# Fan-Luo/Legal-RAG

Hardware: AMD Instinct MI355X
Metric: queries/sec + Recall@10 (hybrid top-10) on UCC-en (higher is better)
Workload: dtype f32 dense (long batches: fp16 first pass, candidates re-scored in f32) / f64 bm25+fusion; 1 GPU; UCC-en 591 chunks, dense(768-d FlatIP)+BM25 hybrid fusion top-10 (BASELINE configs[1]); unique_queries=1168, top_k=10, fusion=rrf_norm_blend w=0.6/0.4 alpha=0.5 rrf_k=60 min_final=0.2

## Files before the change

### include/amdretrieval.h

```cpp
#ifndef AMDRETRIEVAL_H
#define AMDRETRIEVAL_H

#include <stdint.h>

#ifdef __cplusplus
extern "C" {
#endif

#define AMDR_OK 0
#define AMDR_EINVAL (-1)
#define AMDR_EHIP (-2)
#define AMDR_ENOMEM (-3)
#define AMDR_ENODEV (-4)

#define AMDR_MAX_K 256
#define AMDR_MAX_DIM 1024
#define AMDR_MAXSIM_DIM 128
#define AMDR_MAXSIM_QLEN 32

typedef struct amdr_dense amdr_dense_t;
typedef struct amdr_dense_small amdr_dense_small_t;
typedef struct amdr_bm25 amdr_bm25_t;
typedef struct amdr_maxsim amdr_maxsim_t;
typedef struct amdr_tokenizer amdr_tokenizer_t;
typedef struct amdr_tokenizer_device amdr_tokenizer_device_t;
typedef struct amdr_graph amdr_graph_t;

const char* amdr_last_error(void);
int amdr_version(void);
int amdr_device_count(int32_t* count);
int amdr_device_name(int32_t device, char* buf, int32_t buf_len);
int amdr_workspace_growths(int64_t* out);

int amdr_dense_create(const float* X_host, int64_t n, int32_t d, int32_t device, amdr_dense_t** out);
int amdr_dense_create_from_device(const float* X_dev, int64_t n, int32_t d, int32_t device, amdr_dense_t** out);
int amdr_dense_add(amdr_dense_t* h, const float* X_host, int64_t n_add);
int amdr_dense_ntotal(const amdr_dense_t* h, int64_t* n);
int amdr_dense_dim(const amdr_dense_t* h, int32_t* d);
int amdr_dense_reserve(amdr_dense_t* h, int32_t nq_max, int32_t k_max);
int amdr_dense_search(amdr_dense_t* h, const float* Q_host, int32_t nq, int32_t k,
                      float* scores_host, int64_t* ids_host);
int amdr_dense_search_device(amdr_dense_t* h, const float* Q_dev, int32_t nq, int32_t k,
                             float* scores_dev, int64_t* ids_dev, void* stream);
int amdr_dense_score_rows(amdr_dense_t* h, const float* Q_host, int32_t nq, const int64_t* rows_host, int32_t m,
                          float* scores_host);
int amdr_dense_read_rows(const amdr_dense_t* h, int64_t row0, int64_t nrows, float* out_host);
int amdr_dense_plan_info(const amdr_dense_t* h, int32_t nq, int32_t k, char* buf, int32_t buf_len);
int amdr_dense_workspace_plan(int64_t n, int32_t d, int32_t nq_max, int32_t k_max, int32_t nq, int32_t k, int64_t* out6);
int amdr_dense_hi_counters(amdr_dense_t* h, int64_t* out6);
int amdr_dense_profile_begin(amdr_dense_t* h, int32_t max_launches);
int amdr_dense_profile_end(amdr_dense_t* h, double* total_ms, int32_t* launches);
int amdr_dense_destroy(amdr_dense_t* h);

int amdr_bm25_create(const int64_t* term_ptr, const int32_t* post_doc, const int32_t* post_tf,
                     const double* idf, const int32_t* doc_len, int64_t n_terms, int64_t n_docs,
                     double avgdl, double k1, double b, int32_t device, amdr_bm25_t** out);
int amdr_bm25_ndocs(const amdr_bm25_t* h, int64_t* n);
int amdr_bm25_reserve(amdr_bm25_t* h, int32_t nq_max, int32_t k_max, int64_t total_terms_max);
int amdr_bm25_workspace_plan(int64_t n_docs, int32_t nq_max, int32_t k_max, int32_t nq, int32_t k, int64_t* out2);
int amdr_bm25_plan_info(const amdr_bm25_t* h, int32_t nq, int32_t k, char* buf, int32_t buf_len);
int amdr_bm25_search(amdr_bm25_t* h, const int32_t* q_terms, const int64_t* q_ptr, int32_t nq, int32_t k,
                     double* scores_host, int64_t* ids_host);
int amdr_bm25_search_device(amdr_bm25_t* h, const int32_t* q_terms_dev, const int64_t* q_ptr_dev,
                            int32_t nq, int32_t k, double* scores_dev, int64_t* ids_dev, void* stream);
int amdr_bm25_scores(amdr_bm25_t* h, const int32_t* q_terms, const int64_t* q_ptr, int32_t nq,
                     double* scores_host);
int amdr_bm25_destroy(amdr_bm25_t* h);

int amdr_tokenizer_create(const char* vocab_blob, const int64_t* vocab_offsets, int64_t n_terms, amdr_tokenizer_t** out);
int amdr_tokenizer_encode(const amdr_tokenizer_t* t, const char* text_blob, const int64_t* text_offsets, int32_t nq,
                          int32_t* term_ids, int64_t capacity, int64_t* q_ptr, int32_t* needs_segmenter);
int amdr_tokenizer_encode_joined(const amdr_tokenizer_t* t, const char* text_blob, int64_t n_bytes, int32_t nq,
                                 int32_t* term_ids, int64_t capacity, int64_t* q_ptr, int32_t* needs_segmenter);
int amdr_tokenizer_encode_ptrs(const amdr_tokenizer_t* t, const char* const* texts, const int64_t* n_bytes, int32_t nq,
                               int32_t* term_ids, int64_t capacity, int64_t* q_ptr, int32_t* needs_segmenter);
int amdr_tokenizer_spans(const char* text, int64_t n_bytes, int32_t* starts, int32_t* ends, int32_t capacity,
                         int32_t* n_tokens);
int amdr_tokenizer_destroy(amdr_tokenizer_t* t);
int amdr_tokenizer_pack(const char* const* texts, const int64_t* n_bytes, int32_t nq, char* blob, int64_t capacity,
                        int64_t* offsets);

int amdr_tokenizer_device_create(const amdr_tokenizer_t* host, int32_t device, amdr_tokenizer_device_t** out);
int amdr_tokenizer_device_reserve(amdr_tokenizer_device_t* h, int32_t nq_max, int64_t bytes_max);
int amdr_tokenizer_encode_device(amdr_tokenizer_device_t* h, const char* text_dev, const int64_t* offs_dev, int32_t nq,
                                 int64_t n_bytes, int32_t* term_ids_dev, int64_t capacity, int64_t* q_ptr_dev,
                                 int32_t* needs_segmenter_dev, void* stream);
int amdr_tokenizer_device_destroy(amdr_tokenizer_device_t* h);

int amdr_maxsim_create(const float* D_host, const int64_t* doc_ptr, int64_t n_docs, int32_t dim,
                       int32_t device, amdr_maxsim_t** out);
int amdr_maxsim_ndocs(const amdr_maxsim_t* h, int64_t* n);
int amdr_maxsim_plan_info(const amdr_maxsim_t* h, int32_t nq, char* buf, int32_t buf_len);
int amdr_maxsim_reserve(amdr_maxsim_t* h, int32_t nq_max, int32_t k_max);
int amdr_maxsim_workspace_plan(int64_t n_docs, int32_t split_image, int32_t nq_max, int32_t k_max, int32_t nq, int32_t k,
                               int64_t* out2);
int amdr_maxsim_search(amdr_maxsim_t* h, const float* Q_host, int32_t nq, int32_t q_len, int32_t k,
                       float* scores_host, int64_t* ids_host);
int amdr_maxsim_search_device(amdr_maxsim_t* h, const float* Q_dev, int32_t nq, int32_t q_len, int32_t k,
                              float* scores_dev, int64_t* ids_dev, void* stream);
int amdr_maxsim_scores(amdr_maxsim_t* h, const float* Q_host, int32_t nq, int32_t q_len, float* scores_host);
int amdr_maxsim_destroy(amdr_maxsim_t* h);

#define AMDR_FUSE_RRF_NORM_BLEND 0
#define AMDR_FUSE_RRF 1
#define AMDR_FUSE_WRRF 2
#define AMDR_FUSE_WEIGHTED_SUM 3

typedef struct amdr_fuse_params {
  int32_t method;
  int32_t rrf_k;
  double alpha;
  double w_dense, w_bm25, w_colbert;
  double min_final_score;
} amdr_fuse_params_t;

#define AMDR_FUSE_NVALS 9
#define AMDR_FV_SCORE 0
#define AMDR_FV_RRF_NORM 1
#define AMDR_FV_WSUM 2
#define AMDR_FV_NORM_DENSE 3
#define AMDR_FV_NORM_BM25 4
#define AMDR_FV_NORM_COLBERT 5
#define AMDR_FV_CONTRIB_DENSE 6
#define AMDR_FV_CONTRIB_BM25 7
#define AMDR_FV_CONTRIB_COLBERT 8

int amdr_fuse(const amdr_fuse_params_t* p, int32_t nq,
              const int64_t* dense_ids, const double* dense_scores, int32_t kd,
              const int64_t* bm25_ids, const double* bm25_scores, int32_t kb,
              const int64_t* colbert_ids, const double* colbert_scores, int32_t kc,
              int64_t* out_ids, double* out_vals, int32_t* out_mask, int32_t* out_count);
int amdr_fuse_device(const amdr_fuse_params_t* p, int32_t nq,
                     const int64_t* dense_ids, const float* dense_scores, int32_t kd, const int64_t* dense_row2uid,
                     const int64_t* bm25_ids, const double* bm25_scores, int32_t kb, const int64_t* bm25_row2uid,
                     const int64_t* colbert_ids, const float* colbert_scores, int32_t kc, const int64_t* colbert_row2uid,
                     int64_t* out_ids, double* out_vals, int32_t* out_mask, int32_t* out_count,
                     int32_t device, void* stream);

int amdr_dense_search_fuse_device(amdr_dense_t* h, const float* Q_dev, int32_t nq, int32_t k,
                                  const amdr_fuse_params_t* p, const int64_t* dense_row2uid,
                                  const int64_t* bm25_ids, const double* bm25_scores, int32_t kb,
                                  const int64_t* bm25_row2uid, float* dense_scores_dev, int64_t* dense_ids_dev,
                                  int64_t* out_ids, double* out_vals, int32_t* out_mask, int32_t* out_count,
                                  void* stream);

int amdr_hybrid_small_device(amdr_dense_t* dense, amdr_bm25_t* bm25, const float* Q_dev, const int32_t* q_terms_dev,
                             const int64_t* q_ptr_dev, int32_t nq, int32_t kd, int32_t kb, const amdr_fuse_params_t* p,
                             const int64_t* dense_row2uid, const int64_t* bm25_row2uid, float* dense_scores_dev,
                             int64_t* dense_ids_dev, double* bm25_scores_dev, int64_t* bm25_ids_dev, int64_t* out_ids,
                             double* out_vals, int32_t* out_mask, int32_t* out_count, void* stream);

int amdr_dense_two_pass_fallbacks(amdr_dense_t* h, int64_t* out);
int amdr_dense_small_create(amdr_dense_t* dense, amdr_dense_small_t** out);
int amdr_dense_small_approx_device(amdr_dense_small_t* h, const float* Q_dev, int32_t nq, float* S_dev, int64_t ldS,
                                   float* eps_dev , void* stream);
int amdr_dense_small_destroy(amdr_dense_small_t* h);

int amdr_rerank_blend(int32_t nq, int32_t max_out, const int32_t* count, int64_t* ids, double* vals,
                      int32_t* mask, const double* ce_raw, int32_t top_n, double beta, double* out_rerank);
int amdr_rerank_blend_device(int32_t nq, int32_t max_out, const int32_t* count, int64_t* ids, double* vals,
                             int32_t* mask, const double* ce_raw, int32_t top_n, double beta,
                             double* out_rerank, int32_t device, void* stream);

int amdr_fuse_compact_device(int32_t nq, int32_t max_out, int32_t w, const int64_t* ids, const double* vals,
                             const int32_t* mask, const int32_t* count, int64_t* out_rows, double* out_scores,
                             int32_t* out_mask, int32_t* out_count, int32_t device, void* stream);

typedef struct amdr_graph_params {
  int32_t limit;
  int32_t default_depth;
  int32_t lang;
  int32_t pad0;
  double min_conf;
  const int32_t* rel_max_depth;
  const int32_t* rel_allowed;
  const double* rel_weight;
  const double* decay;
} amdr_graph_params_t;
int amdr_graph_create(const int64_t* node_ptr, const int32_t* edge_dst, const int32_t* edge_rel,
                      const double* edge_conf_raw, const double* edge_conf_eff, const int32_t* edge_has_evidence,
                      const int32_t* node_present, const int64_t* node_row, const int32_t* row_node,
                      const float* row_norm, const int32_t* row_lang, int32_t n_nodes, int64_t n_edges,
                      int64_t n_rows, int32_t n_rel, int32_t device, amdr_graph_t** out);
int amdr_graph_reserve(amdr_graph_t* h, int32_t nq_max, int32_t k_max, int32_t limit_max);
int amdr_graph_walk(amdr_graph_t* h, const int64_t* seeds_host, const int32_t* seed_count_host, int32_t ld,
                    int32_t seed_n, int32_t nq, const amdr_graph_params_t* params, int32_t* out_count,
                    int32_t* out_node, int32_t* out_depth, int32_t* out_parent, int32_t* out_rel, int32_t* out_evidence,
                    double* out_conf);
int amdr_graph_search(amdr_graph_t* h, amdr_dense_t* dense, const float* Q_host, const int64_t* seeds_host,
                      const int32_t* seed_count_host, int32_t ld, int32_t seed_n, int32_t nq, int32_t k,
                      const amdr_graph_params_t* params, int32_t* out_count, int64_t* out_rows, double* out_final,
                      float* out_semantic, int32_t* out_depth, int32_t* out_rel, double* out_conf);
int amdr_graph_search_device(amdr_graph_t* h, amdr_dense_t* dense, const float* Q_dev, const int32_t* qsel_dev,
                             const int64_t* seeds_dev, const int32_t* seed_count_dev, int32_t ld, int32_t seed_n,
                             int32_t ng, int32_t k, const amdr_graph_params_t* params, int32_t* out_count,
                             int64_t* out_rows, double* out_final, float* out_semantic, int32_t* out_depth,
                             int32_t* out_rel, double* out_conf, void* stream);
int amdr_graph_destroy(amdr_graph_t* h);

int amdr_merge_topk_f32_device(const float* scores, const int64_t* ids, int32_t n_parts, int32_t nq, int32_t k_in,
                               int32_t k_out, float* out_scores, int64_t* out_ids, int32_t device, void* stream);
int amdr_merge_topk_f64_device(const double* scores, const int64_t* ids, int32_t n_parts, int32_t nq, int32_t k_in,
                               int32_t k_out, double* out_scores, int64_t* out_ids, int32_t device, void* stream);

typedef struct amdr_shard_chan {
  void* scores;
  int64_t* ids;
  int32_t k;
  int32_t f64;
} amdr_shard_chan_t;
int amdr_shard_row_words(const amdr_shard_chan_t* chans, int32_t n_chan, int64_t* words);
int amdr_shard_pack_device(const amdr_shard_chan_t* chans, int32_t n_chan, int32_t nq, int64_t id_offset, int64_t* send,
                           int32_t device, void* stream);
int amdr_shard_merge_device(const int64_t* gathered, int32_t world, int32_t nq, const amdr_shard_chan_t* out_chans,
                            int32_t n_chan, int32_t device, void* stream);

#ifdef __cplusplus
}
#endif
#endif
```

### legal-rag_amd/_native.py

```python
from __future__ import annotations

import ctypes as C
import math
import os
from pathlib import Path
from typing import Optional, Sequence, Tuple

import numpy as np

LIB_NAME = "libamdretrieval.so"
MAX_K = 256
MAX_DIM = 1024
MAXSIM_DIM = 128
MAXSIM_QLEN = 32
FUSE_NVALS = 9
FUSE_METHODS = {"rrf_norm_blend": 0, "rrf": 1, "wrrf": 2, "weighted_sum": 3}
FV = dict(score=0, rrf_norm=1, weighted_sum=2, dense_norm=3, bm25_norm=4, colbert_norm=5,
          contrib_dense=6, contrib_bm25=7, contrib_colbert=8)

EXPORTS = (
    "amdr_last_error", "amdr_version", "amdr_device_count", "amdr_device_name", "amdr_workspace_growths",
    "amdr_dense_create", "amdr_dense_create_from_device", "amdr_dense_add", "amdr_dense_ntotal", "amdr_dense_dim",
    "amdr_dense_reserve", "amdr_dense_search", "amdr_dense_search_device", "amdr_dense_search_fuse_device", "amdr_hybrid_small_device", "amdr_dense_small_create", "amdr_dense_small_approx_device", "amdr_dense_small_destroy", "amdr_dense_two_pass_fallbacks", "amdr_dense_read_rows", "amdr_dense_score_rows",
    "amdr_dense_plan_info", "amdr_dense_workspace_plan", "amdr_dense_hi_counters", "amdr_dense_profile_begin", "amdr_dense_profile_end", "amdr_dense_destroy",
    "amdr_bm25_create", "amdr_bm25_ndocs", "amdr_bm25_reserve", "amdr_bm25_workspace_plan", "amdr_bm25_plan_info", "amdr_bm25_search", "amdr_bm25_search_device",
    "amdr_bm25_scores", "amdr_bm25_destroy",
    "amdr_tokenizer_create", "amdr_tokenizer_encode", "amdr_tokenizer_encode_joined", "amdr_tokenizer_encode_ptrs", "amdr_tokenizer_spans", "amdr_tokenizer_destroy",
    "amdr_tokenizer_pack", "amdr_tokenizer_device_create", "amdr_tokenizer_device_reserve", "amdr_tokenizer_encode_device",
    "amdr_tokenizer_device_destroy",
    "amdr_maxsim_create", "amdr_maxsim_ndocs", "amdr_maxsim_plan_info", "amdr_maxsim_reserve", "amdr_maxsim_workspace_plan", "amdr_maxsim_search",
    "amdr_maxsim_search_device", "amdr_maxsim_scores", "amdr_maxsim_destroy",
    "amdr_fuse", "amdr_fuse_device", "amdr_rerank_blend", "amdr_rerank_blend_device", "amdr_fuse_compact_device",
    "amdr_merge_topk_f32_device", "amdr_merge_topk_f64_device",
    "amdr_shard_row_words", "amdr_shard_pack_device", "amdr_shard_merge_device",
    "amdr_graph_create", "amdr_graph_reserve", "amdr_graph_walk", "amdr_graph_search", "amdr_graph_search_device",
    "amdr_graph_destroy",
)


SIGNATURES = {
    "amdr_last_error": "", "amdr_version": "", "amdr_device_count": "P", "amdr_device_name": "iPi", "amdr_workspace_growths": "P",
    "amdr_dense_create": "PliiP", "amdr_dense_create_from_device": "PliiP", "amdr_dense_add": "PPl",
    "amdr_dense_ntotal": "PP", "amdr_dense_dim": "PP", "amdr_dense_reserve": "Pii", "amdr_dense_search": "PPiiPP",
    "amdr_dense_search_device": "PPiiPPP", "amdr_dense_search_fuse_device": "PPiiPPPPiPPPPPPPP", "amdr_hybrid_small_device": "PPPPPiiiPPPPPPPPPPPP", "amdr_dense_small_create": "PP", "amdr_dense_small_approx_device": "PPiPlPP", "amdr_dense_small_destroy": "P", "amdr_dense_two_pass_fallbacks": "PP", "amdr_dense_read_rows": "PllP", "amdr_dense_score_rows": "PPiPiP",
    "amdr_dense_plan_info": "PiiPi", "amdr_dense_workspace_plan": "liiiiiP", "amdr_dense_hi_counters": "PP", "amdr_dense_profile_begin": "Pi", "amdr_dense_profile_end": "PPP", "amdr_dense_destroy": "P",
    "amdr_bm25_create": "PPPPPlldddiP", "amdr_bm25_ndocs": "PP", "amdr_bm25_reserve": "Piil", "amdr_bm25_workspace_plan": "liiiiP", "amdr_bm25_plan_info": "PiiPi",
    "amdr_bm25_search": "PPPiiPP", "amdr_bm25_search_device": "PPPiiPPP", "amdr_bm25_scores": "PPPiP",
    "amdr_bm25_destroy": "P",
    "amdr_tokenizer_create": "PPlP", "amdr_tokenizer_encode": "PPPiPlPP", "amdr_tokenizer_encode_joined": "PPliPlPP", "amdr_tokenizer_encode_ptrs": "PPPiPlPP", "amdr_tokenizer_spans": "PlPPiP",
    "amdr_tokenizer_destroy": "P",
    "amdr_tokenizer_pack": "PPiPlP", "amdr_tokenizer_device_create": "PiP", "amdr_tokenizer_device_reserve": "Pil",
    "amdr_tokenizer_encode_device": "PPPilPlPPP", "amdr_tokenizer_device_destroy": "P",
    "amdr_maxsim_create": "PPliiP", "amdr_maxsim_ndocs": "PP", "amdr_maxsim_plan_info": "PiPi", "amdr_maxsim_reserve": "Pii", "amdr_maxsim_workspace_plan": "liiiiiP",
    "amdr_maxsim_search": "PPiiiPP", "amdr_maxsim_search_device": "PPiiiPPP", "amdr_maxsim_scores": "PPiiP",
    "amdr_maxsim_destroy": "P",
    "amdr_fuse": "Pi" + "PPi" * 3 + "PPPP", "amdr_fuse_device": "Pi" + "PPiP" * 3 + "PPPP" + "iP",
    "amdr_rerank_blend": "iiPPPPPidP", "amdr_rerank_blend_device": "iiPPPPPidPiP",
    "amdr_fuse_compact_device": "iiiPPPPPPPPiP",
    "amdr_merge_topk_f32_device": "PPiiiiPPiP", "amdr_merge_topk_f64_device": "PPiiiiPPiP",
    "amdr_shard_row_words": "PiP", "amdr_shard_pack_device": "PiilPiP", "amdr_shard_merge_device": "PiiPiiP",
    "amdr_graph_create": "P" * 11 + "illiiP", "amdr_graph_reserve": "Piii", "amdr_graph_walk": "PPPiiiP" + "P" * 7,
    "amdr_graph_search": "PPPPPiiiiP" + "P" * 7, "amdr_graph_search_device": "PPPPPPiiiiP" + "P" * 8,
    "amdr_graph_destroy": "P",
}
_KIND = {"P": C.c_void_p, "i": C.c_int32, "l": C.c_int64, "d": C.c_double}


class NativeError(RuntimeError):
    """A libamdretrieval call returned a non-zero status."""


class FuseParams(C.Structure):
    _fields_ = [("method", C.c_int32), ("rrf_k", C.c_int32), ("alpha", C.c_double), ("w_dense", C.c_double),
                ("w_bm25", C.c_double), ("w_colbert", C.c_double), ("min_final_score", C.c_double)]


class ShardChan(C.Structure):
    _fields_ = [("scores", C.c_void_p), ("ids", C.c_void_p), ("k", C.c_int32), ("f64", C.c_int32)]


class GraphParams(C.Structure):
    _fields_ = [("limit", C.c_int32), ("default_depth", C.c_int32), ("lang", C.c_int32), ("pad0", C.c_int32),
                ("min_conf", C.c_double), ("rel_max_depth", C.c_void_p), ("rel_allowed", C.c_void_p),
                ("rel_weight", C.c_void_p), ("decay", C.c_void_p)]


GRAPH_MAX_LIMIT = 4096
GRAPH_MAX_SEEDS = 1024


_lib: Optional[C.CDLL] = None


_pystr = False


def _pystrings():
    global _pystr
    if _pystr is False:
        _pystr = None
        p = lib_path().parent / "_amdr_pystrings.so"
        if p.exists() and os.environ.get("AMDR_NO_PYSTRINGS") != "1":
            try:
                import importlib.machinery
                import importlib.util
                loader = importlib.machinery.ExtensionFileLoader("_amdr_pystrings", str(p))
                spec = importlib.util.spec_from_loader("_amdr_pystrings", loader)
                mod = importlib.util.module_from_spec(spec)
                loader.exec_module(mod)
                _pystr = mod
            except Exception:
                _pystr = None
    return _pystr


def lib_path() -> Path:
    env = os.environ.get("AMDR_LIB")
    if env:
        return Path(env)
    return Path(__file__).resolve().parent / "lib" / LIB_NAME


def load() -> C.CDLL:
    global _lib
    if _lib is not None:
        return _lib
    if os.environ.get("AMDR_NO_TORCH_PRELOAD") != "1":
        try:
            import torch
        except Exception:
            pass
    p = lib_path()
    if not p.exists():
        raise NativeError(
            f"{p} not found: the HIP extension is not built. Run `python -c 'import __graft_entry__ as g; g.build()'` "
            f"(or `make -C legal-rag_amd/csrc`). There is no CPU fallback.")
    lib = C.CDLL(str(p))
    lib.amdr_last_error.restype = C.c_char_p
    for name in EXPORTS:
        fn = getattr(lib, name)
        if name != "amdr_last_error":
            fn.restype = C.c_int
        fn.argtypes = [_KIND[k] for k in SIGNATURES[name]]
    _lib = lib
    return lib


def _check(rc: int, what: str) -> None:
    if rc != 0:
        msg = load().amdr_last_error()
        raise NativeError(f"{what} failed (status {rc}): {msg.decode('utf-8', 'replace') if msg else ''}")


def device_count() -> int:
    n = C.c_int32(0)
    rc = load().amdr_device_count(C.byref(n))
    return int(n.value) if rc == 0 else 0


def device_name(device: int = 0) -> str:
    buf = C.create_string_buffer(256)
    _check(load().amdr_device_name(C.c_int32(device), buf, C.c_int32(256)), "amdr_device_name")
    return buf.value.decode()


def dense_workspace_plan(n: int, d: int, nq_max: int, k_max: int, nq: int,
                         k: int) -> Tuple[Tuple[int, int, int], Tuple[int, int, int]]:
    out = (C.c_int64 * 6)()
    _check(load().amdr_dense_workspace_plan(C.c_int64(n), C.c_int32(d), C.c_int32(nq_max), C.c_int32(k_max), C.c_int32(nq),
                                            C.c_int32(k), out), "amdr_dense_workspace_plan")
    v = [int(x) for x in out]
    return tuple(v[:3]), tuple(v[3:])


def bm25_workspace_plan(n_docs: int, nq_max: int, k_max: int, nq: int, k: int) -> Tuple[int, int]:
    out = (C.c_int64 * 2)()
    _check(load().amdr_bm25_workspace_plan(C.c_int64(n_docs), C.c_int32(nq_max), C.c_int32(k_max), C.c_int32(nq),
                                           C.c_int32(k), out), "amdr_bm25_workspace_plan")
    return int(out[0]), int(out[1])


def maxsim_workspace_plan(n_docs: int, split_image: bool, nq_max: int, k_max: int, nq: int, k: int) -> Tuple[int, int]:
    out = (C.c_int64 * 2)()
    _check(load().amdr_maxsim_workspace_plan(C.c_int64(n_docs), C.c_int32(1 if split_image else 0), C.c_int32(nq_max),
                                             C.c_int32(k_max), C.c_int32(nq), C.c_int32(k), out),
           "amdr_maxsim_workspace_plan")
    return int(out[0]), int(out[1])


def workspace_growths() -> int:
    n = C.c_int64(0)
    _check(load().amdr_workspace_growths(C.byref(n)), "amdr_workspace_growths")
    return int(n.value)


def _p(a: Optional[np.ndarray], ctype):
    if a is None:
        return None
    return a.ctypes.data_as(C.POINTER(ctype))


def _vp(ptr: int):
    return C.c_void_p(int(ptr) if ptr else 0)


def _c(a, dtype) -> np.ndarray:
    return np.ascontiguousarray(a, dtype=dtype)


class DenseIndex:

    def __init__(self, X: Optional[np.ndarray] = None, *, device: int = 0, dim: Optional[int] = None,
                 device_ptr: Optional[int] = None, n: Optional[int] = None, keepalive=None):
        lib = load()
        self._h = C.c_void_p()
        self.device = int(device)
        self._keepalive = keepalive
        if device_ptr is not None:
            assert n is not None and dim is not None
            _check(lib.amdr_dense_create_from_device(_vp(device_ptr), C.c_int64(n), C.c_int32(dim),
                                                     C.c_int32(device), C.byref(self._h)),
                   "amdr_dense_create_from_device")
            self.d = int(dim)
        else:
            if X is None:
                X = np.zeros((0, int(dim)), dtype=np.float32)
            X = _c(X, np.float32)
# ... 414 lines not shown
        if keep[3].shape[0] < int(limit) + 1:
            raise ValueError("decay needs limit + 1 entries")
        p = GraphParams(int(limit), int(default_depth), int(lang), 0, float(min_conf), *(x.ctypes.data or None for x in keep))
        return p, keep

    def walk(self, seeds: Sequence[Sequence[int]], params: GraphParams):
        nq = len(seeds)
        ld = max([len(s) for s in seeds] + [1])
        S = np.full((max(nq, 1), ld), -1, dtype=np.int64)
        for i, s in enumerate(seeds):
            S[i, :len(s)] = s
        cnt = np.array([len(s) for s in seeds] + [0] * (nq == 0), dtype=np.int32)
        L = int(params.limit)
        outs = [np.empty((max(nq, 1), L), dtype=t) for t in (np.int32,) * 5 + (np.float64,)]
        oc = np.zeros(max(nq, 1), dtype=np.int32)
        _check(load().amdr_graph_walk(self._h, S.ctypes.data, cnt.ctypes.data, ld, ld, nq, C.byref(params), oc.ctypes.data,
                                      *(o.ctypes.data for o in outs)), "amdr_graph_walk")
        node, depth, parent, rel, evid, conf = outs
        return [[(int(node[q, i]), int(depth[q, i]), int(parent[q, i]), int(rel[q, i]), bool(evid[q, i]),
                  float(conf[q, i])) for i in range(int(oc[q]))] for q in range(nq)]

    def search(self, dense: "DenseIndex", Q: np.ndarray, seeds: np.ndarray, seed_count: np.ndarray, seed_n: int, k: int,
               params: GraphParams):
        Q = _c(Q, np.float32).reshape(-1, dense.d)
        nq = Q.shape[0]
        seeds = _c(seeds, np.int64).reshape(nq, -1)
        seed_count = _c(seed_count, np.int32).reshape(nq)
        out = self._outputs(nq, k)
        _check(load().amdr_graph_search(self._h, dense._h, Q.ctypes.data, seeds.ctypes.data, seed_count.ctypes.data,
                                        seeds.shape[1], int(seed_n), nq, int(k), C.byref(params),
                                        *(out[n].ctypes.data for n in self.OUTS)), "amdr_graph_search")
        return out

    OUTS = ("count", "rows", "final", "semantic", "depth", "relation", "edge_conf")
    _OUT_T = (np.int32, np.int64, np.float64, np.float32, np.int32, np.int32, np.float64)

    @classmethod
    def _outputs(cls, nq: int, k: int):
        return {n: np.empty((nq,) if n == "count" else (nq, k), dtype=t) for n, t in zip(cls.OUTS, cls._OUT_T)}

    def search_device(self, dense: "DenseIndex", q_ptr: int, qsel_ptr: int, seeds_ptr: int, seed_count_ptr: int, ld: int,
                      seed_n: int, ng: int, k: int, params: GraphParams, outs: Sequence[int], stream: int = 0) -> None:
        _check(load().amdr_graph_search_device(self._h, dense._h, _vp(q_ptr), _vp(qsel_ptr), _vp(seeds_ptr),
                                               _vp(seed_count_ptr), int(ld), int(seed_n), int(ng), int(k),
                                               C.byref(params), *(_vp(o) for o in outs), _vp(stream)),
               "amdr_graph_search_device")

    def close(self) -> None:
        if getattr(self, "_h", None) and self._h.value:
            load().amdr_graph_destroy(self._h)
            self._h = C.c_void_p()

    def __del__(self):
        try:
            self.close()
        except Exception:
            pass


def make_fuse_params(*, method: str = "rrf_norm_blend", rrf_k: int = 60, alpha: float = 0.5, w_dense: float = 0.6,
                     w_bm25: float = 0.4, w_colbert: float = 0.35, min_final_score: float = -math.inf) -> FuseParams:
    m = FUSE_METHODS.get(str(method).lower(), 0)
    return FuseParams(m, int(rrf_k), float(alpha), float(w_dense), float(w_bm25), float(w_colbert),
                      float(min_final_score))


def _chan(ids, scores, sdtype, nq):
    if ids is None or scores is None:
        return None, None, 0
    ids = _c(ids, np.int64).reshape(nq, -1)
    scores = _c(scores, sdtype).reshape(nq, -1)
    assert ids.shape == scores.shape
    if ids.shape[1] == 0:
        return None, None, 0
    return ids, scores, int(ids.shape[1])


def fuse(params: FuseParams, nq: int, dense=None, bm25=None, colbert=None):
    di, ds, kd = _chan(*(dense or (None, None)), np.float64, nq)
    bi, bs, kb = _chan(*(bm25 or (None, None)), np.float64, nq)
    ci, cs, kc = _chan(*(colbert or (None, None)), np.float64, nq)
    mo = kd + kb + kc
    out_ids = np.full((nq, max(mo, 1)), -1, dtype=np.int64)
    out_vals = np.zeros((nq, max(mo, 1), FUSE_NVALS), dtype=np.float64)
    out_mask = np.zeros((nq, max(mo, 1)), dtype=np.int32)
    out_count = np.zeros((nq,), dtype=np.int32)
    if mo == 0 or nq == 0:
        return out_ids[:, :0], out_vals[:, :0], out_mask[:, :0], out_count
    _check(load().amdr_fuse(C.byref(params), C.c_int32(nq), _p(di, C.c_int64), _p(ds, C.c_double), C.c_int32(kd),
                            _p(bi, C.c_int64), _p(bs, C.c_double), C.c_int32(kb), _p(ci, C.c_int64),
                            _p(cs, C.c_double), C.c_int32(kc), _p(out_ids, C.c_int64), _p(out_vals, C.c_double),
                            _p(out_mask, C.c_int32), _p(out_count, C.c_int32)), "amdr_fuse")
    return out_ids, out_vals, out_mask, out_count


def fuse_device(params: FuseParams, nq: int, dense, bm25, colbert, out_ids: int, out_vals: int, out_mask: int,
                out_count: int, *, device: int = 0, stream: int = 0) -> None:
    def un(c):
        return c if c is not None else (0, 0, 0, 0)
    d, b, c = un(dense), un(bm25), un(colbert)
    _check(load().amdr_fuse_device(C.byref(params), C.c_int32(nq),
                                   _vp(d[0]), _vp(d[1]), C.c_int32(d[2]), _vp(d[3]),
                                   _vp(b[0]), _vp(b[1]), C.c_int32(b[2]), _vp(b[3]),
                                   _vp(c[0]), _vp(c[1]), C.c_int32(c[2]), _vp(c[3]),
                                   _vp(out_ids), _vp(out_vals), _vp(out_mask), _vp(out_count),
                                   C.c_int32(device), _vp(stream)), "amdr_fuse_device")


def rerank_blend(count: np.ndarray, ids: np.ndarray, vals: np.ndarray, mask: np.ndarray, ce_raw: np.ndarray,
                 beta: float):
    nq, max_out = ids.shape
    ce_raw = _c(ce_raw, np.float64).reshape(nq, -1)
    top_n = int(ce_raw.shape[1])
    out = np.full((nq, max_out, 2), np.nan, dtype=np.float64)
    assert ids.flags.c_contiguous and vals.flags.c_contiguous and mask.flags.c_contiguous
    count = _c(count, np.int32)
    _check(load().amdr_rerank_blend(C.c_int32(nq), C.c_int32(max_out), _p(count, C.c_int32), _p(ids, C.c_int64),
                                    _p(vals, C.c_double), _p(mask, C.c_int32), _p(ce_raw, C.c_double),
                                    C.c_int32(top_n), C.c_double(beta), _p(out, C.c_double)), "amdr_rerank_blend")
    return out


def rerank_blend_device(nq: int, max_out: int, count: int, ids: int, vals: int, mask: int, ce_raw: int, top_n: int,
                        beta: float, out_rerank: int, *, device: int = 0, stream: int = 0) -> None:
    _check(load().amdr_rerank_blend_device(C.c_int32(nq), C.c_int32(max_out), _vp(count), _vp(ids), _vp(vals),
                                           _vp(mask), _vp(ce_raw), C.c_int32(top_n), C.c_double(beta),
                                           _vp(out_rerank), C.c_int32(device), _vp(stream)),
           "amdr_rerank_blend_device")


class DenseSmallApprox:

    def __init__(self, dense: "DenseIndex"):
        self._h = C.c_void_p()
        self._dense = dense
        _check(load().amdr_dense_small_create(dense._h, C.byref(self._h)), "amdr_dense_small_create")

    def approx_device(self, q_ptr: int, nq: int, s_ptr: int, ld: int, eps_ptr: int = 0, stream: int = 0) -> None:
        _check(load().amdr_dense_small_approx_device(self._h, _vp(q_ptr), C.c_int32(nq), _vp(s_ptr), C.c_int64(ld), _vp(eps_ptr),
                                                     _vp(stream)), "amdr_dense_small_approx_device")

    def close(self) -> None:
        if self._h:
            load().amdr_dense_small_destroy(self._h)
            self._h = C.c_void_p()

    def __del__(self):
        try:
            self.close()
        except Exception:
            pass


def hybrid_small_plan(dense: "DenseIndex", bm25: "BM25Index", nq: int, kd: int, kb: int, dense_row2uid: int,
                      bm25_row2uid: int, dense_scores: int, dense_ids: int, bm25_scores: int, bm25_ids: int, out_ids: int,
                      out_vals: int, out_mask: int, out_count: int):
    return (load().amdr_hybrid_small_device, dense._h, bm25._h, C.c_int32(nq), C.c_int32(kd), C.c_int32(kb),
            _vp(dense_row2uid), _vp(bm25_row2uid), _vp(dense_scores), _vp(dense_ids), _vp(bm25_scores), _vp(bm25_ids),
            _vp(out_ids), _vp(out_vals), _vp(out_mask), _vp(out_count))


def hybrid_small_device(plan, params: "FuseParams", q_emb: int, q_terms: int, q_ptr: int, stream: int = 0) -> None:
    fn, dh, bh, nq, kd, kb, m0, m1, ds, di, bs, bi, oi, ov, om, oc = plan
    rc = fn(dh, bh, q_emb, q_terms, q_ptr, nq, kd, kb, C.byref(params), m0, m1, ds, di, bs, bi, oi, ov, om, oc, stream)
    if rc:
        _check(rc, "amdr_hybrid_small_device")


def fuse_compact_device(nq: int, max_out: int, w: int, ids: int, vals: int, mask: int, count: int, out_rows: int,
                        out_scores: int, out_mask: int, out_count: int, *, device: int = 0, stream: int = 0) -> None:
    _check(load().amdr_fuse_compact_device(nq, max_out, w, ids, vals, mask, count, out_rows, out_scores, out_mask, out_count,
                                           device, stream), "amdr_fuse_compact_device")


def merge_topk_device(scores: int, ids: int, n_parts: int, nq: int, k_in: int, k_out: int, out_scores: int,
                      out_ids: int, *, f64: bool, device: int = 0, stream: int = 0) -> None:
    fn = load().amdr_merge_topk_f64_device if f64 else load().amdr_merge_topk_f32_device
    _check(fn(_vp(scores), _vp(ids), C.c_int32(n_parts), C.c_int32(nq), C.c_int32(k_in), C.c_int32(k_out),
              _vp(out_scores), _vp(out_ids), C.c_int32(device), _vp(stream)), "amdr_merge_topk_device")


def shard_chans(chans):
    arr = (ShardChan * len(chans))()
    for c, (sp, ip, k, f64) in zip(arr, chans):
        c.scores, c.ids, c.k, c.f64 = int(sp) if sp else None, int(ip) if ip else None, int(k), 1 if f64 else 0
    return arr, len(chans)


def shard_row_words(ks: Sequence[int]) -> int:
    arr, n = shard_chans([(0, 0, k, False) for k in ks])
    w = C.c_int64(0)
    _check(load().amdr_shard_row_words(arr, C.c_int32(n), C.byref(w)), "amdr_shard_row_words")
    return int(w.value)


def shard_pack_args(args, nq: int, id_offset: int, send_ptr: int, *, device: int = 0, stream: int = 0) -> None:
    _check(load().amdr_shard_pack_device(args[0], args[1], nq, id_offset, send_ptr, device, stream),
           "amdr_shard_pack_device")


def shard_merge_args(gathered_ptr: int, world: int, nq: int, args, *, device: int = 0, stream: int = 0) -> None:
    _check(load().amdr_shard_merge_device(gathered_ptr, world, nq, args[0], args[1], device, stream),
           "amdr_shard_merge_device")


def shard_pack_device(chans, nq: int, id_offset: int, send_ptr: int, *, device: int = 0, stream: int = 0) -> None:
    shard_pack_args(shard_chans(chans), nq, id_offset, send_ptr, device=device, stream=stream)


def shard_merge_device(gathered_ptr: int, world: int, nq: int, out_chans, *, device: int = 0, stream: int = 0) -> None:
    shard_merge_args(gathered_ptr, world, nq, shard_chans(out_chans), device=device, stream=stream)
```

### legal-rag_amd/csrc/bm25.hip

```cpp
#include "common.hpp"
#include "topk.hpp"

#include <cfloat>
#include <cmath>
#include <cstdlib>
#include <mutex>
#include <new>
#include <vector>


#include "bm25_core.hpp"

using namespace amdr;

struct amdr_bm25 {
  int device = 0;
  int64_t n_terms = 0, n_docs = 0, nnz = 0;
  double avgdl = 0, k1 = 1.5, b = 0.75;
  long long* term_ptr = nullptr;
  int* post_doc = nullptr;
  double* post_w = nullptr;
  double* idf = nullptr;
  hipStream_t stream = nullptr;
  std::mutex mu;
  DevBuf part[2], qterms, qptr, sbuf, ibuf, full;
  DevBuf ticket;
};

namespace {

constexpr int kSlabMax = 4096;

struct BmPlan {
  int slab, nslabs, cap, cap_merge, waves;
  size_t lds, part_bytes;
};

void bm_plan(int64_t n_docs, int nq, int k, BmPlan* p) {
  const int64_t n = n_docs > 0 ? n_docs : 1;
  auto balanced = [&](int slab_max) {
    p->nslabs = (int)((n + slab_max - 1) / slab_max);
    p->slab = (int)(((n + p->nslabs - 1) / p->nslabs + 15) / 16 * 16);
    if (p->slab > slab_max) p->slab = slab_max;
    p->nslabs = (int)((n + p->slab - 1) / p->slab);
  };
  balanced(kBmOneWaveDocs);
  const bool argmax = bm_use_argmax(k, p->slab);
  if (!argmax) balanced(kSlabMax);
  p->waves = 1;
  p->cap_merge = topk_cap(k);
  p->cap = argmax ? (k <= 16 ? 16 : kBmArgmaxK) : p->cap_merge;
  p->lds = (size_t)p->slab * sizeof(double) + (size_t)p->waves * p->cap * sizeof(C64) + 4 * sizeof(int) +
           128 * sizeof(long) + 8;
  p->part_bytes = (size_t)p->nslabs * nq * k * sizeof(C64);
}

size_t bm_part_bytes(int64_t n_docs, int nq, int k) {
  BmPlan p;
  bm_plan(n_docs, nq, k, &p);
  return p.part_bytes;
}
size_t bm_reserve_bytes(int64_t n_docs, int nq_max, int k_max) {
  size_t need = 0;
  for (int k = 1; k <= k_max; ++k) {
    const size_t b = bm_part_bytes(n_docs, nq_max, k);
    need = b > need ? b : need;
  }
  return need;
}

static bool bm_select_enabled() {
  const char* e = getenv("AMDR_BM25_SELECT");
  return !(e && e[0] == '0');
}

int bm_run(amdr_bm25* h, int ws, const int* q_terms_dev, const long long* q_ptr_dev, int nq, int k, double* scores_dev,
           int64_t* ids_dev, double* full_dev, hipStream_t st) {
  BmPlan p;
  bm_plan(h->n_docs, nq, k, &p);
  C64* part = nullptr;
  if (scores_dev) {
    int rc = h->part[ws].ensure(bm_part_bytes(h->n_docs, nq, k));
    if (rc) return rc;
    part = h->part[ws].as<C64>();
  }
  const bool direct = scores_dev && p.nslabs == 1;
  double* fs = direct ? scores_dev : nullptr;
  long long* fi = direct ? (long long*)ids_dev : nullptr;
  if (direct) part = nullptr;
  if (p.lds > 48 * 1024) {
    return fail(AMDR_EINVAL, "bm25: slab needs %zu B of LDS", p.lds);
  }
#define AMDR_BM_LAUNCH(NVT)                                                                                          \
  hipLaunchKernelGGL((bm25_score_topk_kernel<1, NVT>), dim3(p.nslabs, nq), dim3(64), p.lds, st, h->term_ptr,         \
                     h->post_doc, h->post_w, h->idf, (long)h->n_terms, (long)h->n_docs, q_terms_dev, q_ptr_dev, nq, k, \
                     p.cap, p.slab, bm_select_enabled() ? 1 : 0, full_dev, part, fs, fi)
  const int nv = bm_use_argmax(k, p.slab) ? (p.slab + 63) / 64 : 1;
  if (nv <= 4) AMDR_BM_LAUNCH(4);
  else if (nv <= 8) AMDR_BM_LAUNCH(8);
  else if (nv <= 10) AMDR_BM_LAUNCH(10);
  else if (nv <= 16) AMDR_BM_LAUNCH(16);
  else if (nv <= 20) AMDR_BM_LAUNCH(20);
  else AMDR_BM_LAUNCH(32);
#undef AMDR_BM_LAUNCH
  AMDR_HIP(hipGetLastError());
  if (scores_dev && !direct) {
    size_t lds = (size_t)kBmWaves * p.cap_merge * sizeof(C64) + kBmWaves * sizeof(int);
    hipLaunchKernelGGL(bm25_merge_kernel, dim3(nq), dim3(256), lds, st, part, p.nslabs, nq, k, p.cap_merge, scores_dev,
                       (long long*)ids_dev);
    AMDR_HIP(hipGetLastError());
  }
  return AMDR_OK;
}

}
namespace amdr {
int bm25_small_raw(amdr_bm25_t* h, int nq, int k, Bm25Raw* out) {
  if (!h->ticket.p) return fail(AMDR_EINVAL, "bm25: handle without arrival counters");
  BmPlan p;
  bm_plan(h->n_docs, nq, k, &p);
  out->term_ptr = h->term_ptr;
  out->post_doc = h->post_doc;
  out->post_w = h->post_w;
  out->idf = h->idf;
  out->n_terms = (long)h->n_terms;
  out->n_docs = (long)h->n_docs;
  out->ticket = h->ticket.as<int>();
  out->slab = p.slab;
  out->nslabs = p.nslabs;
  out->cap = p.cap;
  out->lds = p.lds;
  out->argmax = bm_use_argmax(k, p.slab);
  out->nvt = out->argmax ? (p.slab + 63) / 64 : 1;
  out->select_on = bm_select_enabled();
  return AMDR_OK;
}
std::mutex& bm25_mutex(amdr_bm25_t* h) { return h->mu; }
}
namespace {

template <class T>
int upload(T** dst, const T* src, size_t count) {
  *dst = nullptr;
  size_t bytes = (count + 1) * sizeof(T);
  AMDR_HIP(hipMalloc((void**)dst, bytes));
  if (count) AMDR_HIP(hipMemcpy(*dst, src, count * sizeof(T), hipMemcpyHostToDevice));
  return AMDR_OK;
}

}

extern "C" {

int amdr_bm25_create(const int64_t* term_ptr, const int32_t* post_doc, const int32_t* post_tf, const double* idf,
                     const int32_t* doc_len, int64_t n_terms, int64_t n_docs, double avgdl, double k1, double b,
                     int32_t device, amdr_bm25_t** out) {
  AMDR_REQUIRE(out != nullptr, "bm25_create: out is null");
  *out = nullptr;
  AMDR_REQUIRE(term_ptr && idf && doc_len, "bm25_create: null array");
  AMDR_REQUIRE(n_terms >= 0 && n_docs >= 1 && n_docs < (1ll << 31), "bm25_create: bad sizes");
  AMDR_REQUIRE(n_terms < (1ll << 31), "bm25_create: too many terms");
  AMDR_REQUIRE(term_ptr[0] == 0, "bm25_create: term_ptr[0] != 0");
  for (int64_t t = 0; t < n_terms; ++t)
    AMDR_REQUIRE(term_ptr[t + 1] >= term_ptr[t], "bm25_create: term_ptr not monotone at %lld", (long long)t);
  const int64_t nnz = term_ptr[n_terms];
  AMDR_REQUIRE(nnz == 0 || (post_doc && post_tf), "bm25_create: null postings");
  for (int64_t t = 0; t < n_terms; ++t)
    for (int64_t p = term_ptr[t]; p < term_ptr[t + 1]; ++p) {
      AMDR_REQUIRE(post_doc[p] >= 0 && post_doc[p] < n_docs, "bm25_create: posting %lld doc out of range", (long long)p);
      AMDR_REQUIRE(p == term_ptr[t] || post_doc[p] > post_doc[p - 1],
                   "bm25_create: postings of term %lld not strictly ascending", (long long)t);
    }
  int rc = check_device(device);
  if (rc) return rc;
  amdr_bm25* h = new (std::nothrow) amdr_bm25();
  if (!h) return fail(AMDR_ENOMEM, "bm25_create: host alloc");
  h->device = device;
  h->n_terms = n_terms;
  h->n_docs = n_docs;
  h->nnz = nnz;
  h->avgdl = avgdl;
  h->k1 = k1;
  h->b = b;
  std::vector<double> pw((size_t)nnz);
  {
    const double k1p1 = k1 + 1, one_minus_b = 1 - b;
    for (int64_t p = 0; p < nnz; ++p) {
      const double qf = (double)post_tf[p];
      const double dl = (double)doc_len[post_doc[p]];
      const double denom = qf + k1 * (one_minus_b + b * dl / avgdl);
      pw[(size_t)p] = qf * k1p1 / denom;
    }
  }
  rc = upload(&h->term_ptr, (const long long*)term_ptr, (size_t)n_terms + 1);
  if (!rc) rc = upload(&h->post_doc, post_doc, (size_t)nnz);
  if (!rc) rc = upload(&h->post_w, pw.data(), (size_t)nnz);
  if (!rc) rc = upload(&h->idf, idf, (size_t)n_terms);
  if (!rc && hipStreamCreateWithFlags(&h->stream, hipStreamNonBlocking) != hipSuccess)
    rc = fail(AMDR_EHIP, "bm25_create: stream");
  if (!rc) rc = h->ticket.ensure(64 * sizeof(int));
  if (!rc && hipMemset(h->ticket.p, 0, 64 * sizeof(int)) != hipSuccess) rc = fail(AMDR_EHIP, "bm25_create: memset");
  if (rc) {
    amdr_bm25_destroy(h);
    return rc;
  }
  *out = h;
  return AMDR_OK;
}

int amdr_bm25_ndocs(const amdr_bm25_t* h, int64_t* n) {
  AMDR_REQUIRE(h && n, "bm25_ndocs: null");
  *n = h->n_docs;
  return AMDR_OK;
}

int amdr_bm25_reserve(amdr_bm25_t* h, int32_t nq_max, int32_t k_max, int64_t total_terms_max) {
  AMDR_REQUIRE(h != nullptr, "bm25_reserve: null handle");
  AMDR_REQUIRE(nq_max >= 1 && k_max >= 1 && k_max <= AMDR_MAX_K && total_terms_max >= 0, "bm25_reserve: bad sizes");
  std::lock_guard<std::mutex> g(h->mu);
  AMDR_HIP(hipSetDevice(h->device));
  int rc = h->part[0].ensure(bm_reserve_bytes(h->n_docs, nq_max, k_max));
  if (!rc) rc = h->qterms.ensure((size_t)(total_terms_max + 1) * sizeof(int));
  if (!rc) rc = h->qptr.ensure((size_t)(nq_max + 1) * sizeof(long long));
  if (!rc) rc = h->sbuf.ensure((size_t)nq_max * k_max * sizeof(double));
  if (!rc) rc = h->ibuf.ensure((size_t)nq_max * k_max * sizeof(int64_t));
  return rc;
}

int amdr_bm25_workspace_plan(int64_t n_docs, int32_t nq_max, int32_t k_max, int32_t nq, int32_t k, int64_t* out2) {
  AMDR_REQUIRE(out2 != nullptr, "bm25_workspace_plan: null");
  AMDR_REQUIRE(n_docs >= 1 && n_docs < (1ll << 31), "bm25_workspace_plan: bad n_docs");
  AMDR_REQUIRE(nq_max >= 1 && k_max >= 1 && k_max <= AMDR_MAX_K && nq >= 1 && k >= 1 && k <= AMDR_MAX_K,
               "bm25_workspace_plan: bad sizes");
  out2[0] = (int64_t)bm_reserve_bytes(n_docs, nq_max, k_max);
  out2[1] = (int64_t)bm_part_bytes(n_docs, nq, k);
  return AMDR_OK;
}

int amdr_bm25_plan_info(const amdr_bm25_t* h, int32_t nq, int32_t k, char* buf, int32_t buf_len) {
  AMDR_REQUIRE(h && buf && buf_len > 0, "bm25_plan_info: null");
  AMDR_REQUIRE(nq >= 1 && k >= 1 && k <= AMDR_MAX_K, "bm25_plan_info: bad sizes");
  BmPlan p;
  bm_plan(h->n_docs, nq, k, &p);
  snprintf(buf, buf_len, "bm25_score_topk_kernel slabs=%d of <= %d documents, ranked by %s%s", p.nslabs, p.slab,
           bm_use_argmax(k, p.slab) ? "the register arg-max rounds" : "the staged selector",
           p.nslabs == 1 ? " (one slab: direct)" : " + bm25_merge_kernel");
  return AMDR_OK;
}

static int bm_check(const amdr_bm25* h, const void* qt, const void* qp, int nq, int k) {
  AMDR_REQUIRE(h != nullptr, "bm25: null handle");
  AMDR_REQUIRE(nq >= 0, "bm25: nq=%d", nq);
  AMDR_REQUIRE(k >= 1 && k <= AMDR_MAX_K, "bm25: k=%d outside [1,%d]", k, AMDR_MAX_K);
  AMDR_REQUIRE(nq == 0 || qp, "bm25: null q_ptr");
  (void)qt;
  return AMDR_OK;
}

int amdr_bm25_search_device(amdr_bm25_t* h, const int32_t* q_terms_dev, const int64_t* q_ptr_dev, int32_t nq,
                            int32_t k, double* scores_dev, int64_t* ids_dev, void* stream) {
  int rc = bm_check(h, q_terms_dev, q_ptr_dev, nq, k);
  if (rc) return rc;
  AMDR_REQUIRE(nq == 0 || (scores_dev && ids_dev), "bm25: null output");
  if (nq == 0) return AMDR_OK;
  std::lock_guard<std::mutex> g(h->mu);
  AMDR_HIP(hipSetDevice(h->device));
  return bm_run(h, 0, q_terms_dev, (const long long*)q_ptr_dev, nq, k, scores_dev, ids_dev, nullptr, (hipStream_t)stream);
}

static int bm_stage_queries(amdr_bm25* h, const int32_t* q_terms, const int64_t* q_ptr, int nq) {
  AMDR_REQUIRE(q_ptr[0] == 0, "bm25: q_ptr[0] != 0");
  for (int i = 0; i < nq; ++i) AMDR_REQUIRE(q_ptr[i + 1] >= q_ptr[i], "bm25: q_ptr not monotone");
  const int64_t tot = q_ptr[nq];
  AMDR_REQUIRE(tot == 0 || q_terms, "bm25: null q_terms");
  int rc = h->qterms.ensure((size_t)(tot + 1) * sizeof(int));
  if (!rc) rc = h->qptr.ensure((size_t)(nq + 1) * sizeof(long long));
  if (rc) return rc;
  if (tot) AMDR_HIP(hipMemcpyAsync(h->qterms.p, q_terms, (size_t)tot * sizeof(int), hipMemcpyHostToDevice, h->stream));
  AMDR_HIP(hipMemcpyAsync(h->qptr.p, q_ptr, (size_t)(nq + 1) * sizeof(long long), hipMemcpyHostToDevice, h->stream));
  return AMDR_OK;
}

int amdr_bm25_search(amdr_bm25_t* h, const int32_t* q_terms, const int64_t* q_ptr, int32_t nq, int32_t k,
                     double* scores_host, int64_t* ids_host) {
  int rc = bm_check(h, q_terms, q_ptr, nq, k);
  if (rc) return rc;
  AMDR_REQUIRE(nq == 0 || (scores_host && ids_host), "bm25: null output");
  if (nq == 0) return AMDR_OK;
  std::lock_guard<std::mutex> g(h->mu);
  AMDR_HIP(hipSetDevice(h->device));
// ... 55 lines not shown
```

### legal-rag_amd/csrc/bm25_core.hpp

```cpp
#pragma once
#include "common.hpp"
#include "topk.hpp"

#include <cfloat>
#include <cmath>

namespace amdr {

constexpr int kBmWaves = 4;
constexpr int kBmArgmaxK = 96;
__host__ __device__ inline bool bm_use_argmax(int k, int slab) {
  return slab <= 2048 && (k <= 16 || (k <= kBmArgmaxK && k * ((slab + 63) >> 6) <= 480));
}
constexpr int kBmTok = 32;
constexpr int kBmOneWaveDocs = 2048;

__device__ __forceinline__ long uniform_i64(long v) {
  const unsigned lo = (unsigned)__builtin_amdgcn_readfirstlane((int)(unsigned)((unsigned long)v & 0xffffffffu));
  const unsigned hi = (unsigned)__builtin_amdgcn_readfirstlane((int)(unsigned)((unsigned long)v >> 32));
  return (long)(((unsigned long)hi << 32) | lo);
}

__device__ __forceinline__ long lower_bound_i32(const int* __restrict__ a, long lo, long hi, int key) {
  while (lo < hi) {
// ... 6 lines not shown
  return lo;
}

__device__ __forceinline__ double bm25_ranked(double raw) {
  const double x = raw + 0.0;
  return (x != x) ? -DBL_MAX : x;
}

template <int NV>
__device__ __forceinline__ int bm25_argmax_rounds(const double* sc, int m, int k, long lo, int lane, C64* out) {
  const double ninf = -INFINITY;
  double sv[NV];
#pragma unroll
  for (int v = 0; v < NV; ++v) sv[v] = (lane + 64 * v < m) ? bm25_ranked(sc[lane + 64 * v]) : ninf;
  int got = 0;
#if defined(AMDR_BM_ABL) && AMDR_BM_ABL == 1
  for (int it = 0; it < 1; ++it) {
#else
  for (int it = 0; it < k; ++it) {
#endif
    double lm = sv[0];
#pragma unroll
    for (int v = 1; v < NV; ++v) lm = max_f64_raw(lm, sv[v]);
    const double wm = wave_allmax_f64(lm);
    if (wm == ninf) break;
    unsigned long long fm = 0ull;
    int fv = 0;
#pragma unroll
    for (int v = NV - 1; v >= 0; --v) {
      const unsigned long long hit = __ballot(sv[v] == wm);
      fm = hit ? hit : fm;
      fv = hit ? v : fv;
    }
    const int wl = (int)__builtin_ctzll(fm);
    const bool mine = (lane == wl);
#pragma unroll
    for (int v = 0; v < NV; ++v) sv[v] = (mine && v == fv) ? ninf : sv[v];
    if (lane == 0) out[it] = C64::make(wm, lo + wl + 64 * fv);
    got = it + 1;
  }
  return got;
}

template <int NV>
__device__ __forceinline__ int bm25_select_f32(const double* sc, int m, int k, long lo, int lane, C32* scratch,
                                               double* xs , C64* out) {
  u32 img[NV];
  u32 lb = 0u;
#pragma unroll
  for (int v = 0; v < NV; ++v) {
    const int i = lane + 64 * v;
    img[v] = (i < m) ? ord32((float)sc[lane + 64 * v]) : 0u;
    lb = img[v] > lb ? img[v] : lb;
  }
  u32 T = 0u;
#pragma unroll
  for (int bit = 31; bit >= 0; --bit) {
    const u32 cand = T | (1u << bit);
    T = (__popcll(__ballot(lb >= cand)) >= k) ? cand : T;
  }
  const u32 Te = T > 1u ? T : 1u;
  int mine = 0;
#pragma unroll
  for (int v = 0; v < NV; ++v) mine += (img[v] >= Te) ? 1 : 0;
  int incl = mine;
#pragma unroll
  for (int s = 1; s < 64; s <<= 1) {
    const int o = __shfl_up(incl, s);
    incl += (lane >= s) ? o : 0;
  }
  int cnt = __builtin_amdgcn_readlane(incl, 63);
  const bool overflow = cnt > 64;
  if (!overflow) {
    int at = incl - mine;
#pragma unroll
    for (int v = 0; v < NV; ++v) {
      if (img[v] >= Te) {
        C32 c;
        c.c = ((u64)img[v] << 32) | (u64)(((0xffffu - (u32)(lane + 64 * v)) << 8) | (u32)at);
        scratch[at] = c;
        xs[at] = bm25_ranked(sc[lane + 64 * v]);
        ++at;
      }
    }
  }
  if (overflow) {
    int above = 0;
#pragma unroll
    for (int v = 0; v < NV; ++v) above += __popcll(__ballot(img[v] > T));
    if (T == 0u || above > 64) return -1;
    int need = k - above;
    need = need < 0 ? 0 : need;
    if (need > 0) {
      double x0 = 0.0;
      bool have = false;
#pragma unroll
      for (int v = 0; v < NV; ++v) {
        const u64 mk = __ballot(img[v] == T);
        if (!have && mk) {
          x0 = __shfl(bm25_ranked(sc[lane + 64 * v]), (int)__builtin_ctzll(mk));
          have = true;
        }
      }
      u64 differ = 0ull;
#pragma unroll
      for (int v = 0; v < NV; ++v) differ |= __ballot(img[v] == T && bm25_ranked(sc[lane + 64 * v]) != x0);
      if (differ) return -1;
    }
    cnt = 0;
#pragma unroll
    for (int v = 0; v < NV; ++v) {
      const bool hi = img[v] > T;
      const bool eq = img[v] == T;
      const u64 mh = __ballot(hi), me = __ballot(eq);
      const int before_h = (int)__builtin_amdgcn_mbcnt_hi((u32)(mh >> 32), __builtin_amdgcn_mbcnt_lo((u32)mh, 0u));
      const int before_e = (int)__builtin_amdgcn_mbcnt_hi((u32)(me >> 32), __builtin_amdgcn_mbcnt_lo((u32)me, 0u));
      const int nh = __popcll(mh);
      int ne = __popcll(me);
      ne = ne < need ? ne : need;
      const bool take = hi || (eq && before_e < ne);
      if (take) {
        const int at = cnt + (hi ? before_h : nh + before_e);
        C32 c;
        c.c = ((u64)img[v] << 32) | (u64)(((0xffffu - (u32)(lane + 64 * v)) << 8) | (u32)at);
        scratch[at] = c;
        xs[at] = bm25_ranked(sc[lane + 64 * v]);
      }
      cnt += nh + ne;
      need -= ne;
    }
  }
  wave_lds_fence();
  C32 c = (lane < cnt) ? scratch[lane] : C32::pad();
  if (cnt <= 16)
    c = wave_sortN_desc<C32, 16>(c, lane);
  else if (cnt <= 32)
    c = wave_sortN_desc<C32, 32>(c, lane);
  else
    c = wave_sortN_desc<C32, 64>(c, lane);
  const u32 low = (u32)c.c;
  const int doc = (lane < cnt) ? (int)(0xffffu - (low >> 8)) : 0;
  const double x = xs[(lane < cnt) ? (int)(low & 63u) : 0];
  const u32 im = (u32)(c.c >> 32);
  const u32 im_n = (u32)__shfl_down((int)im, 1);
  const double x_n = __shfl_down(x, 1);
  const bool undecided = lane < k && lane + 1 < cnt && im == im_n && x != x_n;
  if (__ballot(undecided)) return -1;
  const int got = cnt < k ? cnt : k;
  if (lane < got) out[lane] = C64::make(x, lo + doc);
  return got;
}

__device__ __forceinline__ void bm25_all_zero_result(int m, int k, long lo, int lane, size_t row, double* fin_scores,
                                                     long long* fin_ids, C64* part_row) {
  for (int j = lane; j < k; j += 64) {
    const bool v = j < m;
    if (fin_ids) {
      fin_scores[row * k + j] = v ? 0.0 : -DBL_MAX;
      fin_ids[row * k + j] = v ? lo + j : -1ll;
    } else {
      part_row[j] = v ? C64::make(0.0, lo + j) : C64::pad();
    }
  }
}

template <int NV>
__device__ __forceinline__ int bm25_rank_slab(const double* sc, int m, int k, long lo, int lane, bool use_select,
                                              C32* scratch, double* xs, C64* out) {
  int got = -1;
  if (k <= 64 && use_select) {
    got = bm25_select_f32<NV>(sc, m, k, lo, lane, scratch, xs, out);
    wave_lds_fence();
  }
  if (got < 0) {
    got = bm25_argmax_rounds<NV>(sc, m, k, lo, lane, out);
    wave_lds_fence();
  }
  return got;
}

template <int WAVES, int NVT>
__device__ __forceinline__ void bm25_block_query(
    const long long* __restrict__ term_ptr, const int* __restrict__ post_doc, const double* __restrict__ post_w,
    const double* __restrict__ idf, long n_terms, long n_docs, const int* __restrict__ q_terms,
    const long long* __restrict__ q_ptr, int nq, int k, int cap, int slab, int use_select,
    double* __restrict__ scores_out , C64* __restrict__ part ,
    double* __restrict__ fin_scores , long long* __restrict__ fin_ids,
    int qi_arg, int slab_ix, unsigned char* smem) {
  double* sc = reinterpret_cast<double*>(smem);
  C64* lists = reinterpret_cast<C64*>(sc + slab);
  int* cnts = reinterpret_cast<int*>(lists + (size_t)WAVES * cap);
  long* tk_ps = reinterpret_cast<long*>(cnts + 4);
  long* tk_pe = tk_ps + kBmTok;
  double* tk_w = reinterpret_cast<double*>(tk_pe + kBmTok);
  int* tk_n = reinterpret_cast<int*>(tk_ps + 128);
  constexpr int NT = WAVES * 64;

  const int tid = threadIdx.x, lane = tid & 63, wave = tid >> 6;
  const int qi = qi_arg;
  const long lo = (long)slab_ix * slab;
  long hi = lo + slab;
  if (hi > n_docs) hi = n_docs;
  const int m = (int)(hi - lo);

  for (int i = tid; i < m; i += NT) sc[i] = 0.0;
  block_sync<WAVES>();

  int nt_total = 0;
  const long t0 = q_ptr[qi], t1 = q_ptr[qi + 1];
  for (long tb = t0; tb < t1; tb += kBmTok) {
    const int nt_all = (int)((t1 - tb) < kBmTok ? (t1 - tb) : kBmTok);
    if (tid < 64) {
      long ps = 0, pe = 0;
      double w = 0.0;
      if (tid < nt_all) {
        const int term = q_terms[tb + tid];
        if (term >= 0 && term < n_terms) {
          const long p0 = term_ptr[term], p1 = term_ptr[term + 1];
          ps = (lo == 0) ? p0 : lower_bound_i32(post_doc, p0, p1, (int)lo);
          pe = (hi >= n_docs) ? p1 : lower_bound_i32(post_doc, ps, p1, (int)hi);
          w = idf[term];
        }
      }
      const bool keep = pe > ps;
      const unsigned long long km = __ballot(keep);
      const unsigned long long below = (tid == 0) ? 0ull : (km & (~0ull >> (64 - tid)));
      if (keep) {
        const int at = __popcll(below);
        tk_ps[at] = ps;
        tk_pe[at] = pe;
        tk_w[at] = w;
      }
      if (tid == 0) *tk_n = __popcll(km);
    }
    block_sync<WAVES>();
    const int nt = __builtin_amdgcn_readfirstlane(*tk_n);
    nt_total += nt;
    if (nt == 0) {
      block_sync<WAVES>();
      continue;
    }
    constexpr int kAhead = 8;
    int t = 0, base = 0;
    long ps = uniform_i64(tk_ps[0]);
    int len = __builtin_amdgcn_readfirstlane((int)(tk_pe[0] - tk_ps[0]));
    double w = tk_w[0];
#if defined(AMDR_BM_ABL) && AMDR_BM_ABL == 2
    t = nt;
#endif
    while (t < nt) {
      int dd[kAhead];
      double ww[kAhead], wv[kAhead];
      bool ok[kAhead];
#pragma unroll
      for (int u = 0; u < kAhead; ++u) {
        const bool have = t < nt;
        const int j = base + tid;
        ok[u] = have && j < len;
        int jj = ok[u] ? j : len - 1;
        jj = jj < 0 ? 0 : jj;
        dd[u] = post_doc[ps + jj];
        ww[u] = post_w[ps + jj];
        wv[u] = w;
        if (have) {
          base += NT;
          if (base >= len) {
            ++t;
            base = 0;
            if (t < nt) {
              ps = uniform_i64(tk_ps[t]);
              len = __builtin_amdgcn_readfirstlane((int)(tk_pe[t] - tk_ps[t]));
              w = tk_w[t];
            }
          }
        }
      }
#pragma unroll
      for (int u = 0; u < kAhead; ++u) {
        if (WAVES == 1) {
          if (ok[u])
            __hip_atomic_fetch_add(&sc[dd[u] - lo], wv[u] * ww[u], __ATOMIC_RELAXED, __HIP_MEMORY_SCOPE_WAVEFRONT);
        } else {
          if (ok[u]) sc[dd[u] - lo] += wv[u] * ww[u];
          block_sync<WAVES>();
        }
      }
      if (WAVES == 1) wave_lds_fence();
    }
  }

  if (scores_out) {
    for (int i = tid; i < m; i += NT) scores_out[(size_t)qi * n_docs + lo + i] = sc[i];
  }
  if (!part && !fin_ids) return;
  if (nt_total == 0) {
    if (wave == 0)
      bm25_all_zero_result(m, k, lo, lane, (size_t)qi, fin_scores, fin_ids,
                           part ? part + ((size_t)slab_ix * nq + qi) * k : nullptr);
    return;
  }
#if defined(AMDR_BM_ABL) && AMDR_BM_ABL == 3
  if (fin_ids && tid < k) {
    fin_ids[(size_t)qi * k + tid] = tid;
    fin_scores[(size_t)qi * k + tid] = sc[tid];
  }
  return;
#endif

  WaveTopK<C64> tk;
  tk.init(lists + (size_t)wave * cap, cap, k);
  bool done = false;
  if (WAVES == 1 && bm_use_argmax(k, slab)) {
    C32* scratch = reinterpret_cast<C32*>(tk_ps);
    double* xs = reinterpret_cast<double*>(tk_ps + 64);
    const int got = bm25_rank_slab<NVT>(sc, m, k, lo, lane, use_select != 0, scratch, xs, tk.buf);
    tk.cnt = got;
    done = true;
  }
  if (!done) {
    for (int base = wave * 64; base < m; base += WAVES * 64) {
      int i = base + lane;
      bool v = i < m;
      C64 c = v ? C64::make(sc[i], lo + i) : C64::pad();
      tk.push_lanes(c, v, lane);
    }
    tk.finalize(lane);
  }
  if (WAVES > 1) block_combine_topk(tk, lists, cap, WAVES, wave, lane, cnts);
  if (wave == 0) {
    if (fin_ids) {
      for (int j = lane; j < k; j += 64) {
        bool v = j < tk.cnt;
        fin_scores[(size_t)qi * k + j] = v ? unord64(tk.buf[j].key) : -DBL_MAX;
        fin_ids[(size_t)qi * k + j] = v ? tk.buf[j].idv : -1ll;
      }
    } else {
      C64* dst = part + ((size_t)slab_ix * nq + qi) * k;
      for (int j = lane; j < k; j += 64) dst[j] = (j < tk.cnt) ? tk.buf[j] : C64::pad();
    }
  }
}

template <int WAVES, int NVT>
__global__ __launch_bounds__(WAVES * 64) void bm25_score_topk_kernel(
    const long long* __restrict__ term_ptr, const int* __restrict__ post_doc, const double* __restrict__ post_w,
    const double* __restrict__ idf, long n_terms, long n_docs, const int* __restrict__ q_terms,
    const long long* __restrict__ q_ptr, int nq, int k, int cap, int slab, int use_select,
    double* __restrict__ scores_out , C64* __restrict__ part ,
    double* __restrict__ fin_scores , long long* __restrict__ fin_ids) {
  extern __shared__ __attribute__((aligned(16))) unsigned char smem[];
  bm25_block_query<WAVES, NVT>(term_ptr, post_doc, post_w, idf, n_terms, n_docs, q_terms, q_ptr, nq, k, cap, slab, use_select, scores_out, part, fin_scores, fin_ids,
                               (int)blockIdx.y, (int)blockIdx.x, smem);
}

static __global__ __launch_bounds__(256) void bm25_merge_kernel(const C64* __restrict__ part, int nparts, int nq, int k,
                                                          int cap, double* __restrict__ out_scores,
                                                          long long* __restrict__ out_ids) {
  extern __shared__ __attribute__((aligned(16))) unsigned char smem[];
  C64* lists = reinterpret_cast<C64*>(smem);
  int* cnts = reinterpret_cast<int*>(lists + (size_t)kBmWaves * cap);
  const int lane = threadIdx.x & 63, wave = threadIdx.x >> 6;
  const int qi = blockIdx.x;
  WaveTopK<C64> tk;
  tk.init(lists + (size_t)wave * cap, cap, k);
  const long total = (long)nparts * k;
  for (long base = (long)wave * 64; base < total; base += (long)kBmWaves * 64) {
    long i = base + lane;
    bool v = i < total;
    C64 c = C64::pad();
    if (v) {
      long p = i / k, j = i - p * k;
      c = part[((size_t)p * nq + qi) * k + j];
      v = !c.is_pad();
    }
    tk.push_lanes(c, v, lane);
  }
  tk.finalize(lane);
  block_combine_topk(tk, lists, cap, kBmWaves, wave, lane, cnts);
  if (wave == 0) {
    for (int j = lane; j < k; j += 64) {
      bool v = j < tk.cnt;
      C64 c = v ? tk.buf[j] : C64::pad();
      out_scores[(size_t)qi * k + j] = v ? unord64(c.key) : -DBL_MAX;
      out_ids[(size_t)qi * k + j] = v ? c.idv : -1ll;
    }
  }
}

}
```

### legal-rag_amd/csrc/dense.hip

```cpp
#include "common.hpp"
#include "dense_dot.hpp"
#include "topk.hpp"

#include <algorithm>
#include <cfloat>
#include <mutex>
#include <new>
#include <vector>

namespace amdr {

constexpr int kWaves = 4;

template <int NQ, int CH, int U, bool NT>
__global__ __launch_bounds__(256) void dense_scan_topk_kernel(const float* __restrict__ X, long n, int d,
                                                               const float* __restrict__ Q, int nq_total, int k,
                                                               int cap, long rows_per_block,
                                                               C32* __restrict__ part ,
                                                               float* __restrict__ fin_scores ,
                                                               long long* __restrict__ fin_ids) {
  extern __shared__ __attribute__((aligned(16))) unsigned char smem[];
  C32* lists = reinterpret_cast<C32*>(smem);
  int* cnts = reinterpret_cast<int*>(lists + (size_t)kWaves * NQ * cap);

  const int lane = threadIdx.x & 63;
  const int wave = threadIdx.x >> 6;
  const int qbase = blockIdx.y * NQ;

  float4 q[NQ][CH];
#pragma unroll
  for (int b = 0; b < NQ; ++b) {
#pragma unroll
    for (int c = 0; c < CH; ++c) {
      int col = c * 256 + lane * 4;
      bool ok = (qbase + b < nq_total) && (col < d);
      q[b][c] = ok ? *reinterpret_cast<const float4*>(Q + (size_t)(qbase + b) * d + col) : make_float4(0, 0, 0, 0);
    }
  }

  WaveTopK<C32> tk[NQ];
#pragma unroll
  for (int b = 0; b < NQ; ++b) tk[b].init(lists + ((size_t)b * kWaves + wave) * cap, cap, k);

  const long row_lo = (long)blockIdx.x * rows_per_block;
  long row_hi = row_lo + rows_per_block;
  if (row_hi > n) row_hi = n;

  for (long r0 = row_lo + (long)wave * U; r0 < row_hi; r0 += (long)kWaves * U) {
    float4 x[U][CH];
#pragma unroll
    for (int u = 0; u < U; ++u) {
      long r = r0 + u;
      if (r >= row_hi) r = row_hi - 1;
      const float* xr = X + (size_t)r * d;
#pragma unroll
      for (int c = 0; c < CH; ++c) {
        int col = c * 256 + lane * 4;
        if (NT) {
          typedef float nt4 __attribute__((ext_vector_type(4)));
          const nt4 t_ = (col < d) ? __builtin_nontemporal_load(reinterpret_cast<const nt4*>(xr + col)) : nt4{0, 0, 0, 0};
          x[u][c] = make_float4(t_.x, t_.y, t_.z, t_.w);
        } else {
          x[u][c] = (col < d) ? *reinterpret_cast<const float4*>(xr + col) : make_float4(0, 0, 0, 0);
        }
      }
    }
#pragma unroll
    for (int u = 0; u < U; ++u) {
      const long r = r0 + u;
      const bool rv = r < row_hi;
#pragma unroll
      for (int b = 0; b < NQ; ++b) {
        float acc = 0.f;
#pragma unroll
        for (int c = 0; c < CH; ++c) acc = dot4(x[u][c], q[b][c], acc);
        acc = wave_sum_to_lane63(acc);
        float s = __int_as_float(__builtin_amdgcn_readlane(__float_as_int(acc), 63));
        if (rv) tk[b].push_uniform(C32::make(s, (u32)r), lane);
      }
    }
  }

#pragma unroll
  for (int b = 0; b < NQ; ++b) tk[b].finalize(lane);
#pragma unroll
  for (int b = 0; b < NQ; ++b) {
    block_combine_topk(tk[b], lists + (size_t)b * kWaves * cap, cap, kWaves, wave, lane, cnts);
    if (wave == 0 && qbase + b < nq_total) {
      if (fin_ids) {
        for (int j = lane; j < k; j += 64) {
          const bool v = j < tk[b].cnt;
          const C32 c = v ? tk[b].buf[j] : C32::pad();
          fin_scores[(size_t)(qbase + b) * k + j] = v ? c.score() : -FLT_MAX;
          fin_ids[(size_t)(qbase + b) * k + j] = v ? c.id() : -1ll;
        }
      } else {
        C32* dst = part + ((size_t)blockIdx.x * nq_total + (qbase + b)) * k;
        for (int j = lane; j < k; j += 64) dst[j] = (j < tk[b].cnt) ? tk[b].buf[j] : C32::pad();
      }
    }
    __syncthreads();
  }
}

__global__ __launch_bounds__(256) void dense_score_rows_kernel(const float* __restrict__ X, long n, int d,
                                                                const float* __restrict__ Q, int nq,
                                                                const long long* __restrict__ rows, int m,
                                                                float* __restrict__ out) {
  const int lane = threadIdx.x & 63, wave = threadIdx.x >> 6;
  const long idx = (long)blockIdx.x * kWaves + wave;
  if (idx >= (long)nq * m) return;
  const int qi = (int)(idx / m);
  const long long r = rows[idx];
  if (r < 0 || r >= n) {
    if (lane == 0) out[idx] = -FLT_MAX;
    return;
  }
  const float acc = dense_row_dot(X + (size_t)r * d, Q + (size_t)qi * d, d, lane);
  if (lane == 63) out[idx] = acc;
}

__global__ __launch_bounds__(256) void dense_all_scores_kernel(const float* __restrict__ X, long n, int d,
                                                                const float* __restrict__ Q, int nq, long ldS,
                                                                float* __restrict__ S) {
  const int lane = threadIdx.x & 63, wave = threadIdx.x >> 6;
  const long idx = (long)blockIdx.x * kWaves + wave;
  if (idx >= (long)nq * n) return;
  const int qi = (int)(idx / n);
  const long r = idx - (long)qi * n;
  const float acc = dense_row_dot(X + (size_t)r * d, Q + (size_t)qi * d, d, lane);
  if (lane == 63) S[(size_t)qi * ldS + r] = acc;
}

__global__ __launch_bounds__(256) void dense_merge_kernel(const C32* __restrict__ part, int nparts, int nq, int k,
                                                           int cap, float* __restrict__ out_scores,
                                                           long long* __restrict__ out_ids) {
  extern __shared__ __attribute__((aligned(16))) unsigned char smem[];
  C32* lists = reinterpret_cast<C32*>(smem);
  int* cnts = reinterpret_cast<int*>(lists + (size_t)kWaves * cap);
  const int lane = threadIdx.x & 63, wave = threadIdx.x >> 6;
  const int qi = blockIdx.x;
  WaveTopK<C32> tk;
  tk.init(lists + (size_t)wave * cap, cap, k);
  const long total = (long)nparts * k;
  for (long base = (long)wave * 64; base < total; base += (long)kWaves * 64) {
    long i = base + lane;
    bool v = i < total;
    C32 c = C32::pad();
    if (v) {
      long p = i / k, j = i - p * k;
      c = part[((size_t)p * nq + qi) * k + j];
      v = !c.is_pad();
    }
// ... 324 lines not shown
  p->kc = kc;
  p->tiles = ((long)h->n + 31) / 32;
  dense_mfma_plan((long)h->n, h->d, m, k, &p->scan, grids);
  p->ldM = (p->tiles + 31) / 32 * 32;
  p->scan.ld = p->ldM;
  p->ldS2 = (long)kc * 32;
  p->qcap = dense_hi2_qcap((long)h->n, p->qtiles, kc);
  p->off_S2 = up((size_t)m * p->ldM * sizeof(float));
  p->off_MT = p->off_S2 + up((size_t)m * p->ldS2 * sizeof(float));
  p->off_qlist = p->off_MT + up((size_t)(2048 + 64 * kHi2Tiles) * 64 * sizeof(float));
  p->smat_bytes = p->off_qlist + up((size_t)m * p->qcap * sizeof(C32));
  p->off_count = up((size_t)m * kc * sizeof(int));
  p->off_unres = p->off_count + up((size_t)m * sizeof(int));
  p->off_tau = p->off_unres + up((size_t)m * sizeof(int));
  p->off_qcount = p->off_tau + up((size_t)m * sizeof(float));
  p->off_flag = p->off_qcount + up((size_t)m * sizeof(unsigned int));
  p->aux_bytes = p->off_flag + 256;
}

struct TwoLevelPlan {
  DenseMfmaPlan scan, tk1, pass2;
  long tiles, cand_rows;
  size_t m_bytes, s2_bytes, aux_bytes, part_bytes;
};
void two_level_plan(const amdr_dense* h, int m, int k, TwoLevelPlan* t, bool grids = true) {
  t->tiles = ((long)h->n + 31) / 32;
  dense_mfma_plan((long)h->n, h->d, m, k, &t->scan, grids);
  dense_mfma_plan(t->tiles, h->d, m, k, &t->tk1, false);
  t->scan.ld = t->tk1.ld;
  t->cand_rows = (long)m * k * 32;
  dense_mfma_plan(t->cand_rows, h->d, m, k, &t->pass2, grids);
  t->m_bytes = ((size_t)m * t->tk1.ld * sizeof(float) + 255) / 256 * 256;
  t->s2_bytes = ((size_t)m * t->pass2.ld * sizeof(float) + 255) / 256 * 256;
  t->aux_bytes = (size_t)m * k * (sizeof(int64_t) + sizeof(float)) + (size_t)(m * k + 64) * sizeof(int) + 256 + 256;
  t->part_bytes = t->tk1.part_bytes > t->pass2.part_bytes ? t->tk1.part_bytes : t->pass2.part_bytes;
}

struct Need {
  size_t smat, part, aux;
  void add(const Need& o) { smat = std::max(smat, o.smat), part = std::max(part, o.part), aux = std::max(aux, o.aux); }
};
size_t score_rows_bytes(const amdr_dense* h, int nq) { return (size_t)nq * (size_t)(((long)h->n + 31) / 32 * 32) * sizeof(float); }

Need pass_need(const amdr_dense* h, Form form, int m, int k) {
  if (form == Form::Scan) {
    ScanPlan p;
    make_plan(h->n, h->d, m, k, &p);
    return {0, p.part_bytes, 0};
  }
  if (form == Form::TwoLevel) {
    TwoLevelPlan t;
    two_level_plan(h, m, k, &t, false);
    return {t.m_bytes + t.s2_bytes, t.part_bytes, t.aux_bytes};
  }
  if (form == Form::Hi) {
    Hi2Plan p;
    hi2_plan(h, m, k, hi_kc_max(k), &p, false);
    return {p.smat_bytes, 0, p.aux_bytes};
  }
  DenseMfmaPlan p;
  dense_mfma_plan((long)h->n, h->d, m, k, &p, false);
  return {p.s_bytes, p.part_bytes, 0};
}
Need call_need(const amdr_dense* h, const Route& r, int nq, int k) {
  const Form form = r.hi ? Form::TwoLevel : r.form;
  const int chunk = r.hi ? two_level_chunk(nq, k) : r.chunk;
  Need need = pass_need(h, form, chunk, k);
  if (nq % chunk) need.add(pass_need(h, form, nq % chunk, k));
  if (r.hi) need.add(pass_need(h, Form::Hi, hi2_chunk(h, nq), k));
  return need;
}
Need reserve_need(const amdr_dense* h, const DensePins& pins, int nq_max, int k_max) {
  Need need{0, 0, 0};
  int ks[8], nk = 0;
  for (int k = 1; k < k_max; ++k)
    if (topk_cap(k + 1) != topk_cap(k)) ks[nk++] = k;
  ks[nk++] = k_max;
  int nq = 1;
  for (; nq <= nq_max; ++nq) {
    const Route r = dense_route(h, pins, nq, k_max);
    if (r.form != Form::Scan && r.form != Form::RowWaves) break;
    for (int i = 0; i < nk; ++i) need.add(pass_need(h, r.form, r.chunk, ks[i]));
    if (r.form == Form::RowWaves) need.add({score_rows_bytes(h, r.chunk), 0, 0});
  }
  if (nq > nq_max) return need;
  int k_batched = 0;
  for (int k = 1; k <= k_max; ++k) {
    const Route lo = dense_route(h, pins, nq, k), hi = dense_route(h, pins, nq_max, k);
    if (lo.form == Form::Batched || hi.form == Form::Batched) k_batched = k;
    if (hi.hi) need.add(pass_need(h, Form::Hi, hi2_chunk(h, nq_max), k));
    if (hi.hi || lo.form == Form::TwoLevel || hi.form == Form::TwoLevel)
      for (int m = two_level_chunk(nq_max, k); m >= 1; --m) need.add(pass_need(h, Form::TwoLevel, m, k));
  }
  if (k_batched)
    for (int m = batched_chunk(h, nq_max); m >= 1; --m) need.add(pass_need(h, Form::Batched, m, k_batched));
  return need;
}
int ensure_need(amdr_dense* h, int ws, const Need& need) {
  int rc = h->smat[ws].ensure(need.smat);
  if (!rc) rc = h->part[ws].ensure(need.part);
  if (!rc) rc = h->aux[ws].ensure(need.aux);
  return rc;
}

template <class F>
int profiled(amdr_dense* h, hipStream_t st, F&& launch) {
  const bool on = h->prof_on && (size_t)(h->prof_used + 2) <= h->prof_ev.size();
  if (on) AMDR_HIP(hipEventRecord(h->prof_ev[h->prof_used], st));
  const int rc = launch();
  if (rc) return rc;
  if (on) {
    AMDR_HIP(hipEventRecord(h->prof_ev[h->prof_used + 1], st));
    h->prof_used += 2;
  }
  return AMDR_OK;
}

int launch_merge(const C32* part, int nparts, int nq, int k, int cap, float* out_scores, int64_t* out_ids, hipStream_t st) {
  const size_t lds = (size_t)kWaves * cap * sizeof(C32) + kWaves * sizeof(int);
  hipLaunchKernelGGL(dense_merge_kernel, dim3(nq), dim3(256), lds, st, part, nparts, nq, k, cap, out_scores, (long long*)out_ids);
  AMDR_HIP(hipGetLastError());
  return AMDR_OK;
}
int topk_pass(const DenseMfmaPlan& p, const float* S, long cols, int m, int k, DevBuf& partb, float* out_scores,
              int64_t* out_ids, hipStream_t st) {
  const bool direct = p.slabs == 1;
  int rc = dense_mfma_launch_topk(p, S, cols, m, k, partb.p, direct ? out_scores : nullptr, direct ? out_ids : nullptr, st);
  if (rc || direct) return rc;
  return launch_merge(partb.as<C32>(), p.slabs, m, k, p.cap, out_scores, out_ids, st);
}

bool small_hi_ready(amdr_dense* h, int m, hipStream_t st) {
  if (h->small_failed) return false;
  hipStreamCaptureStatus cs = hipStreamCaptureStatusNone;
  const bool capturing = st && hipStreamIsCapturing(st, &cs) == hipSuccess && cs != hipStreamCaptureStatusNone;
  if (!h->small) {
    if (capturing) return false;
    if (dense_small_create_from(h->device, h->X, h->n, h->d, &h->small) != AMDR_OK || !dense_small_usable(h->small)) {
      h->small_failed = true;
      return false;
    }
  }
  const size_t need = (size_t)m * sizeof(float);
  if (capturing && (h->small_eps.cap < need || !h->small_fb.p)) return false;
  if (h->small_eps.ensure(need) != AMDR_OK) return false;
  if (!h->small_fb.p) {
    if (h->small_fb.ensure(sizeof(unsigned int)) != AMDR_OK) return false;
    (void)hipMemset(h->small_fb.p, 0, sizeof(unsigned int));
  }
  return capturing ? true : dense_small_reserve(h->small, m) == AMDR_OK;
}

int run_search_batched(amdr_dense* h, int ws, const DensePins& pins, const Route& r, const float* Q_dev, int nq, int k,
                       float* scores_dev, int64_t* ids_dev, hipStream_t st, const FuseTail* tail) {
  float* S = h->smat[ws].as<float>();
  const long n = (long)h->n;
  DenseMfmaPlan p;
  int rc;
  for (int q0 = 0; q0 < nq; q0 += r.chunk) {
    const int m = nq - q0 < r.chunk ? nq - q0 : r.chunk;
    if (q0 == 0 || m != r.chunk) dense_mfma_plan(n, h->d, m, k, &p);
    const PassForm f = batched_pass_form(h, pins, r, p, m, k, tail);
    const float* Qc = Q_dev + (size_t)q0 * h->d;
    float* os = scores_dev + (size_t)q0 * k;
    int64_t* oi = ids_dev + (size_t)q0 * k;
    if (f.small_hi && small_hi_ready(h, m, st)) {
      rc = profiled(h, st, [&] { return amdr_dense_small_approx_device(h->small, Qc, m, S, p.ld, h->small_eps.as<float>(), st); });
      if (rc) return rc;
      if ((rc = dense_hi_select_launch(tail, q0, S, p.ld, n, m, k, h->X, Qc, h->d, h->small_eps.as<float>(), os, oi,
                                       h->small_fb.as<unsigned int>(), st)))
        return rc;
      continue;
    }
    rc = profiled(h, st, [&]() -> int {
      if (f.scores == PassForm::RowWaves) {
        hipLaunchKernelGGL(dense_all_scores_kernel, dim3(ceil_div((long)m * n, kWaves)), dim3(256), 0, st, h->X, n, h->d, Qc,
                           m, p.ld, S);
        AMDR_HIP(hipGetLastError());
        return AMDR_OK;
      }
      if (f.scores == PassForm::Panel) {
        DensePanelPlan pp;
        dense_panel_plan(n, h->d, m, &pp);
        return dense_panel_launch_scores(pp, h->X, n, h->d, Qc, m, p.ld, S, st);
      }
      return dense_mfma_launch_scores(p, h->X, n, h->d, Qc, m, S, st);
    });
    if (rc) return rc;
    if (f.select_fuse) {
      if ((rc = dense_select_fuse_launch(*tail, q0, S, p.ld, n, m, k, p.cap, os, oi, st))) return rc;
      continue;
    }
    if ((rc = topk_pass(p, S, n, m, k, h->part[ws], os, oi, st))) return rc;
    if (tail && (rc = dense_fuse_plain_launch(*tail, q0, m, k, os, oi, st))) return rc;
  }
  return AMDR_OK;
}

int two_level_pass(amdr_dense* h, int ws, const float* Qc, int m, int k, float* out_scores, int64_t* out_ids,
                   hipStream_t st) {
  TwoLevelPlan t;
  two_level_plan(h, m, k, &t);
  float* M = h->smat[ws].as<float>();
  float* S2 = reinterpret_cast<float*>(reinterpret_cast<unsigned char*>(h->smat[ws].p) + t.m_bytes);
  unsigned char* aux = reinterpret_cast<unsigned char*>(h->aux[ws].p);
  int64_t* tile_ids = reinterpret_cast<int64_t*>(aux);
  float* tile_max = reinterpret_cast<float*>(aux + (size_t)m * k * sizeof(int64_t));
  int* list = reinterpret_cast<int*>(aux + (size_t)m * k * (sizeof(int64_t) + sizeof(float)));
  int* count = list + (size_t)m * k;
  int rc;
  if ((rc = profiled(h, st, [&] { return dense_mfma_launch_scores(t.scan, h->X, (long)h->n, h->d, Qc, m, M, st, 1); }))) return rc;
  if ((rc = topk_pass(t.tk1, M, t.tiles, m, k, h->part[ws], tile_max, tile_ids, st))) return rc;
  if ((rc = dense_tiles_unique_launch(tile_ids, m * k, t.tiles, list, count, st))) return rc;
  if ((rc = dense_mfma_launch_scores(t.pass2, h->X, t.cand_rows, h->d, Qc, m, S2, st, 2, list, count, (long)h->n))) return rc;
  if ((rc = topk_pass(t.pass2, S2, t.cand_rows, m, k, h->part[ws], out_scores, out_ids, st))) return rc;
  return dense_tiles_remap_launch(out_ids, m * k, list, count, (long)h->n, st);
}

int hi2_pass(amdr_dense* h, int ws, const float* Qc, int m, int k, int kc, float* out_scores, int64_t* out_ids, hipStream_t st) {
  Hi2Plan p;
  hi2_plan(h, m, k, kc, &p);
  unsigned char* sm = reinterpret_cast<unsigned char*>(h->smat[ws].p);
  unsigned char* ax = reinterpret_cast<unsigned char*>(h->aux[ws].p);
  float* M = reinterpret_cast<float*>(sm);
  float* S2 = reinterpret_cast<float*>(sm + p.off_S2);
  float* MT = reinterpret_cast<float*>(sm + p.off_MT);
  C32* qlist = reinterpret_cast<C32*>(sm + p.off_qlist);
  int* list = reinterpret_cast<int*>(ax);
  int* count = reinterpret_cast<int*>(ax + p.off_count);
  int* unres = reinterpret_cast<int*>(ax + p.off_unres);
  float* tau = reinterpret_cast<float*>(ax + p.off_tau);
  unsigned int* qcount = reinterpret_cast<unsigned int*>(ax + p.off_qcount);
  int* flag = reinterpret_cast<int*>(ax + p.off_flag);
  unsigned int* stats = h->stats.as<unsigned int>();
  int rc;
  if ((rc = dense_hi2_launch_sample(h->X, (long)h->n, h->d, Qc, m, p.qtiles, MT, st, h->x_scale))) return rc;
  if ((rc = dense_hi2_launch_tau(MT, (long)h->n, h->d, m, p.qtiles, kc, tau, qcount, flag, stats, st))) return rc;
  {
    const char* sp = getenv("AMDR_DENSE_HI_SCANS");
    const bool split = sp && sp[0] == 's';
    const int qt = dense_hi_max_queries(h->d);
    for (int y = 0; y < (split ? p.qtiles : 1); ++y) {
      const int q0 = y * qt, mq = split ? (m - q0 < qt ? m - q0 : qt) : m;
      rc = profiled(h, st, [&] {
        return dense_hi2_launch_emit(h->X, (long)h->n, h->d, Qc + (size_t)q0 * h->d, mq, tau + q0, qlist + (size_t)q0 * p.qcap,
                                     qcount + q0, p.qcap, st, h->x_scale, split ? 1 : p.qtiles);
      });
      if (rc) return rc;
    }
  }
  h->hi_queries += m;
  h->hi_passes += p.qtiles;
  if ((rc = dense_hi2_launch_select(qlist, qcount, p.qcap, m, kc, k, Qc, h->d, h->row_norm_max, h->x_scale, p.tiles, list,
                                    count, unres, flag, stats + 2, st)))
    return rc;
  if ((rc = dense_mfma_launch_scores(p.scan, h->X, (long)h->n, h->d, Qc, m, M, st, 1, nullptr, nullptr, 0, flag))) return rc;
  if ((rc = dense_hi2_launch_exact_select(M, p.ldM, p.tiles, m, k, kc, list, count, unres, flag, st))) return rc;
  if ((rc = dense_rescore_tiles_launch(h->X, (long)h->n, h->d, Qc, m, list, count, kc, kc, p.ldS2, S2, st))) return rc;
  return dense_final_topk_launch(S2, p.ldS2, list, count, kc, kc, (long)h->n, m, k, out_scores, out_ids, st);
}

int run_search_two_level(amdr_dense* h, int ws, const DensePins& pins, Route r, const float* Q_dev, int nq, int k,
                         float* scores_dev, int64_t* ids_dev, hipStream_t st) {
  hipStreamCaptureStatus cap_st = hipStreamCaptureStatusNone;
  (void)hipStreamIsCapturing(st, &cap_st);
  const bool capturing = cap_st != hipStreamCaptureStatusNone;
  if (r.hi && !capturing && hi_adapt(h, pins)) r = dense_route(h, pins, nq, k);
  const bool hi = r.form == Form::Hi;
  int rc;
  for (int q0 = 0; q0 < nq; q0 += r.chunk) {
    const int m = nq - q0 < r.chunk ? nq - q0 : r.chunk;
    const float* Qc = Q_dev + (size_t)q0 * h->d;
    float* os = scores_dev + (size_t)q0 * k;
    int64_t* oi = ids_dev + (size_t)q0 * k;
    rc = hi ? hi2_pass(h, ws, Qc, m, k, r.kc, os, oi, st) : two_level_pass(h, ws, Qc, m, k, os, oi, st);
    if (rc) return rc;
  }
  if (hi && h->hi_host && !capturing && !h->hi_copy_pending) {
    AMDR_HIP(hipMemcpyAsync(h->hi_host, h->stats.as<unsigned int>() + 2, 3 * sizeof(unsigned int), hipMemcpyDeviceToHost, st));
    AMDR_HIP(hipEventRecord(h->hi_ev, st));
    h->hi_copy_pending = true;
  }
  return AMDR_OK;
}

int run_search_scan(amdr_dense* h, int ws, const float* Q_dev, int nq, int k, float* scores_dev, int64_t* ids_dev,
                    hipStream_t st) {
  ScanPlan p;
  make_plan(h->n, h->d, nq, k, &p);
  C32* part = h->part[ws].as<C32>();
  const bool direct = h->n > 0 && p.grid_x == 1;
  float* fs = direct ? scores_dev : nullptr;
  int64_t* fi = direct ? ids_dev : nullptr;
  if (h->n > 0) {
    const int rc = profiled(h, st, [&] {
      switch (p.nq_per_block) {
        case 1: return launch_scan_ch<1>(p, h, Q_dev, nq, k, part, fs, fi, st);
        case 2: return launch_scan_ch<2>(p, h, Q_dev, nq, k, part, fs, fi, st);
        case 4: return launch_scan_ch<4>(p, h, Q_dev, nq, k, part, fs, fi, st);
        default: return launch_scan_ch<8>(p, h, Q_dev, nq, k, part, fs, fi, st);
      }
    });
    if (rc) return rc;
  }
  if (direct) return AMDR_OK;
  return launch_merge(part, h->n > 0 ? p.grid_x : 0, nq, k, p.cap, scores_dev, ids_dev, st);
}

int run_search(amdr_dense* h, int ws, const float* Q_dev, int nq, int k, float* scores_dev, int64_t* ids_dev,
               hipStream_t st, const FuseTail* tail = nullptr) {
  const DensePins pins = read_pins();
  const Route r = dense_route(h, pins, nq, k);
  int rc = ensure_need(h, ws, call_need(h, r, nq, k));
  if (rc) return rc;
  switch (r.form) {
    case Form::Batched: return run_search_batched(h, ws, pins, r, Q_dev, nq, k, scores_dev, ids_dev, st, tail);
    case Form::RowWaves: rc = run_search_batched(h, ws, pins, r, Q_dev, nq, k, scores_dev, ids_dev, st, nullptr); break;
    case Form::TwoLevel:
    case Form::Hi: rc = run_search_two_level(h, ws, pins, r, Q_dev, nq, k, scores_dev, ids_dev, st); break;
    case Form::Scan: rc = run_search_scan(h, ws, Q_dev, nq, k, scores_dev, ids_dev, st); break;
  }
  if (rc || !tail) return rc;
  return dense_fuse_plain_launch(*tail, 0, nq, k, scores_dev, ids_dev, st);
}

int check_search_args(const amdr_dense* h, const void* Q, int nq, int k, const void* s, const void* i) {
// ... 52 lines not shown

extern "C" {

int amdr_dense_create(const float* X_host, int64_t n, int32_t d, int32_t device, amdr_dense_t** out) {
  AMDR_REQUIRE(out != nullptr, "dense_create: out is null");
  *out = nullptr;
  AMDR_REQUIRE(n >= 0 && n < (1ll << 32), "dense_create: n=%lld outside [0, 2^32)", (long long)n);
  AMDR_REQUIRE(d >= 4 && d <= AMDR_MAX_DIM && d % 4 == 0, "dense_create: d=%d must be a multiple of 4 in [4,%d]", d,
               AMDR_MAX_DIM);
  AMDR_REQUIRE(n == 0 || X_host != nullptr, "dense_create: X is null");
  int rc = check_device(device);
  if (rc) return rc;
  amdr_dense* h = new (std::nothrow) amdr_dense();
  if (!h) return fail(AMDR_ENOMEM, "dense_create: host alloc");
  h->device = device;
  h->n = n;
  h->d = d;
  h->cap_rows = n;
  hipError_t e = hipStreamCreateWithFlags(&h->stream, hipStreamNonBlocking);
  if (e == hipSuccess && n > 0) e = hipMalloc((void**)&h->X, (size_t)n * d * sizeof(float));
  if (e == hipSuccess && n > 0) e = hipMemcpy(h->X, X_host, (size_t)n * d * sizeof(float), hipMemcpyHostToDevice);
  if (e != hipSuccess) {
    amdr_dense_destroy(h);
    return fail(e == hipErrorOutOfMemory ? AMDR_ENOMEM : AMDR_EHIP, "dense_create: %s", hipGetErrorString(e));
  }
  if ((rc = update_stats(h, 0, n))) {
    amdr_dense_destroy(h);
    return rc;
  }
  *out = h;
  return AMDR_OK;
}

int amdr_dense_create_from_device(const float* X_dev, int64_t n, int32_t d, int32_t device, amdr_dense_t** out) {
  AMDR_REQUIRE(out != nullptr, "dense_create_from_device: out is null");
  *out = nullptr;
  AMDR_REQUIRE(n >= 0 && n < (1ll << 32), "dense_create_from_device: n=%lld outside [0, 2^32)", (long long)n);
  AMDR_REQUIRE(d >= 4 && d <= AMDR_MAX_DIM && d % 4 == 0, "dense_create_from_device: bad d=%d", d);
  AMDR_REQUIRE(n == 0 || X_dev != nullptr, "dense_create_from_device: X is null");
  AMDR_REQUIRE(((uintptr_t)X_dev & 15) == 0, "dense_create_from_device: X must be 16-byte aligned");
  int rc = check_device(device);
  if (rc) return rc;
  amdr_dense* h = new (std::nothrow) amdr_dense();
  if (!h) return fail(AMDR_ENOMEM, "dense_create_from_device: host alloc");
  h->device = device;
  h->n = n;
  h->d = d;
  h->cap_rows = n;
  h->X = const_cast<float*>(X_dev);
  h->owns = false;
  hipError_t e = hipStreamCreateWithFlags(&h->stream, hipStreamNonBlocking);
  if (e != hipSuccess) {
    amdr_dense_destroy(h);
    return fail(AMDR_EHIP, "dense_create_from_device: %s", hipGetErrorString(e));
  }
  AMDR_HIP(hipDeviceSynchronize());
  if ((rc = update_stats(h, 0, n))) {
    amdr_dense_destroy(h);
    return rc;
  }
  *out = h;
  return AMDR_OK;
}

int amdr_dense_add(amdr_dense_t* h, const float* X_host, int64_t n_add) {
  AMDR_REQUIRE(h != nullptr, "dense_add: null handle");
  AMDR_REQUIRE(h->owns, "dense_add: handle wraps caller-owned memory");
  AMDR_REQUIRE(n_add >= 0 && (n_add == 0 || X_host), "dense_add: bad arguments");
  AMDR_REQUIRE(h->n + n_add < (1ll << 32), "dense_add: too many rows");
  std::lock_guard<std::mutex> g(h->mu);
  AMDR_HIP(hipSetDevice(h->device));
  if (n_add == 0) return AMDR_OK;
  if (h->n + n_add > h->cap_rows) {
    int64_t ncap = h->cap_rows * 2 > h->n + n_add ? h->cap_rows * 2 : h->n + n_add;
    float* nx = nullptr;
    AMDR_HIP(hipMalloc((void**)&nx, (size_t)ncap * h->d * sizeof(float)));
    if (h->n > 0) AMDR_HIP(hipMemcpy(nx, h->X, (size_t)h->n * h->d * sizeof(float), hipMemcpyDeviceToDevice));
    if (h->X) (void)hipFree(h->X);
    h->X = nx;
    h->cap_rows = ncap;
  }
  AMDR_HIP(hipMemcpy(h->X + (size_t)h->n * h->d, X_host, (size_t)n_add * h->d * sizeof(float), hipMemcpyHostToDevice));
  const int64_t row0 = h->n;
  h->n += n_add;
  if (h->small) {
    (void)hipDeviceSynchronize();
    (void)amdr_dense_small_destroy(h->small);
    h->small = nullptr;
  }
  h->small_failed = false;
  h->hi_level = 0;
  h->hi_off = false;
  if (h->hi_copy_pending && hipEventSynchronize(h->hi_ev) == hipSuccess) {
    h->hi_copy_pending = false;
    for (int i = 0; i < 3; ++i) h->hi_seen[i] = h->hi_host[i];
  }
  h->lvl_f0 = h->hi_seen[1];
  h->lvl_p0 = (int64_t)h->hi_seen[2];
  return update_stats(h, row0, n_add);
}

int amdr_dense_ntotal(const amdr_dense_t* h, int64_t* n) {
  AMDR_REQUIRE(h && n, "dense_ntotal: null");
  *n = h->n;
  return AMDR_OK;
}
int amdr_dense_dim(const amdr_dense_t* h, int32_t* d) {
  AMDR_REQUIRE(h && d, "dense_dim: null");
  *d = h->d;
  return AMDR_OK;
}

int amdr_dense_reserve(amdr_dense_t* h, int32_t nq_max, int32_t k_max) {
  AMDR_REQUIRE(h != nullptr, "dense_reserve: null handle");
  AMDR_REQUIRE(nq_max >= 1 && k_max >= 1 && k_max <= AMDR_MAX_K, "dense_reserve: bad sizes");
  std::lock_guard<std::mutex> g(h->mu);
  AMDR_HIP(hipSetDevice(h->device));
  const DensePins pins = read_pins();
  int rc = ensure_need(h, 0, reserve_need(h, pins, nq_max, k_max));
  if (rc) return rc;
  if ((rc = h->qbuf.ensure((size_t)nq_max * h->d * sizeof(float)))) return rc;
  if ((rc = h->sbuf.ensure((size_t)nq_max * k_max * sizeof(float)))) return rc;
  if (small_hi_shape(h, pins, nq_max, k_max < 12 ? k_max : 12, 0))
    (void)small_hi_ready(h, batched_chunk(h, nq_max), nullptr);
  return h->ibuf.ensure((size_t)nq_max * k_max * sizeof(int64_t));
}

int amdr_dense_search_device(amdr_dense_t* h, const float* Q_dev, int32_t nq, int32_t k, float* scores_dev,
                             int64_t* ids_dev, void* stream) {
  int rc = check_search_args(h, Q_dev, nq, k, scores_dev, ids_dev);
  if (rc) return rc;
  if (nq == 0) return AMDR_OK;
  std::lock_guard<std::mutex> g(h->mu);
  AMDR_HIP(hipSetDevice(h->device));
  return run_search(h, 0, Q_dev, nq, k, scores_dev, ids_dev, (hipStream_t)stream);
}

int amdr_dense_search_fuse_device(amdr_dense_t* h, const float* Q_dev, int32_t nq, int32_t k,
                                  const amdr_fuse_params_t* p, const int64_t* dense_row2uid, const int64_t* bm25_ids,
                                  const double* bm25_scores, int32_t kb, const int64_t* bm25_row2uid,
                                  float* dense_scores_dev, int64_t* dense_ids_dev, int64_t* out_ids, double* out_vals,
                                  int32_t* out_mask, int32_t* out_count, void* stream) {
  int rc = check_search_args(h, Q_dev, nq, k, dense_scores_dev, dense_ids_dev);
  if (rc) return rc;
  AMDR_REQUIRE(p != nullptr, "dense_search_fuse: null params");
  AMDR_REQUIRE(p->method >= 0 && p->method <= AMDR_FUSE_WEIGHTED_SUM, "dense_search_fuse: method=%d", p->method);
  AMDR_REQUIRE(kb >= 0 && kb <= AMDR_MAX_K && (kb == 0 || (bm25_ids && bm25_scores)), "dense_search_fuse: bad BM25 lists");
  AMDR_REQUIRE(nq == 0 || (out_ids && out_vals && out_mask && out_count), "dense_search_fuse: null output");
  if (nq == 0) return AMDR_OK;
  std::lock_guard<std::mutex> g(h->mu);
  AMDR_HIP(hipSetDevice(h->device));
  FuseTail tail{p, dense_row2uid, bm25_ids, bm25_scores, kb, bm25_row2uid, out_ids, out_vals, out_mask, out_count};
  return run_search(h, 0, Q_dev, nq, k, dense_scores_dev, dense_ids_dev, (hipStream_t)stream, &tail);
}

int amdr_dense_search(amdr_dense_t* h, const float* Q_host, int32_t nq, int32_t k, float* scores_host,
                      int64_t* ids_host) {
  int rc = check_search_args(h, Q_host, nq, k, scores_host, ids_host);
  if (rc) return rc;
  if (nq == 0) return AMDR_OK;
  std::lock_guard<std::mutex> g(h->mu);
  AMDR_HIP(hipSetDevice(h->device));
  if ((rc = h->qbuf.ensure((size_t)nq * h->d * sizeof(float)))) return rc;
  if ((rc = h->sbuf.ensure((size_t)nq * k * sizeof(float)))) return rc;
  if ((rc = h->ibuf.ensure((size_t)nq * k * sizeof(int64_t)))) return rc;
  AMDR_HIP(hipMemcpyAsync(h->qbuf.p, Q_host, (size_t)nq * h->d * sizeof(float), hipMemcpyHostToDevice, h->stream));
  rc = run_search(h, 1, h->qbuf.as<float>(), nq, k, h->sbuf.as<float>(), h->ibuf.as<int64_t>(), h->stream);
  if (rc) return rc;
  AMDR_HIP(hipMemcpyAsync(scores_host, h->sbuf.p, (size_t)nq * k * sizeof(float), hipMemcpyDeviceToHost, h->stream));
  AMDR_HIP(hipMemcpyAsync(ids_host, h->ibuf.p, (size_t)nq * k * sizeof(int64_t), hipMemcpyDeviceToHost, h->stream));
  AMDR_HIP(hipStreamSynchronize(h->stream));
  return AMDR_OK;
}

int amdr_dense_score_rows(amdr_dense_t* h, const float* Q_host, int32_t nq, const int64_t* rows_host, int32_t m,
                          float* scores_host) {
  AMDR_REQUIRE(h != nullptr, "dense_score_rows: null handle");
  AMDR_REQUIRE(nq >= 0 && m >= 0, "dense_score_rows: bad sizes");
  if (nq == 0 || m == 0) return AMDR_OK;
  AMDR_REQUIRE(Q_host && rows_host && scores_host, "dense_score_rows: null buffer");
  std::lock_guard<std::mutex> g(h->mu);
  AMDR_HIP(hipSetDevice(h->device));
  int rc;
  const size_t cnt = (size_t)nq * m;
  if ((rc = h->qbuf.ensure((size_t)nq * h->d * sizeof(float)))) return rc;
  if ((rc = h->sbuf.ensure(cnt * sizeof(float)))) return rc;
  if ((rc = h->ibuf.ensure(cnt * sizeof(int64_t)))) return rc;
  AMDR_HIP(hipMemcpyAsync(h->qbuf.p, Q_host, (size_t)nq * h->d * sizeof(float), hipMemcpyHostToDevice, h->stream));
  AMDR_HIP(hipMemcpyAsync(h->ibuf.p, rows_host, cnt * sizeof(int64_t), hipMemcpyHostToDevice, h->stream));
  hipLaunchKernelGGL(dense_score_rows_kernel, dim3(ceil_div((long)cnt, kWaves)), dim3(256), 0, h->stream, h->X,
                     (long)h->n, h->d, h->qbuf.as<float>(), nq, h->ibuf.as<long long>(), m, h->sbuf.as<float>());
  AMDR_HIP(hipGetLastError());
  AMDR_HIP(hipMemcpyAsync(scores_host, h->sbuf.p, cnt * sizeof(float), hipMemcpyDeviceToHost, h->stream));
  AMDR_HIP(hipStreamSynchronize(h->stream));
  return AMDR_OK;
}

int amdr_dense_read_rows(const amdr_dense_t* h, int64_t row0, int64_t nrows, float* out_host) {
  AMDR_REQUIRE(h && out_host, "dense_read_rows: null");
  AMDR_REQUIRE(row0 >= 0 && nrows >= 0 && row0 + nrows <= h->n, "dense_read_rows: range outside [0,%lld)",
               (long long)h->n);
  AMDR_HIP(hipSetDevice(h->device));
  if (nrows)
    AMDR_HIP(hipMemcpy(out_host, h->X + (size_t)row0 * h->d, (size_t)nrows * h->d * sizeof(float),
                       hipMemcpyDeviceToHost));
  return AMDR_OK;
}

int amdr_dense_workspace_plan(int64_t n, int32_t d, int32_t nq_max, int32_t k_max, int32_t nq, int32_t k, int64_t* out6) {
  AMDR_REQUIRE(out6 != nullptr, "dense_workspace_plan: null");
  AMDR_REQUIRE(n >= 1 && n < (1ll << 32) && d >= 4 && d <= AMDR_MAX_DIM && d % 4 == 0, "dense_workspace_plan: bad shape");
  AMDR_REQUIRE(nq_max >= 1 && k_max >= 1 && k_max <= AMDR_MAX_K && nq >= 1 && k >= 1 && k <= AMDR_MAX_K,
               "dense_workspace_plan: bad sizes");
  amdr_dense h;
  h.n = n;
  h.d = d;
  h.hi_ok = dense_hi_supported(d);
  const DensePins pins = read_pins();
  const Need res = reserve_need(&h, pins, nq_max, k_max), used = call_need(&h, dense_route(&h, pins, nq, k), nq, k);
  out6[0] = (int64_t)res.smat, out6[1] = (int64_t)res.part, out6[2] = (int64_t)res.aux;
  out6[3] = (int64_t)used.smat, out6[4] = (int64_t)used.part, out6[5] = (int64_t)used.aux;
  return AMDR_OK;
}

int amdr_dense_plan_info(const amdr_dense_t* h, int32_t nq, int32_t k, char* buf, int32_t buf_len) {
  AMDR_REQUIRE(h && buf && buf_len > 0, "dense_plan_info: null");
  AMDR_REQUIRE(nq >= 1 && k >= 1 && k <= AMDR_MAX_K, "dense_plan_info: bad sizes");
  const DensePins pins = read_pins();
  const Route r = dense_route(h, pins, nq, k);
  const int m = r.chunk;
  if (h->n <= 0) {
    snprintf(buf, buf_len, "empty index");
  } else if (r.form == Form::Hi) {
    Hi2Plan p;
    hi2_plan(h, m, k, r.kc, &p);
    snprintf(buf, buf_len,
             "dense_hi_tilemax_kernel fp16 first pass queries_per_launch=%d scans_per_launch=%d (%d per scan, one tail): per-query lists of the "
             "approximate tile maxima above a sampled threshold (every %ld-th tile, width level %d) -> top-%d + rounding-bound "
             "check + exact re-scoring of each query's tiles at or above its cut (<= %d each) + top-k: 4 launches behind the "
             "scan(s), the exact first pass behind a device flag in 2",
             m, p.qtiles, m < dense_hi_max_queries(h->d) ? m : dense_hi_max_queries(h->d),
             dense_hi2_sample_stride((long)h->n, p.qtiles), r.hi_level, r.kc, r.kc);
  } else if (r.form == Form::TwoLevel) {
    TwoLevelPlan t;
    two_level_plan(h, m, k, &t);
    snprintf(buf, buf_len,
             "dense_mfma_scores_kernel tile-maxima grid=%dx%d queries_per_launch=%d two-level: top-%d of %ld tile maxima "
             "+ re-scoring of <= %d candidate tiles + top-k%s",
             t.scan.grid_x, t.scan.grid_y, m, k, t.tiles, m * k,
             r.hi ? " (fp16 first pass given up: too many unresolved queries)" : "");
  } else if (r.form != Form::Scan) {
    DenseMfmaPlan p;
    dense_mfma_plan((long)h->n, h->d, m, k, &p);
    const PassForm f = batched_pass_form(h, pins, r, p, m, k, nullptr);
    const char* tail = p.slabs == 1 ? "scores_slab_topk_kernel" : "scores_slab_topk_kernel + dense_merge_kernel";
    if (f.small_hi && !h->small_failed) {
      snprintf(buf, buf_len,
               "dsh_scores_kernel fp16 first pass queries_per_launch=%d (dsh_split_queries_kernel + v_mfma_f32_32x32x16_f16 on "
               "fp16 roundings of both operands, proven per-query bound) + dense_hi_select_fuse_kernel (rows inside 2 eps of the "
               "k-th best re-scored exactly, top-k, fusion); exact form: dense_panel_scores_kernel",
               m);
    } else if (f.scores == PassForm::RowWaves) {
      snprintf(buf, buf_len, "dense_all_scores_kernel (one wave per query x row) + %s", tail);
    } else if (f.scores == PassForm::Panel) {
      DensePanelPlan pp;
      dense_panel_plan((long)h->n, h->d, m, &pp);
      snprintf(buf, buf_len, "dense_panel_scores_kernel nb=%d parts=%d blocks=%d queries_per_launch=%d + %s", pp.nb,
               pp.parts, pp.m_tiles * pp.parts, m, tail);
    } else {
      snprintf(buf, buf_len, "dense_mfma_scores_kernel query-tiles-in-LDS grid=%dx%d queries_per_launch=%d + %s",
               p.grid_x, p.grid_y, m, tail);
    }
  } else {
    ScanPlan p;
    make_plan(h->n, h->d, nq, k, &p);
    snprintf(buf, buf_len, "dense_scan_topk_kernel<NQ=%d> grid=%dx%d%s", p.nq_per_block, p.grid_x, p.grid_y,
             p.grid_x == 1 ? "" : " + dense_merge_kernel");
  }
  return AMDR_OK;
}

int amdr_dense_hi_counters(amdr_dense_t* h, int64_t* out6) {
  AMDR_REQUIRE(h && out6, "dense_hi_counters: null");
  std::lock_guard<std::mutex> g(h->mu);
  AMDR_HIP(hipSetDevice(h->device));
  out6[0] = h->hi_queries;
  out6[1] = out6[5] = 0;
  if (h->stats.p) {
    unsigned int c[3] = {0, 0, 0};
    AMDR_HIP(hipDeviceSynchronize());
    AMDR_HIP(hipMemcpy(c, h->stats.as<unsigned int>() + 2, sizeof(c), hipMemcpyDeviceToHost));
    out6[1] = (int64_t)c[0];
    out6[5] = (int64_t)c[1];
  }
  const DensePins pins = read_pins();
  out6[2] = pins.hi_level >= 0 ? pins.hi_level : h->hi_level;
  out6[3] = h->hi_ok && !h->hi_off ? 1 : 0;
  out6[4] = h->hi_passes;
  return AMDR_OK;
}

int amdr_dense_profile_begin(amdr_dense_t* h, int32_t max_launches) {
  AMDR_REQUIRE(h != nullptr && max_launches >= 1 && max_launches <= (1 << 16), "dense_profile_begin: bad arguments");
  std::lock_guard<std::mutex> g(h->mu);
  AMDR_HIP(hipSetDevice(h->device));
  while (h->prof_ev.size() < (size_t)max_launches * 2) {
    hipEvent_t e;
    AMDR_HIP(hipEventCreate(&e));
    h->prof_ev.push_back(e);
  }
  h->prof_used = 0;
  h->prof_on = true;
  return AMDR_OK;
}

int amdr_dense_profile_end(amdr_dense_t* h, double* total_ms, int32_t* launches) {
  AMDR_REQUIRE(h && total_ms && launches, "dense_profile_end: null");
  std::lock_guard<std::mutex> g(h->mu);
  AMDR_HIP(hipSetDevice(h->device));
  h->prof_on = false;
  double tot = 0;
  for (int i = 0; i + 1 < h->prof_used; i += 2) {
    float ms = 0;
    AMDR_HIP(hipEventSynchronize(h->prof_ev[i + 1]));
    AMDR_HIP(hipEventElapsedTime(&ms, h->prof_ev[i], h->prof_ev[i + 1]));
    tot += ms;
  }
  *total_ms = tot;
  *launches = h->prof_used / 2;
  h->prof_used = 0;
  return AMDR_OK;
}

int amdr_dense_two_pass_fallbacks(amdr_dense_t* h, int64_t* out) {
  AMDR_REQUIRE(h && out, "dense_two_pass_fallbacks: null");
  *out = 0;
  std::lock_guard<std::mutex> g(h->mu);
  if (!h->small_fb.p) return AMDR_OK;
  AMDR_HIP(hipSetDevice(h->device));
  unsigned int v = 0;
  AMDR_HIP(hipMemcpy(&v, h->small_fb.p, sizeof(v), hipMemcpyDeviceToHost));
  *out = (int64_t)v;
  return AMDR_OK;
}

int amdr_dense_destroy(amdr_dense_t* h) {
  if (!h) return AMDR_OK;
  (void)hipSetDevice(h->device);
  for (hipEvent_t e : h->prof_ev) (void)hipEventDestroy(e);
  if (h->stream) {
    (void)hipStreamSynchronize(h->stream);
    (void)hipStreamDestroy(h->stream);
  }
  if (h->owns && h->X) (void)hipFree(h->X);
  for (int w = 0; w < 2; ++w) {
    h->part[w].release();
    h->smat[w].release();
    h->aux[w].release();
  }
  h->qbuf.release();
  h->sbuf.release();
  h->ibuf.release();
  h->stats.release();
  if (h->small) (void)amdr_dense_small_destroy(h->small);
  h->small_eps.release();
  h->small_fb.release();
  if (h->hi_host) (void)hipHostFree(h->hi_host);
  if (h->hi_ev) (void)hipEventDestroy(h->hi_ev);
  delete h;
  return AMDR_OK;
}

int amdr_merge_topk_f32_device(const float* scores, const int64_t* ids, int32_t n_parts, int32_t nq, int32_t k_in,
                               int32_t k_out, float* out_scores, int64_t* out_ids, int32_t device, void* stream) {
  AMDR_REQUIRE(scores && ids && out_scores && out_ids, "merge_topk: null buffer");
  AMDR_REQUIRE(n_parts >= 1 && nq >= 1 && k_in >= 1 && k_out >= 1 && k_out <= AMDR_MAX_K, "merge_topk: bad sizes");
  AMDR_HIP(hipSetDevice(device));
  return launch_merge_parts<float>(scores, ids, n_parts, nq, k_in, k_out, out_scores, out_ids, (hipStream_t)stream);
}
int amdr_merge_topk_f64_device(const double* scores, const int64_t* ids, int32_t n_parts, int32_t nq, int32_t k_in,
                               int32_t k_out, double* out_scores, int64_t* out_ids, int32_t device, void* stream) {
  AMDR_REQUIRE(scores && ids && out_scores && out_ids, "merge_topk: null buffer");
  AMDR_REQUIRE(n_parts >= 1 && nq >= 1 && k_in >= 1 && k_out >= 1 && k_out <= AMDR_MAX_K, "merge_topk: bad sizes");
  AMDR_HIP(hipSetDevice(device));
  return launch_merge_parts<double>(scores, ids, n_parts, nq, k_in, k_out, out_scores, out_ids, (hipStream_t)stream);
}

}
```

### legal-rag_amd/csrc/fuse.hip

```cpp
#include "bm25_core.hpp"
#include "common.hpp"
#include "dense_dot.hpp"
#include "topk.hpp"

#include <cfloat>
#include <cmath>
#include <cstdlib>
#include <cstring>
#include <vector>

namespace amdr {

constexpr int kFuseMax = 3 * AMDR_MAX_K;

__device__ __forceinline__ double wave_min(double v) { return wave_allmin_f64(v); }
__device__ __forceinline__ double wave_max(double v) { return wave_allmax_f64(v); }
__device__ __forceinline__ void lds_sync() {
  __builtin_amdgcn_fence(__ATOMIC_ACQ_REL, "wavefront");
  __builtin_amdgcn_wave_barrier();
}

struct ChanIn {
  const long long* ids;
  const void* scores;
  const long long* row2uid;
  int k;
  int is_f64;
};

__device__ __forceinline__ double chan_score(const ChanIn& c, int qi, int j) {
  size_t off = (size_t)qi * c.k + j;
  return c.is_f64 ? ((const double*)c.scores)[off] : (double)((const float*)c.scores)[off];
}
__device__ __forceinline__ long long chan_uid(const ChanIn& c, int qi, int j) {
  long long id = c.ids[(size_t)qi * c.k + j];
  if (id >= 0 && c.row2uid) id = c.row2uid[id];
  return id;
}

struct FuseCtx {
  double rmn, rmx;
  bool rdeg, wrrf;
  double w[3], lo[3], hi[3];
};
template <class ScoreAt>
__device__ __forceinline__ void fuse_eval(const amdr_fuse_params_t& P, const FuseCtx& X, double t, const int (&pos)[3],
                                          ScoreAt&& score_at, double (&val)[AMDR_FUSE_NVALS], int& mk) {
  const double rrf_norm = X.rdeg ? 0.0 : (t - X.rmn) / (X.rmx - X.rmn);
  double nrm[3], raw[3], wt[3];
  mk = 0;
#pragma unroll
  for (int c = 0; c < 3; ++c) {
    const int p = pos[c];
    nrm[c] = 0.0;
    raw[c] = 0.0;
    if (p >= 0) {
      mk |= (1 << c);
      const double s = score_at(c, p);
      nrm[c] = (X.hi[c] - X.lo[c] < 1e-12) ? 0.0 : (s - X.lo[c]) / (X.hi[c] - X.lo[c]);
      const double wc = X.wrrf ? X.w[c] : 1.0;
      raw[c] = wc * (1.0 / (double)(P.rrf_k + p + 1));
    }
    wt[c] = X.w[c] * nrm[c];
  }
  const double wsum = (wt[0] + wt[1]) + wt[2];
  double score, con[3] = {0.0, 0.0, 0.0};
  if (P.method == AMDR_FUSE_WEIGHTED_SUM) {
    score = wsum;
#pragma unroll
    for (int c = 0; c < 3; ++c) con[c] = wt[c];
  } else if (P.method == AMDR_FUSE_RRF || P.method == AMDR_FUSE_WRRF) {
    score = rrf_norm;
    const double mass = score;
    if (!(mass <= 0.0 || t <= 1e-18)) {
#pragma unroll
      for (int c = 0; c < 3; ++c)
        if (pos[c] >= 0) con[c] = mass * raw[c] / t;
    }
  } else {
    score = P.alpha * rrf_norm + (1.0 - P.alpha) * wsum;
#pragma unroll
    for (int c = 0; c < 3; ++c) con[c] = 0.0 + (1.0 - P.alpha) * wt[c];
    const double mass = P.alpha * rrf_norm;
    if (!(mass <= 0.0 || t <= 1e-18)) {
#pragma unroll
      for (int c = 0; c < 3; ++c)
        if (pos[c] >= 0) con[c] = con[c] + mass * raw[c] / t;
    }
  }
  val[AMDR_FV_SCORE] = score;
  val[AMDR_FV_RRF_NORM] = rrf_norm;
  val[AMDR_FV_WSUM] = wsum;
  val[AMDR_FV_NORM_DENSE] = nrm[0];
  val[AMDR_FV_NORM_BM25] = nrm[1];
  val[AMDR_FV_NORM_COLBERT] = nrm[2];
  val[AMDR_FV_CONTRIB_DENSE] = con[0];
  val[AMDR_FV_CONTRIB_BM25] = con[1];
  val[AMDR_FV_CONTRIB_COLBERT] = con[2];
}

__global__ __launch_bounds__(64) void fuse_kernel(amdr_fuse_params_t P, ChanIn c0, ChanIn c1, ChanIn c2, int max_out,
                                                  long long* __restrict__ out_ids, double* __restrict__ out_vals,
                                                  int* __restrict__ out_mask, int* __restrict__ out_count) {
  extern __shared__ __attribute__((aligned(16))) unsigned char fsm[];
  long long* uid = reinterpret_cast<long long*>(fsm);
  double* sc = reinterpret_cast<double*>(uid + max_out);
  double* tot = sc + max_out;
  int* pos0 = reinterpret_cast<int*>(tot + max_out);
  int* pos[3] = {pos0, pos0 + max_out, pos0 + 2 * max_out};
  const int lane = threadIdx.x;
  const int qi = blockIdx.x;
  const ChanIn ch[3] = {c0, c1, c2};
  const double w[3] = {P.w_dense, P.w_bm25, P.w_colbert};

  int n[3];
  double lo[3], hi[3];
#pragma unroll
  for (int c = 0; c < 3; ++c) {
    int cnt = 0;
    double mn = INFINITY, mx = -INFINITY;
    for (int j = lane; j < ch[c].k; j += 64) {
      if (ch[c].ids[(size_t)qi * ch[c].k + j] >= 0) {
        cnt++;
        double s = chan_score(ch[c], qi, j);
        mn = fmin(mn, s);
        mx = fmax(mx, s);
      }
    }
    n[c] = wave_allsum_i32(cnt);
    lo[c] = wave_min(mn);
    hi[c] = wave_max(mx);
  }

  int U = 0;
#pragma unroll
  for (int c = 0; c < 3; ++c) {
    const int U0 = U;
    for (int base = 0; base < n[c]; base += 64) {
      const int j = base + lane;
      const bool v = j < n[c];
      long long my = v ? chan_uid(ch[c], qi, j) : -1;
      int f = -1;
      if (v)
        for (int u = 0; u < U0; ++u)
          if (uid[u] == my) {
            f = u;
            break;
          }
      const bool isnew = v && f < 0;
      const unsigned long long m = __ballot(isnew);
      const unsigned long long lt = (lane == 0) ? 0ull : (m & (~0ull >> (64 - lane)));
      const int idx = isnew ? U + __popcll(lt) : f;
      if (isnew) {
        uid[idx] = my;
        pos[0][idx] = -1;
// ... 263 lines not shown
  kept = __popcll(__ballot(kept != 0) & seg_bits);
  if (live && sl == 0) out_count[qi] = kept;
}

template <int W>
__global__ __launch_bounds__(64) void fuse_packed_kernel(amdr_fuse_params_t P, ChanIn c0, ChanIn c1, ChanIn c2, int nq,
                                                         int max_out, long long* __restrict__ out_ids,
                                                         double* __restrict__ out_vals, int* __restrict__ out_mask,
                                                         int* __restrict__ out_count) {
  FusePre none;
  none.have[0] = none.have[1] = none.have[2] = false;
  fuse_packed_body<W, false>(P, c0, c1, c2, nq, max_out, out_ids, out_vals, out_mask, out_count, none, blockIdx.x * (64 / W));
}

__global__ __launch_bounds__(64) void dense_select_fuse_kernel(amdr_fuse_params_t P, const float* __restrict__ S,
                                                               long ldS, long n, int nq, int kd, int cap,
                                                               float* __restrict__ fin_scores,
                                                               long long* __restrict__ fin_ids, ChanIn c0, ChanIn c1,
                                                               int max_out, long long* __restrict__ out_ids,
                                                               double* __restrict__ out_vals, int* __restrict__ out_mask,
                                                               int* __restrict__ out_count) {
  extern __shared__ __attribute__((aligned(16))) unsigned char smem[];
  C32* buf = reinterpret_cast<C32*>(smem);
  const int lane = threadIdx.x, sl = lane & 31;
  const int q = 2 * blockIdx.x + (lane >> 5);
  const bool has_q = q < nq;
  FusePre pre;
  pre.have[0] = pre.have[1] = true;
  pre.have[2] = false;
  pre.id[1] = -1;
  pre.s[1] = 0.0;
  if (has_q && sl < c1.k) {
    pre.id[1] = c1.ids[(size_t)q * c1.k + sl];
    pre.s[1] = chan_score(c1, q, sl);
  }
  C32 out = C32::pad();
  int got = select_row_pair_any(S, ldS, n, q, has_q, kd, lane, buf, out);
  if (got < 0) {
    for (int hh = 0; hh < 2; ++hh) {
      const int qq = 2 * blockIdx.x + hh;
      if (qq >= nq) break;
      const float* row = S + (size_t)qq * ldS;
      WaveTopK<C32> tk;
      tk.init(buf, cap, kd);
      for (long base = 0; base < n; base += 64) {
        const long r = base + lane;
        const bool v = r < n;
        tk.push_lanes(v ? C32::make(row[r], (u32)r) : C32::pad(), v, lane);
      }
      tk.finalize(lane);
      if ((lane >> 5) == hh) {
        got = tk.cnt;
        out = sl < tk.cnt ? tk.buf[sl] : C32::pad();
      }
      wave_lds_fence();
    }
  }
  const bool v = sl < got;
  if (has_q && sl < kd) {
    fin_scores[(size_t)q * kd + sl] = v ? out.score() : -FLT_MAX;
    fin_ids[(size_t)q * kd + sl] = v ? out.id() : -1ll;
  }
  pre.id[0] = v ? out.id() : -1ll;
  pre.s[0] = v ? (double)out.score() : 0.0;
  ChanIn none;
  none.ids = nullptr;
  none.scores = nullptr;
  none.row2uid = nullptr;
  none.k = 0;
  none.is_f64 = 0;
  fuse_packed_body<32, true>(P, c0, c1, none, nq, max_out, out_ids, out_vals, out_mask, out_count, pre, blockIdx.x * 2);
}

template <int V>
__device__ __forceinline__ int select_row_pair_margin(const float* __restrict__ S, long ldS, long n, int q, bool has_q, int k,
                                                      float margin, int lane, C32* scratch, C32& out, int& need) {
  const float* row = S + (size_t)q * ldS;
  const int j = lane & 31;
  tk_v4f blk[V / 4];
#pragma unroll
  for (int u = 0; u < V / 4; ++u) {
    const long c0 = 128L * u + 4 * j;
    const tk_v4f z = {0.f, 0.f, 0.f, 0.f};
    blk[u] = (has_q && c0 < ldS) ? __builtin_nontemporal_load(reinterpret_cast<const tk_v4f*>(row + c0)) : z;
  }
  u32 sk[V];
#pragma unroll
  for (int u = 0; u < V / 4; ++u)
#pragma unroll
    for (int e = 0; e < 4; ++e) {
      const long r = 128L * u + 4 * j + e;
      sk[4 * u + e] = (has_q && r < n) ? ord32(blk[u][e]) : 0u;
    }
  K32 lb;
  lb.c = 0u;
#pragma unroll
  for (int v = 0; v < V; ++v) lb.c = sk[v] > lb.c ? sk[v] : lb.c;
  const K32 sorted_best = wave_sortN_desc<K32, 32>(lb, lane);
  const int kk = (k - 1 < 31 ? k - 1 : 31);
  auto half_lane = [&](int x, int pos) -> int {
    const int a = __builtin_amdgcn_readlane(x, pos), b = __builtin_amdgcn_readlane(x, 32 + pos);
    return (lane & 32) ? b : a;
  };
  const u32 T = (u32)half_lane((int)sorted_best.c, kk);
  auto gather = [&](u32 Te, C32& c) -> int {
    int mine = 0;
#pragma unroll
    for (int v = 0; v < V; ++v) mine += (sk[v] >= Te) ? 1 : 0;
    int incl = mine;
    incl += __builtin_amdgcn_update_dpp(0, incl, 0x111, 0xf, 0xf, false);
    incl += __builtin_amdgcn_update_dpp(0, incl, 0x112, 0xf, 0xf, false);
    incl += __builtin_amdgcn_update_dpp(0, incl, 0x114, 0xf, 0xf, false);
    incl += __builtin_amdgcn_update_dpp(0, incl, 0x118, 0xf, 0xf, false);
    incl += __builtin_amdgcn_update_dpp(0, incl, 0x142, 0xa, 0xf, false);
    const int cnt = half_lane(incl, 31);
    if (cnt > 32) return -1;
    int at = (lane & 32) + incl - mine;
#pragma unroll
    for (int v = 0; v < V; ++v) {
      if (sk[v] >= Te) {
        C32 e;
        e.c = ((u64)sk[v] << 32) | (u64)(0xffffffffu - (u32)(128 * (v >> 2) + 4 * j + (v & 3)));
        scratch[at++] = e;
      }
    }
    wave_lds_fence();
    c = (j < cnt) ? scratch[lane] : C32::pad();
    c = wave_sortN_desc<C32, 32>(c, lane);
    wave_lds_fence();
    return cnt;
  };
  const u32 Te1 = T > 1u ? T : 1u;
  C32 c;
  int cnt = gather(Te1, c);
  if (cnt < 0) return -1;
  u32 cut = 1u;
  if (cnt > kk) {
    const float tk_f = __int_as_float(half_lane(__float_as_int(c.score()), kk));
    cut = ord32(tk_f - margin);
    cut = cut > 1u ? cut : 1u;
  }
  if (cut < Te1) {
    cnt = gather(cut, c);
    if (cnt < 0) return -1;
    need = cnt;
  } else {
    const unsigned long long m = __ballot(j < cnt && (u32)(c.c >> 32) >= cut);
    need = __popcll((lane & 32) ? (m >> 32) : (m & 0xffffffffull));
  }
  out = c;
  return cnt;
}

template <bool FUSE, int D128>
__global__ __launch_bounds__(64) void dense_hi_select_fuse_kernel(amdr_fuse_params_t P, const float* __restrict__ S, long ldS, long n,
                                                                  int nq, int kd, const float* __restrict__ X,
                                                                  const float* __restrict__ Q, int d,
                                                                  const float* __restrict__ eps, float margin_scale,
                                                                  float* __restrict__ fin_scores, long long* __restrict__ fin_ids,
                                                                  ChanIn c0, ChanIn c1, int max_out,
                                                                  long long* __restrict__ out_ids, double* __restrict__ out_vals,
                                                                  int* __restrict__ out_mask, int* __restrict__ out_count,
                                                                  unsigned int* __restrict__ fallbacks) {
  extern __shared__ __attribute__((aligned(16))) unsigned char smem[];
  C32* buf = reinterpret_cast<C32*>(smem);
  const int lane = threadIdx.x, sl = lane & 31, half = lane >> 5;
  const int q = 2 * blockIdx.x + half;
  const bool has_q = q < nq;
  FusePre pre;
  pre.have[0] = pre.have[1] = true;
  pre.have[2] = false;
  pre.id[1] = -1;
  pre.s[1] = 0.0;
  if (FUSE && has_q && sl < c1.k) {
    pre.id[1] = c1.ids[(size_t)q * c1.k + sl];
    pre.s[1] = chan_score(c1, q, sl);
  }
  const float e_q = has_q ? eps[q] : 0.f;
  const float margin = 2.f * e_q * margin_scale;
  bool exact_all = has_q && !(margin == margin && margin <= FLT_MAX);
  tk_v4f qv[D128];
#pragma unroll
  for (int u = 0; u < D128; ++u) {
    const tk_v4f z = {0.f, 0.f, 0.f, 0.f};
    qv[u] = has_q ? __builtin_nontemporal_load(reinterpret_cast<const tk_v4f*>(Q + (size_t)q * d + 128 * u + 4 * sl)) : z;
  }
  auto half_sum = [&](float v) -> float {
    v = dpp_add<0x111, 0xf>(v);
    v = dpp_add<0x112, 0xf>(v);
    v = dpp_add<0x114, 0xf>(v);
    v = dpp_add<0x118, 0xf>(v);
    v = dpp_add<0x142, 0xa>(v);
    const float s0 = __int_as_float(__builtin_amdgcn_readlane(__float_as_int(v), 31));
    const float s1 = __int_as_float(__builtin_amdgcn_readlane(__float_as_int(v), 63));
    return half ? s1 : s0;
  };
  auto row_load = [&](long r, tk_v4f (&xv)[D128]) {
    const float* xr = X + (size_t)r * d + 4 * sl;
#pragma unroll
    for (int u = 0; u < D128; ++u) xv[u] = *reinterpret_cast<const tk_v4f*>(xr + 128 * u);
  };
  auto row_fma = [&](const tk_v4f (&xv)[D128]) -> float {
    float acc = 0.f;
#pragma unroll
    for (int u = 0; u < D128; ++u)
#pragma unroll
      for (int e = 0; e < 4; ++e) acc = fmaf(xv[u][e], qv[u][e], acc);
    return half_sum(acc);
  };
  auto row_dot = [&](long r) -> float {
    tk_v4f xv[D128];
    row_load(r, xv);
    return row_fma(xv);
  };
  C32 out = C32::pad();
  int need = 0, got = 0;
  {
    const float mg = (has_q && !exact_all) ? margin : 0.f;
    if (n <= 256)
      got = select_row_pair_margin<8>(S, ldS, n, q, has_q, kd, mg, lane, buf, out, need);
    else if (n <= 512)
      got = select_row_pair_margin<16>(S, ldS, n, q, has_q, kd, mg, lane, buf, out, need);
    else if (n <= 640)
      got = select_row_pair_margin<20>(S, ldS, n, q, has_q, kd, mg, lane, buf, out, need);
    else
      got = select_row_pair_margin<32>(S, ldS, n, q, has_q, kd, mg, lane, buf, out, need);
    exact_all = exact_all || (has_q && got < 0);
    if (exact_all) need = 0;
  }
  if (__any(exact_all)) {
    const unsigned long long fbm = __ballot(exact_all && sl == 0);
    if (lane == 0 && fallbacks) atomicAdd(fallbacks, (unsigned int)__popcll(fbm));
    const C32 keep = out;
    const int keep_need = need, keep_got = got;
    float* xs = const_cast<float*>(S);
    for (long r = 0; r < n; ++r) {
      const float v = row_dot(r);
      if (exact_all && sl == 0) xs[(size_t)q * ldS + r] = v;
    }
    __threadfence_block();
    C32 o2 = C32::pad();
    int g2 = select_row_pair_any(xs, ldS, n, q, has_q && exact_all, kd, lane, buf, o2);
    if (g2 < 0) {
      for (int hh = 0; hh < 2; ++hh) {
        const int qq = 2 * blockIdx.x + hh;
        const bool mine_h = __shfl((int)exact_all, 32 * hh) != 0;
        if (qq >= nq || !mine_h) continue;
        const float* row = xs + (size_t)qq * ldS;
        WaveTopK<C32> tk;
        tk.init(buf, 128, kd);
        for (long base = 0; base < n; base += 64) {
          const long r = base + lane;
          const bool v = r < n;
          tk.push_lanes(v ? C32::make(row[r], (u32)r) : C32::pad(), v, lane);
        }
        tk.finalize(lane);
        if (half == hh) {
          g2 = tk.cnt;
          o2 = sl < tk.cnt ? tk.buf[sl] : C32::pad();
        }
        wave_lds_fence();
      }
    }
    if (exact_all) {
      out = o2;
      got = g2 < kd ? g2 : kd;
      need = 0;
    } else {
      out = keep;
      got = keep_got;
      need = keep_need;
    }
  }
  const int steps = __builtin_amdgcn_readfirstlane(max(__shfl(need, 0), __shfl(need, 32)));
  float mine_exact = 0.f;
  const int my_id = (int)out.id();
  for (int c = 0; c < steps; c += 2) {
    const int c1 = c + 1 < 32 ? c + 1 : 31;
    const int ra0 = __builtin_amdgcn_readlane(my_id, c), ra1 = __builtin_amdgcn_readlane(my_id, 32 + c);
    const int rb0 = __builtin_amdgcn_readlane(my_id, c1), rb1 = __builtin_amdgcn_readlane(my_id, 32 + c1);
    const bool la = c < need, lb = c + 1 < need;
    tk_v4f xa[D128], xb[D128];
    row_load(la ? (long)(half ? ra1 : ra0) : 0, xa);
    row_load(lb ? (long)(half ? rb1 : rb0) : 0, xb);
    const float va = row_fma(xa), vb = row_fma(xb);
    if (la && sl == c) mine_exact = va;
    if (lb && sl == c + 1) mine_exact = vb;
  }
  if (need > 0) {
    C32 c = (sl < need) ? C32::make(mine_exact, (u32)out.id()) : C32::pad();
    c = wave_sortN_desc<C32, 32>(c, lane);
    out = c;
    got = need < kd ? need : kd;
  }
  const bool v = sl < got && sl < kd;
  if (has_q && sl < kd) {
    fin_scores[(size_t)q * kd + sl] = v ? out.score() : -FLT_MAX;
    fin_ids[(size_t)q * kd + sl] = v ? out.id() : -1ll;
  }
  if (FUSE) {
    pre.id[0] = v ? out.id() : -1ll;
    pre.s[0] = v ? (double)out.score() : 0.0;
    ChanIn none;
    none.ids = nullptr;
    none.scores = nullptr;
    none.row2uid = nullptr;
    none.k = 0;
    none.is_f64 = 0;
    fuse_packed_body<32, true>(P, c0, c1, none, nq, max_out, out_ids, out_vals, out_mask, out_count, pre, blockIdx.x * 2);
  }
}

struct SmallArgs {
  const long long* term_ptr;
  const int* post_doc;
  const double* post_w;
  const double* idf;
  long n_terms, n_docs;
  const int* q_terms;
  const long long* q_ptr;
  int kb, cap, slab, use_select;
  double* bm_scores;
  long long* bm_ids;
  const float* X;
  const float* Q;
  long n_rows;
  int d, rows_per_block, blocks_per_query;
  float* S;
  long ldS;
  int kd, cap_sel;
  float* d_scores;
  long long* d_ids;
  int* ticket;
};

__device__ __forceinline__ int small_arrive(int* counter, int lane) {
  asm volatile("s_waitcnt vmcnt(0)" ::: "memory");
  int t = 0;
  if (lane == 0) {
    __builtin_amdgcn_fence(__ATOMIC_RELEASE, "agent");
    asm volatile("s_waitcnt vmcnt(0)" ::: "memory");
    t = __hip_atomic_fetch_add(counter, 1, __ATOMIC_RELAXED, __HIP_MEMORY_SCOPE_AGENT);
  }
  return __builtin_amdgcn_readfirstlane(t);
}
__device__ __forceinline__ void small_acquire(int* counter, int lane) {
  if (lane == 0) __hip_atomic_store(counter, 0, __ATOMIC_RELAXED, __HIP_MEMORY_SCOPE_AGENT);
  __builtin_amdgcn_fence(__ATOMIC_ACQUIRE, "agent");
  asm volatile("s_waitcnt vmcnt(0)" ::: "memory");
}

template <int NVT>
__global__ __launch_bounds__(256) void hybrid_small_kernel(SmallArgs A, amdr_fuse_params_t P, ChanIn c0, ChanIn c1, int nq,
                                                           int max_out, long long* __restrict__ out_ids,
                                                           double* __restrict__ out_vals, int* __restrict__ out_mask,
                                                           int* __restrict__ out_count) {
  extern __shared__ __attribute__((aligned(16))) unsigned char smem[];
  const int q = blockIdx.y, role = blockIdx.x;
  const int lane = threadIdx.x & 63, wave = threadIdx.x >> 6;
  int* rows_done = A.ticket + q;
  int* lists_done = A.ticket + 32 + q;
  const int sl = lane & 31;
  FusePre pre;
  pre.have[0] = pre.have[1] = true;
  pre.have[2] = false;
  bool have_dense = false;
  if (role == 0) {
    if (wave != 0) return;
    bm25_block_query<1, NVT>(A.term_ptr, A.post_doc, A.post_w, A.idf, A.n_terms, A.n_docs, A.q_terms, A.q_ptr, nq, A.kb,
                             A.cap, A.slab, A.use_select, nullptr, nullptr, A.bm_scores, A.bm_ids, q, 0, smem);
  } else {
    const long r0 = (long)(role - 1) * A.rows_per_block;
    long r1 = r0 + A.rows_per_block;
    if (r1 > A.n_rows) r1 = A.n_rows;
    for (long r = r0 + wave; r < r1; r += 4) {
      const float acc = dense_row_dot(A.X + (size_t)r * A.d, A.Q + (size_t)q * A.d, A.d, lane);
      if (lane == 63) A.S[(size_t)q * A.ldS + r] = acc;
    }
    asm volatile("s_waitcnt vmcnt(0)" ::: "memory");
    __syncthreads();
    if (wave != 0) return;
    if (small_arrive(rows_done, lane) != A.blocks_per_query - 2) return;
    small_acquire(rows_done, lane);
    C32* buf = reinterpret_cast<C32*>(smem);
    const float* row = A.S + (size_t)q * A.ldS;
    const long n = A.n_rows;
    WaveTopK<C32> tk;
    tk.init(buf, A.cap_sel, A.kd);
    int got;
    if (n <= 256)
      got = select_row<4>(row, 0, n, A.kd, lane, tk.buf);
    else if (n <= 640)
      got = select_row<10>(row, 0, n, A.kd, lane, tk.buf);
    else if (n <= 1024)
      got = select_row<16>(row, 0, n, A.kd, lane, tk.buf);
    else if (n <= 1280)
      got = select_row<20>(row, 0, n, A.kd, lane, tk.buf);
    else
      got = select_row<32>(row, 0, n, A.kd, lane, tk.buf);
    if (got >= 0) {
      tk.cnt = got;
    } else {
      for (long base = 0; base < n; base += 64) {
        const long r = base + lane;
        const bool v = r < n;
        tk.push_lanes(v ? C32::make(row[r], (u32)r) : C32::pad(), v, lane);
      }
      tk.finalize(lane);
    }
    wave_lds_fence();
    const bool v = lane < 32 && sl < tk.cnt;
    const C32 mine = v ? tk.buf[sl] : C32::pad();
    if (lane < A.kd) {
      A.d_scores[(size_t)q * A.kd + lane] = v ? mine.score() : -FLT_MAX;
      A.d_ids[(size_t)q * A.kd + lane] = v ? mine.id() : -1ll;
    }
    pre.id[0] = v ? mine.id() : -1ll;
    pre.s[0] = v ? (double)mine.score() : 0.0;
    have_dense = true;
    wave_lds_fence();
  }
  if (small_arrive(lists_done, lane) != 1) return;
  small_acquire(lists_done, lane);
  if (!have_dense) {
    pre.id[0] = -1;
    pre.s[0] = 0.0;
    if (lane < 32 && sl < A.kd) {
      const long long id = A.d_ids[(size_t)q * A.kd + sl];
      pre.id[0] = id;
      pre.s[0] = id >= 0 ? (double)A.d_scores[(size_t)q * A.kd + sl] : 0.0;
    }
  }
  pre.id[1] = -1;
  pre.s[1] = 0.0;
  if (lane < 32 && sl < c1.k) {
    pre.id[1] = c1.ids[(size_t)q * c1.k + sl];
    pre.s[1] = chan_score(c1, q, sl);
  }
  ChanIn none;
  none.ids = nullptr;
  none.scores = nullptr;
  none.row2uid = nullptr;
  none.k = 0;
  none.is_f64 = 0;
  fuse_packed_body<32, true>(P, c0, c1, none, q + 1, max_out, out_ids, out_vals, out_mask, out_count, pre, q);
}

static void launch_fuse(const amdr_fuse_params_t& P, const ChanIn& c0, const ChanIn& c1, const ChanIn& c2, int nq,
                        int max_out, long long* ids, double* vals, int* mask, int* count, hipStream_t st) {
  if (max_out <= 16)
    hipLaunchKernelGGL(fuse_packed_kernel<16>, dim3((nq + 3) / 4), dim3(64), 0, st, P, c0, c1, c2, nq, max_out, ids, vals,
                       mask, count);
  else if (max_out <= 32)
    hipLaunchKernelGGL(fuse_packed_kernel<32>, dim3((nq + 1) / 2), dim3(64), 0, st, P, c0, c1, c2, nq, max_out, ids, vals,
                       mask, count);
  else
    hipLaunchKernelGGL(fuse_kernel, dim3(nq), dim3(64), (size_t)max_out * 36, st, P, c0, c1, c2, max_out, ids, vals, mask,
                       count);
}

__global__ __launch_bounds__(64) void rerank_blend_kernel(int max_out, const int* __restrict__ count,
                                                          long long* __restrict__ ids, double* __restrict__ vals,
                                                          int* __restrict__ mask, const double* __restrict__ ce_raw,
                                                          int top_n, double beta, double* __restrict__ out_rerank) {
  extern __shared__ __attribute__((aligned(16))) unsigned char smem[];
  double* svals = reinterpret_cast<double*>(smem);
  double* snew = svals + (size_t)max_out * AMDR_FUSE_NVALS;
  double* snorm = snew + max_out;
  long long* sids = reinterpret_cast<long long*>(snorm + max_out);
  int* smask = reinterpret_cast<int*>(sids + max_out);
  int* spre = smask + max_out;
  const int lane = threadIdx.x, qi = blockIdx.x;
  const size_t base = (size_t)qi * max_out;
  const int cnt = count[qi];
  const int n = cnt < top_n ? cnt : top_n;
  const double nan = __longlong_as_double(0x7ff8000000000000ll);

  for (int r = lane; r < max_out; r += 64) {
    out_rerank[(base + r) * 2 + 0] = nan;
    out_rerank[(base + r) * 2 + 1] = nan;
  }
  if (n <= 0) return;

  double mn = INFINITY, mx = -INFINITY;
  for (int j = lane; j < n; j += 64) {
    double r = ce_raw[(size_t)qi * top_n + j];
    mn = fmin(mn, r);
    mx = fmax(mx, r);
  }
  mn = wave_min(mn);
  mx = wave_max(mx);
  const bool deg = (mx - mn < 1e-12);

  for (int j = lane; j < cnt; j += 64) {
    for (int x = 0; x < AMDR_FUSE_NVALS; ++x) svals[(size_t)j * AMDR_FUSE_NVALS + x] = vals[(base + j) * AMDR_FUSE_NVALS + x];
    sids[j] = ids[base + j];
    smask[j] = mask[base + j];
    double s = svals[(size_t)j * AMDR_FUSE_NVALS + AMDR_FV_SCORE];
    if (j < n) {
      double raw = ce_raw[(size_t)qi * top_n + j];
      double nm = deg ? 0.0 : (raw - mn) / (mx - mn);
      snorm[j] = nm;
      s = (1 - beta) * s + beta * nm;
    }
    snew[j] = s;
  }
  lds_sync();
  for (int j = lane; j < cnt; j += 64) {
    int p = j;
    if (j < n) {
      const double nm = snorm[j];
      p = 0;
      for (int i = 0; i < n; ++i) {
        const double o = snorm[i];
        p += (o > nm) || (o == nm && i < j);
      }
    }
    spre[j] = p;
  }
  lds_sync();
  for (int j = lane; j < cnt; j += 64) {
    const double s = snew[j];
    const int pj = spre[j];
    int r = 0;
    for (int i = 0; i < cnt; ++i) {
      const double o = snew[i];
      r += (o > s) || (o == s && spre[i] < pj);
    }
    ids[base + r] = sids[j];
    mask[base + r] = smask[j];
    for (int x = 0; x < AMDR_FUSE_NVALS; ++x) vals[(base + r) * AMDR_FUSE_NVALS + x] = svals[(size_t)j * AMDR_FUSE_NVALS + x];
    vals[(base + r) * AMDR_FUSE_NVALS + AMDR_FV_SCORE] = s;
    if (j < n) {
      out_rerank[(base + r) * 2 + 0] = ce_raw[(size_t)qi * top_n + j];
      out_rerank[(base + r) * 2 + 1] = snorm[j];
    }
  }
}

static size_t rerank_lds(int max_out) {
  return (size_t)max_out * (AMDR_FUSE_NVALS + 2) * sizeof(double) + (size_t)max_out * sizeof(long long) +
         (size_t)max_out * 2 * sizeof(int);
}

bool dense_select_fuse_applies(long n, int slabs, int m, int kd, int kb) {
  const char* e = getenv("AMDR_DENSE_FUSE");
  if (e && e[0] == '0') return false;
  return slabs == 1 && n >= 1 && n <= 1024 && kd >= 1 && kd <= 32 && kb >= 0 && kd + kb <= 32 && m >= 1;
}

int dense_select_fuse_launch(const FuseTail& t, int q0, const float* S, long ldS, long n, int m, int kd, int cap,
                             float* fin_scores, int64_t* fin_ids, hipStream_t st) {
  const int mo = kd + t.kb;
  ChanIn c0{nullptr, nullptr, (const long long*)t.dense_row2uid, kd, 0};
  ChanIn c1{(const long long*)(t.kb ? t.bm25_ids + (size_t)q0 * t.kb : nullptr),
            t.kb ? (const void*)(t.bm25_scores + (size_t)q0 * t.kb) : nullptr, (const long long*)t.bm25_row2uid, t.kb, 1};
  hipLaunchKernelGGL(dense_select_fuse_kernel, dim3((m + 1) / 2), dim3(64), (size_t)cap * sizeof(C32), st, *t.p, S, ldS, n,
                     m, kd, cap, fin_scores, (long long*)fin_ids, c0, c1, mo, (long long*)(t.out_ids + (size_t)q0 * mo),
                     t.out_vals + (size_t)q0 * mo * AMDR_FUSE_NVALS, t.out_mask + (size_t)q0 * mo, t.out_count + q0);
  AMDR_HIP(hipGetLastError());
  return AMDR_OK;
}

int dense_hi_select_launch(const FuseTail* t, int q0, const float* S, long ldS, long n, int m, int kd, const float* X,
                           const float* Q, int d, const float* eps, float* fin_scores, int64_t* fin_ids,
                           unsigned int* fallbacks, hipStream_t st) {
  const char* ms = getenv("AMDR_DENSE_SMALL_HI_MARGIN");
  const float margin_scale = ms ? (float)atof(ms) : 1.f;
  const size_t lds = 128 * sizeof(C32);
  if (t) {
    const int mo = kd + t->kb;
    ChanIn c0{nullptr, nullptr, (const long long*)t->dense_row2uid, kd, 0};
    ChanIn c1{(const long long*)(t->kb ? t->bm25_ids + (size_t)q0 * t->kb : nullptr),
              t->kb ? (const void*)(t->bm25_scores + (size_t)q0 * t->kb) : nullptr, (const long long*)t->bm25_row2uid, t->kb, 1};
#define AMDR_HSF_FUSED(D)                                                                                                  \
  hipLaunchKernelGGL((dense_hi_select_fuse_kernel<true, D>), dim3((m + 1) / 2), dim3(64), lds, st, *t->p, S, ldS, n, m, kd, X, \
                     Q, d, eps, margin_scale, fin_scores, (long long*)fin_ids, c0, c1, mo,                                 \
                     (long long*)(t->out_ids + (size_t)q0 * mo), t->out_vals + (size_t)q0 * mo * AMDR_FUSE_NVALS,          \
                     t->out_mask + (size_t)q0 * mo, t->out_count + q0, fallbacks)
    switch (d >> 7) {
      case 1: AMDR_HSF_FUSED(1); break;
      case 2: AMDR_HSF_FUSED(2); break;
      case 3: AMDR_HSF_FUSED(3); break;
      case 4: AMDR_HSF_FUSED(4); break;
      case 5: AMDR_HSF_FUSED(5); break;
      case 6: AMDR_HSF_FUSED(6); break;
      case 7: AMDR_HSF_FUSED(7); break;
      default: AMDR_HSF_FUSED(8); break;
    }
#undef AMDR_HSF_FUSED
  } else {
    amdr_fuse_params_t P{};
    ChanIn none{nullptr, nullptr, nullptr, 0, 0};
#define AMDR_HSF_PLAIN(D)                                                                                                   \
  hipLaunchKernelGGL((dense_hi_select_fuse_kernel<false, D>), dim3((m + 1) / 2), dim3(64), lds, st, P, S, ldS, n, m, kd, X, Q, \
                     d, eps, margin_scale, fin_scores, (long long*)fin_ids, none, none, 0, (long long*)nullptr,             \
                     (double*)nullptr, (int*)nullptr, (int*)nullptr, fallbacks)
    switch (d >> 7) {
      case 1: AMDR_HSF_PLAIN(1); break;
      case 2: AMDR_HSF_PLAIN(2); break;
      case 3: AMDR_HSF_PLAIN(3); break;
      case 4: AMDR_HSF_PLAIN(4); break;
      case 5: AMDR_HSF_PLAIN(5); break;
      case 6: AMDR_HSF_PLAIN(6); break;
      case 7: AMDR_HSF_PLAIN(7); break;
      default: AMDR_HSF_PLAIN(8); break;
    }
#undef AMDR_HSF_PLAIN
  }
  AMDR_HIP(hipGetLastError());
  return AMDR_OK;
}

int dense_fuse_plain_launch(const FuseTail& t, int q0, int m, int kd, const float* dense_scores, const int64_t* dense_ids,
                            hipStream_t st) {
  const int mo = kd + t.kb;
  ChanIn c0{(const long long*)dense_ids, dense_scores, (const long long*)t.dense_row2uid, kd, 0};
  ChanIn c1{(const long long*)(t.kb ? t.bm25_ids + (size_t)q0 * t.kb : nullptr),
            t.kb ? (const void*)(t.bm25_scores + (size_t)q0 * t.kb) : nullptr, (const long long*)t.bm25_row2uid, t.kb, 1};
  ChanIn c2{nullptr, nullptr, nullptr, 0, 0};
  launch_fuse(*t.p, c0, c1, c2, m, mo, (long long*)(t.out_ids + (size_t)q0 * mo),
              t.out_vals + (size_t)q0 * mo * AMDR_FUSE_NVALS, t.out_mask + (size_t)q0 * mo, t.out_count + q0, st);
  AMDR_HIP(hipGetLastError());
  return AMDR_OK;
}

bool hybrid_small_applies(long n_dense, long n_bm25, int nslabs, int nq, int kd, int kb) {
  const char* e = getenv("AMDR_HYBRID_SMALL");
  if (e && e[0] == '0') return false;
  return nq >= 1 && nq <= 4 && n_dense >= 1 && n_dense <= kSelectRowsMax && n_bm25 >= 1 && nslabs == 1 && kd >= 1 && kb >= 1 &&
         kd + kb <= 32;
}

static int hybrid_small_rows(long n, int nq) {
  static const int pinned = [] {
    const char* e = getenv("AMDR_HYBRID_SMALL_ROWS");
    int r = e ? atoi(e) : 0;
    if (r <= 0) return 0;
    if (r < 4) r = 4;
    if (r > 64) r = 64;
    return (r + 3) / 4 * 4;
  }();
  if (pinned) return pinned;
  return n * nq <= 2560 ? 16 : 32;
}

int hybrid_small_launch(const DenseRaw& dr, const Bm25Raw& br, const float* Q, const int* q_terms, const long long* q_ptr,
                        int nq, int kd, int kb, const amdr_fuse_params_t& P, const int64_t* dense_row2uid,
                        const int64_t* bm25_row2uid, float* dense_scores, int64_t* dense_ids, double* bm25_scores,
                        int64_t* bm25_ids, int64_t* out_ids, double* out_vals, int32_t* out_mask, int32_t* out_count,
                        hipStream_t st) {
  SmallArgs A;
  A.term_ptr = br.term_ptr;
  A.post_doc = br.post_doc;
  A.post_w = br.post_w;
  A.idf = br.idf;
  A.n_terms = br.n_terms;
  A.n_docs = br.n_docs;
  A.q_terms = q_terms;
  A.q_ptr = q_ptr;
  A.kb = kb;
  A.cap = br.cap;
  A.slab = br.slab;
  A.use_select = br.select_on ? 1 : 0;
  A.bm_scores = bm25_scores;
  A.bm_ids = (long long*)bm25_ids;
  A.X = dr.X;
  A.Q = Q;
  A.d = dr.d;
  A.n_rows = dr.n;
  A.rows_per_block = hybrid_small_rows(dr.n, nq);
  const int dense_blocks = (int)((dr.n + A.rows_per_block - 1) / A.rows_per_block);
  A.blocks_per_query = 1 + dense_blocks;
  A.S = dr.S;
  A.ldS = dr.ld;
  A.kd = kd;
  int cap_sel = topk_cap(kd);
  if (cap_sel < 128) cap_sel = 128;
  A.cap_sel = cap_sel;
  A.d_scores = dense_scores;
  A.d_ids = (long long*)dense_ids;
  A.ticket = br.ticket;
  size_t lds = br.lds;
  if (lds < (size_t)cap_sel * sizeof(C32)) lds = (size_t)cap_sel * sizeof(C32);
  const int mo = kd + kb;
  ChanIn c0{nullptr, nullptr, (const long long*)dense_row2uid, kd, 0};
  ChanIn c1{(const long long*)bm25_ids, (const void*)bm25_scores, (const long long*)bm25_row2uid, kb, 1};
#define AMDR_HS_LAUNCH(NVT)                                                                                        \
  hipLaunchKernelGGL((hybrid_small_kernel<NVT>), dim3(A.blocks_per_query, nq), dim3(256), lds, st, A, P, c0, c1, nq, mo, \
                     (long long*)out_ids, out_vals, out_mask, out_count)
  const int nv = br.nvt;
  if (nv <= 4) AMDR_HS_LAUNCH(4);
  else if (nv <= 8) AMDR_HS_LAUNCH(8);
  else if (nv <= 10) AMDR_HS_LAUNCH(10);
  else if (nv <= 16) AMDR_HS_LAUNCH(16);
  else if (nv <= 20) AMDR_HS_LAUNCH(20);
  else AMDR_HS_LAUNCH(32);
#undef AMDR_HS_LAUNCH
  AMDR_HIP(hipGetLastError());
  return AMDR_OK;
}

}

using namespace amdr;

namespace {

int fuse_check(const amdr_fuse_params_t* p, int nq, int kd, int kb, int kc) {
  AMDR_REQUIRE(p != nullptr, "fuse: null params");
  AMDR_REQUIRE(p->method >= 0 && p->method <= 3, "fuse: unknown method %d", p->method);
  AMDR_REQUIRE(nq >= 0, "fuse: nq=%d", nq);
  AMDR_REQUIRE(kd >= 0 && kd <= AMDR_MAX_K && kb >= 0 && kb <= AMDR_MAX_K && kc >= 0 && kc <= AMDR_MAX_K,
               "fuse: channel depth outside [0,%d]", AMDR_MAX_K);
  AMDR_REQUIRE(kd + kb + kc >= 1, "fuse: all channels empty (max_out would be 0)");
  return AMDR_OK;
}

}

namespace {
struct Arena {
  char* base = nullptr;
  size_t cap = 0, used = 0;
  int device = -1;
  ~Arena() {
    if (base) (void)hipFree(base);
  }
  int begin(int dev, size_t total) {
    if (dev != device || total > cap) {
      if (base) (void)hipFree(base);
      base = nullptr;
      cap = 0;
      size_t want = total < (1u << 20) ? (1u << 20) : total;
      AMDR_HIP(hipMalloc((void**)&base, want));
      cap = want;
      device = dev;
    }
    used = 0;
    return AMDR_OK;
  }
  void* take(size_t bytes) {
    void* p = base + used;
    used += (bytes + 255) & ~(size_t)255;
    return p;
  }
};
inline size_t pad256(size_t b) { return (b + 255) & ~(size_t)255; }
Arena& arena() {
  static thread_local Arena a;
  return a;
}
}

namespace {
struct Pack {
  std::vector<char>& buf;
  size_t used = 0;
  explicit Pack(std::vector<char>& b) : buf(b) {}
  size_t add(const void* src, size_t bytes) {
    size_t off = used;
    used += pad256(bytes);
// ... 202 lines not shown
```

### legal-rag_amd/retrieval/engine.py

```python
from __future__ import annotations

from dataclasses import dataclass
from typing import Optional

import os

import numpy as np
import torch

from .. import _native


@dataclass
class BatchResult:
    ids: torch.Tensor
    vals: torch.Tensor
    mask: torch.Tensor
    count: torch.Tensor
    dense_ids: Optional[torch.Tensor] = None
    dense_scores: Optional[torch.Tensor] = None
    bm25_ids: Optional[torch.Tensor] = None
    bm25_scores: Optional[torch.Tensor] = None
    colbert_ids: Optional[torch.Tensor] = None
    colbert_scores: Optional[torch.Tensor] = None
# ... 113 lines not shown
        nq, mo = res.ids.shape
        w = max(1, min(int(w), int(mo)))
        o1 = nq * w * 8
        o2 = o1 + nq * w * 8
        o3 = o2 + nq * w * 4
        tot = o3 + nq * 4
        pk = self._buf("cpk", (tot,), torch.uint8)
        base = pk.data_ptr()
        _native.fuse_compact_device(nq, mo, w, res.ids.data_ptr(), res.vals.data_ptr(), res.mask.data_ptr(),
                                    res.count.data_ptr(), base, base + o1, base + o2, base + o3, device=self.device,
                                    stream=_stream())
        host = self._pinned("cpkh", tot)
        host[:tot].copy_(pk, non_blocking=True)
        torch.cuda.current_stream(self.tdev).synchronize()
        h = host.numpy()
        return (h[:o1].view("int64").reshape(nq, w).copy(), h[o1:o2].view("float64").reshape(nq, w).copy(),
                h[o2:o3].view("int32").reshape(nq, w).copy(), h[o3:tot].view("int32").copy())

    def reserve(self, nq: int, k: int, total_terms: int = 0, bytes_max: int = 0) -> None:
        if bytes_max > 0 and self.tokenizer is not None:
            self.tokenizer.reserve(nq, bytes_max)
            total_terms = max(total_terms, bytes_max)
        if self.dense is not None:
            self.dense.reserve(nq, k)
        if self.bm25 is not None:
            self.bm25.reserve(nq, k, max(total_terms, 1))
        if self.maxsim is not None:
            self.maxsim.reserve(nq, k)
        if self.graph is not None and self.graph_limit > 0:
            self.graph.reserve(nq, k, self.graph_limit)

    def set_graph(self, graph: _native.GraphIndex, params: dict, lang: int = -1) -> None:
        import numpy as np
        key = (id(graph), int(params["limit"]), int(params["default_depth"]), float(params["min_conf"]), int(lang),
               params["rel_max_depth"].tobytes(), params["rel_allowed"].tobytes(), params["rel_weight"].tobytes(),
               params["decay"].tobytes())
        if self.graph is graph and self._graph_key == key:
            return
        tabs = tuple(torch.from_numpy(np.ascontiguousarray(params[n])).to(self.tdev)
                     for n in ("rel_max_depth", "rel_allowed", "rel_weight", "decay"))
        torch.cuda.current_stream(self.tdev).synchronize()
        self.graph, self._graph_tabs, self._graph_key = graph, tabs, key
        self.graph_limit = int(params["limit"])
        self.graph_params = _native.GraphParams(int(params["limit"]), int(params["default_depth"]), int(lang), 0,
                                                float(params["min_conf"]), *(t.data_ptr() for t in tabs))

    def graph_topk(self, seeds: torch.Tensor, seed_count: torch.Tensor, q_emb: torch.Tensor, k: int, seed_n: int,
                   qsel: Optional[torch.Tensor] = None) -> dict:
        if self.graph is None or self.graph_params is None:
            raise RuntimeError("graph_topk: this engine has no graph channel (set_graph)")
        assert seeds.is_cuda and seeds.dtype == torch.int64 and seeds.is_contiguous() and seed_count.dtype == torch.int32
        assert q_emb.is_cuda and q_emb.dtype == torch.float32 and q_emb.is_contiguous()
        ld = int(seeds.shape[1])
        ng = int(qsel.numel()) if qsel is not None else int(seeds.shape[0])
        if qsel is not None:
            assert qsel.is_cuda and qsel.dtype == torch.int32 and qsel.is_contiguous()
        k = int(k)
        outs = {n: self._buf("g_" + n, (ng,) if n == "count" else (ng, k), getattr(torch, np.dtype(t).name))
                for n, t in zip(_native.GraphIndex.OUTS, _native.GraphIndex._OUT_T)}
        self.graph.search_device(self.dense, q_emb.data_ptr(), qsel.data_ptr() if qsel is not None else 0,
                                 seeds.data_ptr(), seed_count.data_ptr(), ld, min(int(seed_n), ld, _native.GRAPH_MAX_SEEDS),
                                 ng, k, self.graph_params, [outs[n].data_ptr() for n in _native.GraphIndex.OUTS], _stream())
        return outs

    def dense_topk(self, q_emb: torch.Tensor, k: int):
        nq = q_emb.shape[0]
        assert q_emb.is_cuda and q_emb.dtype == torch.float32 and q_emb.is_contiguous()
        s = self._buf("ds", (nq, k), torch.float32)
        i = self._buf("di", (nq, k), torch.int64)
        self.dense.search_device(q_emb.data_ptr(), nq, k, s.data_ptr(), i.data_ptr(), _stream())
        return s, i

    def bm25_topk(self, q_terms: torch.Tensor, q_ptr: torch.Tensor, k: int):
        nq = q_ptr.shape[0] - 1
        assert q_terms.dtype == torch.int32 and q_ptr.dtype == torch.int64 and q_terms.is_cuda and q_ptr.is_cuda
        s = self._buf("bs", (nq, k), torch.float64)
        i = self._buf("bi", (nq, k), torch.int64)
        self.bm25.search_device(q_terms.data_ptr(), q_ptr.data_ptr(), nq, k, s.data_ptr(), i.data_ptr(), _stream())
        return s, i

    def colbert_topk(self, q_tok: torch.Tensor, k: int):
        nq, q_len = q_tok.shape[0], q_tok.shape[1]
        assert q_tok.is_cuda and q_tok.dtype == torch.float32 and q_tok.is_contiguous()
        s = self._buf("cs", (nq, k), torch.float32)
        i = self._buf("ci", (nq, k), torch.int64)
        self.maxsim.search_device(q_tok.data_ptr(), nq, q_len, k, s.data_ptr(), i.data_ptr(), _stream())
        return s, i

    def fuse(self, params: _native.FuseParams, nq: int, dense=None, bm25=None, colbert=None) -> BatchResult:
        def chan(c, m):
            if c is None:
                return None, 0
            s, i = c
            return (i.data_ptr(), s.data_ptr(), int(i.shape[1]), m.data_ptr() if m is not None else 0), int(i.shape[1])
        d, kd = chan(dense, self.maps[0])
        b, kb = chan(bm25, self.maps[1])
        c, kc = chan(colbert, self.maps[2])
        mo = kd + kb + kc
        pk, ids, vals, mask, count = self._fused_outputs(nq, mo)
        _native.fuse_device(params, nq, d, b, c, ids.data_ptr(), vals.data_ptr(), mask.data_ptr(), count.data_ptr(),
                            device=self.device, stream=_stream())
        return BatchResult(ids=ids, vals=vals, mask=mask, count=count, packed=pk)

    def _fused_outputs(self, nq: int, mo: int):
        o1 = nq * mo * 8
        o2 = o1 + nq * mo * _native.FUSE_NVALS * 8
        o3 = o2 + nq * mo * 4
        pk = self._buf("fpk", (o3 + nq * 4,), torch.uint8)
        return (pk, pk[:o1].view(torch.int64).view(nq, mo), pk[o1:o2].view(torch.float64).view(nq, mo, _native.FUSE_NVALS),
                pk[o2:o3].view(torch.int32).view(nq, mo), pk[o3:].view(torch.int32))

    def dense_topk_fuse(self, params: _native.FuseParams, q_emb: torch.Tensor, k: int, bm25):
        nq = q_emb.shape[0]
        assert q_emb.is_cuda and q_emb.dtype == torch.float32 and q_emb.is_contiguous()
        bs, bi = bm25
        kb = int(bi.shape[1])
        s = self._buf("ds", (nq, k), torch.float32)
        i = self._buf("di", (nq, k), torch.int64)
        pk, ids, vals, mask, count = self._fused_outputs(nq, k + kb)
        m0, m1 = self.maps[0], self.maps[1]
        self.dense.search_fuse_device(params, q_emb.data_ptr(), nq, k,
                                      (bi.data_ptr(), bs.data_ptr(), kb, m1.data_ptr() if m1 is not None else 0),
                                      m0.data_ptr() if m0 is not None else 0, s.data_ptr(), i.data_ptr(), ids.data_ptr(),
                                      vals.data_ptr(), mask.data_ptr(), count.data_ptr(), _stream())
        return (s, i), BatchResult(ids=ids, vals=vals, mask=mask, count=count, packed=pk)

    def _hybrid_small(self, params: _native.FuseParams, q_emb: torch.Tensor, q_terms: torch.Tensor, q_ptr: torch.Tensor,
                      k: int) -> BatchResult:
        nq = int(q_emb.shape[0])
        assert q_emb.is_cuda and q_emb.dtype == torch.float32 and q_emb.is_contiguous()
        assert q_terms.dtype == torch.int32 and q_ptr.dtype == torch.int64 and q_terms.is_cuda and q_ptr.is_cuda
        assert q_ptr.shape[0] - 1 == nq
        ent = self._xcache.get(("hs", nq, k))
        if ent is None:
            ds = self._buf("ds", (nq, k), torch.float32)
            di = self._buf("di", (nq, k), torch.int64)
            bs = self._buf("bs", (nq, k), torch.float64)
            bi = self._buf("bi", (nq, k), torch.int64)
            pk, ids, vals, mask, count = self._fused_outputs(nq, 2 * k)
            m0, m1 = self.maps[0], self.maps[1]
            plan = _native.hybrid_small_plan(self.dense, self.bm25, nq, k, k, m0.data_ptr() if m0 is not None else 0,
                                             m1.data_ptr() if m1 is not None else 0, ds.data_ptr(), di.data_ptr(),
                                             bs.data_ptr(), bi.data_ptr(), ids.data_ptr(), vals.data_ptr(), mask.data_ptr(),
                                             count.data_ptr())
            ent = (plan, (ids, vals, mask, count, pk), (ds, di, bs, bi))
            self._xcache[("hs", nq, k)] = ent
        plan, (ids, vals, mask, count, pk), (ds, di, bs, bi) = ent
        _native.hybrid_small_device(plan, params, q_emb.data_ptr(), q_terms.data_ptr(), q_ptr.data_ptr(), _stream())
        res = BatchResult(ids=ids, vals=vals, mask=mask, count=count, packed=pk)
        res.dense_scores, res.dense_ids = ds, di
        res.bm25_scores, res.bm25_ids = bs, bi
        return res

    def rerank_blend(self, res: BatchResult, ce_raw: torch.Tensor, beta: float) -> BatchResult:
        nq, mo = res.ids.shape
        assert ce_raw.is_cuda and ce_raw.dtype == torch.float64 and ce_raw.is_contiguous() and ce_raw.shape[0] == nq
        out = self._buf("fr", (nq, mo, 2), torch.float64)
        _native.rerank_blend_device(nq, mo, res.count.data_ptr(), res.ids.data_ptr(), res.vals.data_ptr(),
                                    res.mask.data_ptr(), ce_raw.data_ptr(), int(ce_raw.shape[1]), float(beta),
                                    out.data_ptr(), device=self.device, stream=_stream())
        res.rerank = out
        return res

    def search_batch(self, params: _native.FuseParams, k: int, *, q_emb: Optional[torch.Tensor] = None,
                     q_terms: Optional[torch.Tensor] = None, q_ptr: Optional[torch.Tensor] = None,
                     q_tok: Optional[torch.Tensor] = None, q_text=None) -> BatchResult:
        if q_text is not None:
            if q_terms is not None or q_ptr is not None:
                raise ValueError("search_batch: pass q_text or q_terms / q_ptr, not both")
            q_terms, q_ptr, flags = self.tokenize_device(*q_text)
            res = self.search_batch(params, k, q_emb=q_emb, q_terms=q_terms, q_ptr=q_ptr, q_tok=q_tok)
            res.needs_segmenter = flags
            return res
        d = b = c = None
        nq = None
        if (self.dense is not None and q_emb is not None and self.bm25 is not None and q_ptr is not None
                and not (self.maxsim is not None and q_tok is not None) and self.shard_offset is None):
            nq = int(q_emb.shape[0])
            if nq <= 4 and 2 * k <= 32:
                return self._hybrid_small(params, q_emb, q_terms, q_ptr, k)
            b = self.bm25_topk(q_terms, q_ptr, k)
            d, res = self.dense_topk_fuse(params, q_emb, k, b)
            res.dense_scores, res.dense_ids = d
            res.bm25_scores, res.bm25_ids = b
            return res
        with_col = self.maxsim is not None and q_tok is not None
        overlap = (with_col and os.environ.get("AMDR_ENGINE_OVERLAP", "1") != "0"
                   and ((self.dense is not None and q_emb is not None) or (self.bm25 is not None and q_ptr is not None)))
        if overlap:
            main = torch.cuda.current_stream(self.tdev)
            side = self.__dict__.get("_side_stream")
            if side is None:
                side = self.__dict__["_side_stream"] = torch.cuda.Stream(device=self.tdev)
            side.wait_stream(main)
            with torch.cuda.stream(side):
                if self.dense is not None and q_emb is not None:
                    d = self.dense_topk(q_emb, k)
                if self.bm25 is not None and q_ptr is not None:
                    b = self.bm25_topk(q_terms, q_ptr, k)
            c = self.colbert_topk(q_tok, k)
            main.wait_stream(side)
            nq = q_tok.shape[0]
        else:
            if self.dense is not None and q_emb is not None:
                d = self.dense_topk(q_emb, k)
                nq = q_emb.shape[0]
            if self.bm25 is not None and q_ptr is not None:
                b = self.bm25_topk(q_terms, q_ptr, k)
                nq = q_ptr.shape[0] - 1
            if with_col:
                c = self.colbert_topk(q_tok, k)
                nq = q_tok.shape[0]
        if self.shard_offset is not None:
            from . import sharding
            chans = [x for x in (d, b, c) if x is not None]
            merged = iter(sharding.exchange_topk(chans, int(self.shard_offset), group=self.shard_group, buf=self._buf,
                                                 cache=self._xcache))
            d, b, c = (next(merged) if x is not None else None for x in (d, b, c))
        res = self.fuse(params, nq, d, b, c)
        if d is not None:
            res.dense_scores, res.dense_ids = d
        if b is not None:
            res.bm25_scores, res.bm25_ids = b
        if c is not None:
            res.colbert_scores, res.colbert_ids = c
        return res

    def capture(self, params: _native.FuseParams, k: int, *, q_emb: Optional[torch.Tensor] = None,
                q_terms: Optional[torch.Tensor] = None, q_ptr: Optional[torch.Tensor] = None,
                q_tok: Optional[torch.Tensor] = None, q_text=None, graph: Optional[dict] = None):
        if self.shard_offset is not None:
            raise RuntimeError("capture: a sharded step contains a collective; it is not recorded into a hipGraph")
        if q_text is not None:
            nq = int(q_text[1].numel()) - 1
            self.reserve(nq, int(k), 0, bytes_max=max(int(q_text[0].numel()), 1))
        else:
            nq = (q_emb.shape[0] if q_emb is not None else q_ptr.shape[0] - 1 if q_ptr is not None else q_tok.shape[0])
            self.reserve(int(nq), int(k), int(q_terms.numel()) if q_terms is not None else 0)
        gstage = graph
        if gstage is not None:
            ng = int(gstage["qsel"].numel()) if gstage.get("qsel") is not None else int(nq)
            self.graph.reserve(ng, int(gstage["k"]), self.graph_limit)

        def step():
            r = self.search_batch(params, k, q_emb=q_emb, q_terms=q_terms, q_ptr=q_ptr, q_tok=q_tok, q_text=q_text)
            if gstage is not None:
                r.graph = self.graph_topk(r.ids, r.count, gstage["q_emb"], gstage["k"], gstage["seed_n"],
                                          qsel=gstage.get("qsel"))
            return r
        side = torch.cuda.Stream(device=self.tdev)
        side.wait_stream(torch.cuda.current_stream(self.tdev))
        with torch.cuda.stream(side):
            step()
        side.synchronize()
        graph = torch.cuda.CUDAGraph()
        with torch.cuda.graph(graph):
            res = step()
        return graph, res
```

Measured before the change: 155.9 million queries/s.

## Fuse BM25 top-k into the dense two-pass select-and-fuse kernel for long batches

Adds a hybrid_long path: for batches of more than four queries, BM25 top-k runs in a second wave of the same block that does the dense high-precision re-score and fusion. This removes the separate BM25 search launch and the round trip of BM25 results through global memory before fusion. The fused path applies only when the dense route is the batched two-pass fp16 form with a single BM25 slab and a matching template instance. Otherwise it falls back to the old path. The cost is extra LDS per block and two waves per block, which may lower occupancy.

Result: slower. 138.7 million queries/s (-11.0%).

```diff
diff --git a/include/amdretrieval.h b/include/amdretrieval.h
--- a/include/amdretrieval.h
+++ b/include/amdretrieval.h
@@ -149,6 +149,26 @@
                              const int64_t* dense_row2uid, const int64_t* bm25_row2uid, float* dense_scores_dev,
                              int64_t* dense_ids_dev, double* bm25_scores_dev, int64_t* bm25_ids_dev, int64_t* out_ids,
                              double* out_vals, int32_t* out_mask, int32_t* out_count, void* stream);
+
+typedef struct amdr_hybrid_long_args {
+  const float* Q_dev;
+  const int32_t* q_terms_dev;
+  const int64_t* q_ptr_dev;
+  int32_t nq, kd, kb, reserved;
+  const amdr_fuse_params_t* p;
+  const int64_t* dense_row2uid;
+  const int64_t* bm25_row2uid;
+  float* dense_scores_dev;
+  int64_t* dense_ids_dev;
+  double* bm25_scores_dev;
+  int64_t* bm25_ids_dev;
+  int64_t* out_ids;
+  double* out_vals;
+  int32_t* out_mask;
+  int32_t* out_count;
+} amdr_hybrid_long_args_t;
+int amdr_hybrid_long_device(amdr_dense_t* dense, amdr_bm25_t* bm25, const amdr_hybrid_long_args_t* a, int32_t* applied,
+                            void* stream);
 
 int amdr_dense_two_pass_fallbacks(amdr_dense_t* h, int64_t* out);
 int amdr_dense_small_create(amdr_dense_t* dense, amdr_dense_small_t** out);
diff --git a/legal-rag_amd/_native.py b/legal-rag_amd/_native.py
--- a/legal-rag_amd/_native.py
+++ b/legal-rag_amd/_native.py
@@ -21,7 +21,7 @@
 EXPORTS = (
     "amdr_last_error", "amdr_version", "amdr_device_count", "amdr_device_name", "amdr_workspace_growths",
     "amdr_dense_create", "amdr_dense_create_from_device", "amdr_dense_add", "amdr_dense_ntotal", "amdr_dense_dim",
-    "amdr_dense_reserve", "amdr_dense_search", "amdr_dense_search_device", "amdr_dense_search_fuse_device", "amdr_hybrid_small_device", "amdr_dense_small_create", "amdr_dense_small_approx_device", "amdr_dense_small_destroy", "amdr_dense_two_pass_fallbacks", "amdr_dense_read_rows", "amdr_dense_score_rows",
+    "amdr_dense_reserve", "amdr_dense_search", "amdr_dense_search_device", "amdr_dense_search_fuse_device", "amdr_hybrid_small_device", "amdr_hybrid_long_device", "amdr_dense_small_create", "amdr_dense_small_approx_device", "amdr_dense_small_destroy", "amdr_dense_two_pass_fallbacks", "amdr_dense_read_rows", "amdr_dense_score_rows",
     "amdr_dense_plan_info", "amdr_dense_workspace_plan", "amdr_dense_hi_counters", "amdr_dense_profile_begin", "amdr_dense_profile_end", "amdr_dense_destroy",
     "amdr_bm25_create", "amdr_bm25_ndocs", "amdr_bm25_reserve", "amdr_bm25_workspace_plan", "amdr_bm25_plan_info", "amdr_bm25_search", "amdr_bm25_search_device",
     "amdr_bm25_scores", "amdr_bm25_destroy",
@@ -42,7 +42,7 @@
     "amdr_last_error": "", "amdr_version": "", "amdr_device_count": "P", "amdr_device_name": "iPi", "amdr_workspace_growths": "P",
     "amdr_dense_create": "PliiP", "amdr_dense_create_from_device": "PliiP", "amdr_dense_add": "PPl",
     "amdr_dense_ntotal": "PP", "amdr_dense_dim": "PP", "amdr_dense_reserve": "Pii", "amdr_dense_search": "PPiiPP",
-    "amdr_dense_search_device": "PPiiPPP", "amdr_dense_search_fuse_device": "PPiiPPPPiPPPPPPPP", "amdr_hybrid_small_device": "PPPPPiiiPPPPPPPPPPPP", "amdr_dense_small_create": "PP", "amdr_dense_small_approx_device": "PPiPlPP", "amdr_dense_small_destroy": "P", "amdr_dense_two_pass_fallbacks": "PP", "amdr_dense_read_rows": "PllP", "amdr_dense_score_rows": "PPiPiP",
+    "amdr_dense_search_device": "PPiiPPP", "amdr_dense_search_fuse_device": "PPiiPPPPiPPPPPPPP", "amdr_hybrid_small_device": "PPPPPiiiPPPPPPPPPPPP", "amdr_hybrid_long_device": "PPPPP", "amdr_dense_small_create": "PP", "amdr_dense_small_approx_device": "PPiPlPP", "amdr_dense_small_destroy": "P", "amdr_dense_two_pass_fallbacks": "PP", "amdr_dense_read_rows": "PllP", "amdr_dense_score_rows": "PPiPiP",
     "amdr_dense_plan_info": "PiiPi", "amdr_dense_workspace_plan": "liiiiiP", "amdr_dense_hi_counters": "PP", "amdr_dense_profile_begin": "Pi", "amdr_dense_profile_end": "PPP", "amdr_dense_destroy": "P",
     "amdr_bm25_create": "PPPPPlldddiP", "amdr_bm25_ndocs": "PP", "amdr_bm25_reserve": "Piil", "amdr_bm25_workspace_plan": "liiiiP", "amdr_bm25_plan_info": "PiiPi",
     "amdr_bm25_search": "PPPiiPP", "amdr_bm25_search_device": "PPPiiPPP", "amdr_bm25_scores": "PPPiP",
@@ -73,6 +73,14 @@
 class FuseParams(C.Structure):
     _fields_ = [("method", C.c_int32), ("rrf_k", C.c_int32), ("alpha", C.c_double), ("w_dense", C.c_double),
                 ("w_bm25", C.c_double), ("w_colbert", C.c_double), ("min_final_score", C.c_double)]
+
+
+class HybridLongArgs(C.Structure):
+    _fields_ = [("Q_dev", C.c_void_p), ("q_terms_dev", C.c_void_p), ("q_ptr_dev", C.c_void_p), ("nq", C.c_int32),
+                ("kd", C.c_int32), ("kb", C.c_int32), ("reserved", C.c_int32), ("p", C.c_void_p),
+                ("dense_row2uid", C.c_void_p), ("bm25_row2uid", C.c_void_p), ("dense_scores_dev", C.c_void_p),
+                ("dense_ids_dev", C.c_void_p), ("bm25_scores_dev", C.c_void_p), ("bm25_ids_dev", C.c_void_p),
+                ("out_ids", C.c_void_p), ("out_vals", C.c_void_p), ("out_mask", C.c_void_p), ("out_count", C.c_void_p)]
 
 
 class ShardChan(C.Structure):
@@ -793,6 +801,15 @@
             pass
 
 
+def hybrid_long_device(dense: "DenseIndex", bm25: "BM25Index", params: "FuseParams", args: "HybridLongArgs",
+                       stream: int = 0) -> bool:
+    args.p = C.cast(C.pointer(params), C.c_void_p)
+    applied = C.c_int32(0)
+    _check(load().amdr_hybrid_long_device(dense._h, bm25._h, C.byref(args), C.byref(applied), _vp(stream)),
+           "amdr_hybrid_long_device")
+    return bool(applied.value)
+
+
 def hybrid_small_plan(dense: "DenseIndex", bm25: "BM25Index", nq: int, kd: int, kb: int, dense_row2uid: int,
                       bm25_row2uid: int, dense_scores: int, dense_ids: int, bm25_scores: int, bm25_ids: int, out_ids: int,
                       out_vals: int, out_mask: int, out_count: int):
diff --git a/legal-rag_amd/csrc/bm25.hip b/legal-rag_amd/csrc/bm25.hip
--- a/legal-rag_amd/csrc/bm25.hip
+++ b/legal-rag_amd/csrc/bm25.hip
@@ -10,6 +10,7 @@
 
 
 #include "bm25_core.hpp"
+#include "hybrid_long.hpp"
 
 using namespace amdr;
 
@@ -136,6 +137,7 @@
   return AMDR_OK;
 }
 std::mutex& bm25_mutex(amdr_bm25_t* h) { return h->mu; }
+int bm25_device_of(const amdr_bm25_t* h) { return h->device; }
 }
 namespace {
 
diff --git a/legal-rag_amd/csrc/bm25_core.hpp b/legal-rag_amd/csrc/bm25_core.hpp
--- a/legal-rag_amd/csrc/bm25_core.hpp
+++ b/legal-rag_amd/csrc/bm25_core.hpp
@@ -182,12 +182,17 @@
 }
 
 __device__ __forceinline__ void bm25_all_zero_result(int m, int k, long lo, int lane, size_t row, double* fin_scores,
-                                                     long long* fin_ids, C64* part_row) {
+                                                     long long* fin_ids, C64* part_row, double* hand_scores = nullptr,
+                                                     long long* hand_ids = nullptr) {
   for (int j = lane; j < k; j += 64) {
     const bool v = j < m;
     if (fin_ids) {
       fin_scores[row * k + j] = v ? 0.0 : -DBL_MAX;
       fin_ids[row * k + j] = v ? lo + j : -1ll;
+      if (hand_ids) {
+        hand_scores[j] = v ? 0.0 : -DBL_MAX;
+        hand_ids[j] = v ? lo + j : -1ll;
+      }
     } else {
       part_row[j] = v ? C64::make(0.0, lo + j) : C64::pad();
     }
@@ -216,7 +221,7 @@
     const long long* __restrict__ q_ptr, int nq, int k, int cap, int slab, int use_select,
     double* __restrict__ scores_out , C64* __restrict__ part ,
     double* __restrict__ fin_scores , long long* __restrict__ fin_ids,
-    int qi_arg, int slab_ix, unsigned char* smem) {
+    int qi_arg, int slab_ix, int tid, unsigned char* smem, double* hand_scores = nullptr, long long* hand_ids = nullptr) {
   double* sc = reinterpret_cast<double*>(smem);
   C64* lists = reinterpret_cast<C64*>(sc + slab);
   int* cnts = reinterpret_cast<int*>(lists + (size_t)WAVES * cap);
@@ -226,7 +231,7 @@
   int* tk_n = reinterpret_cast<int*>(tk_ps + 128);
   constexpr int NT = WAVES * 64;
 
-  const int tid = threadIdx.x, lane = tid & 63, wave = tid >> 6;
+  const int lane = tid & 63, wave = tid >> 6;
   const int qi = qi_arg;
   const long lo = (long)slab_ix * slab;
   long hi = lo + slab;
@@ -326,7 +331,7 @@
   if (nt_total == 0) {
     if (wave == 0)
       bm25_all_zero_result(m, k, lo, lane, (size_t)qi, fin_scores, fin_ids,
-                           part ? part + ((size_t)slab_ix * nq + qi) * k : nullptr);
+                           part ? part + ((size_t)slab_ix * nq + qi) * k : nullptr, hand_scores, hand_ids);
     return;
   }
 #if defined(AMDR_BM_ABL) && AMDR_BM_ABL == 3
@@ -363,6 +368,10 @@
         bool v = j < tk.cnt;
         fin_scores[(size_t)qi * k + j] = v ? unord64(tk.buf[j].key) : -DBL_MAX;
         fin_ids[(size_t)qi * k + j] = v ? tk.buf[j].idv : -1ll;
+        if (hand_ids) {
+          hand_scores[j] = v ? unord64(tk.buf[j].key) : -DBL_MAX;
+          hand_ids[j] = v ? tk.buf[j].idv : -1ll;
+        }
       }
     } else {
       C64* dst = part + ((size_t)slab_ix * nq + qi) * k;
@@ -380,7 +389,7 @@
     double* __restrict__ fin_scores , long long* __restrict__ fin_ids) {
   extern __shared__ __attribute__((aligned(16))) unsigned char smem[];
   bm25_block_query<WAVES, NVT>(term_ptr, post_doc, post_w, idf, n_terms, n_docs, q_terms, q_ptr, nq, k, cap, slab, use_select, scores_out, part, fin_scores, fin_ids,
-                               (int)blockIdx.y, (int)blockIdx.x, smem);
+                               (int)blockIdx.y, (int)blockIdx.x, (int)threadIdx.x, smem);
 }
 
 static __global__ __launch_bounds__(256) void bm25_merge_kernel(const C64* __restrict__ part, int nparts, int nq, int k,
diff --git a/legal-rag_amd/csrc/dense.hip b/legal-rag_amd/csrc/dense.hip
--- a/legal-rag_amd/csrc/dense.hip
+++ b/legal-rag_amd/csrc/dense.hip
@@ -1,4 +1,5 @@
 #include "common.hpp"
+#include "hybrid_long.hpp"
 #include "dense_dot.hpp"
 #include "topk.hpp"
 
@@ -629,7 +630,7 @@
 }
 
 int run_search_batched(amdr_dense* h, int ws, const DensePins& pins, const Route& r, const float* Q_dev, int nq, int k,
-                       float* scores_dev, int64_t* ids_dev, hipStream_t st, const FuseTail* tail) {
+                       float* scores_dev, int64_t* ids_dev, hipStream_t st, const FuseTail* tail, const LongBmJob* bm = nullptr) {
   float* S = h->smat[ws].as<float>();
   const long n = (long)h->n;
   DenseMfmaPlan p;
@@ -644,11 +645,14 @@
     if (f.small_hi && small_hi_ready(h, m, st)) {
       rc = profiled(h, st, [&] { return amdr_dense_small_approx_device(h->small, Qc, m, S, p.ld, h->small_eps.as<float>(), st); });
       if (rc) return rc;
-      if ((rc = dense_hi_select_launch(tail, q0, S, p.ld, n, m, k, h->X, Qc, h->d, h->small_eps.as<float>(), os, oi,
-                                       h->small_fb.as<unsigned int>(), st)))
-        return rc;
+      rc = bm ? hybrid_long_select_launch(*tail, *bm, q0, S, p.ld, n, m, k, h->X, Qc, h->d, h->small_eps.as<float>(), os, oi,
+                                          h->small_fb.as<unsigned int>(), st)
+              : dense_hi_select_launch(tail, q0, S, p.ld, n, m, k, h->X, Qc, h->d, h->small_eps.as<float>(), os, oi,
+                                       h->small_fb.as<unsigned int>(), st);
+      if (rc) return rc;
       continue;
     }
+    if (bm) return fail(AMDR_EINVAL, "dense: the BM25 channel can ride in the two-pass form's second pass only");
     rc = profiled(h, st, [&]() -> int {
       if (f.scores == PassForm::RowWaves) {
         hipLaunchKernelGGL(dense_all_scores_kernel, dim3(ceil_div((long)m * n, kWaves)), dim3(256), 0, st, h->X, n, h->d, Qc,
@@ -1007,6 +1011,51 @@
   AMDR_HIP(hipSetDevice(h->device));
   FuseTail tail{p, dense_row2uid, bm25_ids, bm25_scores, kb, bm25_row2uid, out_ids, out_vals, out_mask, out_count};
   return run_search(h, 0, Q_dev, nq, k, dense_scores_dev, dense_ids_dev, (hipStream_t)stream, &tail);
+}
+
+int amdr_hybrid_long_device(amdr_dense_t* h, amdr_bm25_t* bm25, const amdr_hybrid_long_args_t* a, int32_t* applied,
+                            void* stream) {
+  AMDR_REQUIRE(h && bm25 && a && applied, "hybrid_long: null argument");
+  *applied = 0;
+  const int nq = a->nq, k = a->kd, kb = a->kb;
+  int rc = check_search_args(h, a->Q_dev, nq, k, a->dense_scores_dev, a->dense_ids_dev);
+  if (rc) return rc;
+  AMDR_REQUIRE(a->p != nullptr, "hybrid_long: null params");
+  AMDR_REQUIRE(a->p->method >= 0 && a->p->method <= AMDR_FUSE_WEIGHTED_SUM, "hybrid_long: method=%d", a->p->method);
+  AMDR_REQUIRE(kb >= 1 && kb <= AMDR_MAX_K, "hybrid_long: kb=%d", kb);
+  AMDR_REQUIRE(nq == 0 || (a->q_ptr_dev && a->bm25_scores_dev && a->bm25_ids_dev), "hybrid_long: null BM25 buffers");
+  AMDR_REQUIRE(nq == 0 || (a->out_ids && a->out_vals && a->out_mask && a->out_count), "hybrid_long: null output");
+  const char* e = getenv("AMDR_HYBRID_LONG");
+  if (nq == 0 || (e && e[0] == '0')) return AMDR_OK;
+  std::lock_guard<std::mutex> g(h->mu);
+  std::lock_guard<std::mutex> gb(bm25_mutex(bm25));
+  AMDR_HIP(hipSetDevice(h->device));
+  hipStream_t st = (hipStream_t)stream;
+  LongBmJob job;
+  if ((rc = bm25_small_raw(bm25, nq, kb, &job.br))) return rc;
+  if (bm25_device_of(bm25) != h->device || !hybrid_long_kernel_exists(h->d, job.br)) return AMDR_OK;
+  const DensePins pins = read_pins();
+  const Route r = dense_route(h, pins, nq, k);
+  if (r.form != Form::Batched) return AMDR_OK;
+  FuseTail tail{a->p,       a->dense_row2uid, a->bm25_ids_dev, a->bm25_scores_dev, kb, a->bm25_row2uid,
+                a->out_ids, a->out_vals,      a->out_mask,     a->out_count};
+  const int sizes[2] = {nq < r.chunk ? nq : r.chunk, nq % r.chunk};
+  for (int m : sizes) {
+    if (m == 0) continue;
+    DenseMfmaPlan p;
+    dense_mfma_plan((long)h->n, h->d, m, k, &p);
+    if (!batched_pass_form(h, pins, r, p, m, k, &tail).small_hi || !small_hi_ready(h, m, st)) return AMDR_OK;
+  }
+  if ((rc = ensure_need(h, 0, call_need(h, r, nq, k)))) return rc;
+  job.q_terms = a->q_terms_dev;
+  job.q_ptr = (const long long*)a->q_ptr_dev;
+  job.nq_all = nq;
+  job.bm_scores = a->bm25_scores_dev;
+  job.bm_ids = a->bm25_ids_dev;
+  if ((rc = run_search_batched(h, 0, pins, r, a->Q_dev, nq, k, a->dense_scores_dev, a->dense_ids_dev, st, &tail, &job)))
+    return rc;
+  *applied = 1;
+  return AMDR_OK;
 }
 
 int amdr_dense_search(amdr_dense_t* h, const float* Q_host, int32_t nq, int32_t k, float* scores_host,
@@ -1113,7 +1162,8 @@
       snprintf(buf, buf_len,
                "dsh_scores_kernel fp16 first pass queries_per_launch=%d (dsh_split_queries_kernel + v_mfma_f32_32x32x16_f16 on "
                "fp16 roundings of both operands, proven per-query bound) + dense_hi_select_fuse_kernel (rows inside 2 eps of the "
-               "k-th best re-scored exactly, top-k, fusion); exact form: dense_panel_scores_kernel",
+               "k-th best re-scored exactly, top-k, fusion; with the BM25 channel in the same launch: "
+               "hybrid_long_select_fuse_kernel); exact form: dense_panel_scores_kernel",
                m);
     } else if (f.scores == PassForm::RowWaves) {
       snprintf(buf, buf_len, "dense_all_scores_kernel (one wave per query x row) + %s", tail);
diff --git a/legal-rag_amd/csrc/fuse.hip b/legal-rag_amd/csrc/fuse.hip
--- a/legal-rag_amd/csrc/fuse.hip
+++ b/legal-rag_amd/csrc/fuse.hip
@@ -1,6 +1,7 @@
 #include "bm25_core.hpp"
 #include "common.hpp"
 #include "dense_dot.hpp"
+#include "hybrid_long.hpp"
 #include "topk.hpp"
 
 #include <cfloat>
@@ -570,30 +571,16 @@
   return cnt;
 }
 
-template <bool FUSE, int D128>
-__global__ __launch_bounds__(64) void dense_hi_select_fuse_kernel(amdr_fuse_params_t P, const float* __restrict__ S, long ldS, long n,
-                                                                  int nq, int kd, const float* __restrict__ X,
-                                                                  const float* __restrict__ Q, int d,
-                                                                  const float* __restrict__ eps, float margin_scale,
-                                                                  float* __restrict__ fin_scores, long long* __restrict__ fin_ids,
-                                                                  ChanIn c0, ChanIn c1, int max_out,
-                                                                  long long* __restrict__ out_ids, double* __restrict__ out_vals,
-                                                                  int* __restrict__ out_mask, int* __restrict__ out_count,
-                                                                  unsigned int* __restrict__ fallbacks) {
-  extern __shared__ __attribute__((aligned(16))) unsigned char smem[];
-  C32* buf = reinterpret_cast<C32*>(smem);
-  const int lane = threadIdx.x, sl = lane & 31, half = lane >> 5;
-  const int q = 2 * blockIdx.x + half;
+template <int D128>
+__device__ __forceinline__ void dense_hi_select_pair(const float* __restrict__ S, long ldS, long n, int nq, int kd,
+                                                     const float* __restrict__ X, const float* __restrict__ Q, int d,
+                                                     const float* __restrict__ eps, float margin_scale,
+                                                     float* __restrict__ fin_scores, long long* __restrict__ fin_ids,
+                                                     unsigned int* __restrict__ fallbacks, C32* buf, int pair, int lane,
+                                                     long long& id0, double& s0) {
+  const int sl = lane & 31, half = lane >> 5;
+  const int q = 2 * pair + half;
   const bool has_q = q < nq;
-  FusePre pre;
-  pre.have[0] = pre.have[1] = true;
-  pre.have[2] = false;
-  pre.id[1] = -1;
-  pre.s[1] = 0.0;
-  if (FUSE && has_q && sl < c1.k) {
-    pre.id[1] = c1.ids[(size_t)q * c1.k + sl];
-    pre.s[1] = chan_score(c1, q, sl);
-  }
   const float e_q = has_q ? eps[q] : 0.f;
   const float margin = 2.f * e_q * margin_scale;
   bool exact_all = has_q && !(margin == margin && margin <= FLT_MAX);
@@ -661,7 +648,7 @@
     int g2 = select_row_pair_any(xs, ldS, n, q, has_q && exact_all, kd, lane, buf, o2);
     if (g2 < 0) {
       for (int hh = 0; hh < 2; ++hh) {
-        const int qq = 2 * blockIdx.x + hh;
+        const int qq = 2 * pair + hh;
         const bool mine_h = __shfl((int)exact_all, 32 * hh) != 0;
         if (qq >= nq || !mine_h) continue;
         const float* row = xs + (size_t)qq * ldS;
@@ -716,9 +703,36 @@
     fin_scores[(size_t)q * kd + sl] = v ? out.score() : -FLT_MAX;
     fin_ids[(size_t)q * kd + sl] = v ? out.id() : -1ll;
   }
+  id0 = v ? out.id() : -1ll;
+  s0 = v ? (double)out.score() : 0.0;
+}
+
+template <bool FUSE, int D128>
+__global__ __launch_bounds__(64) void dense_hi_select_fuse_kernel(amdr_fuse_params_t P, const float* __restrict__ S, long ldS, long n,
+                                                                  int nq, int kd, const float* __restrict__ X,
+                                                                  const float* __restrict__ Q, int d,
+                                                                  const float* __restrict__ eps, float margin_scale,
+                                                                  float* __restrict__ fin_scores, long long* __restrict__ fin_ids,
+                                                                  ChanIn c0, ChanIn c1, int max_out,
+                                                                  long long* __restrict__ out_ids, double* __restrict__ out_vals,
+                                                                  int* __restrict__ out_mask, int* __restrict__ out_count,
+                                                                  unsigned int* __restrict__ fallbacks) {
+  extern __shared__ __attribute__((aligned(16))) unsigned char smem[];
+  C32* buf = reinterpret_cast<C32*>(smem);
+  const int lane = threadIdx.x, sl = lane & 31;
+  const int q = 2 * blockIdx.x + (lane >> 5);
+  FusePre pre;
+  pre.have[0] = pre.have[1] = true;
+  pre.have[2] = false;
+  pre.id[1] = -1;
+  pre.s[1] = 0.0;
+  if (FUSE && q < nq && sl < c1.k) {
+    pre.id[1] = c1.ids[(size_t)q * c1.k + sl];
+    pre.s[1] = chan_score(c1, q, sl);
+  }
+  dense_hi_select_pair<D128>(S, ldS, n, nq, kd, X, Q, d, eps, margin_scale, fin_scores, fin_ids, fallbacks, buf, blockIdx.x, lane,
+                             pre.id[0], pre.s[0]);
   if (FUSE) {
-    pre.id[0] = v ? out.id() : -1ll;
-    pre.s[0] = v ? (double)out.score() : 0.0;
     ChanIn none;
     none.ids = nullptr;
     none.scores = nullptr;
@@ -727,6 +741,91 @@
     none.is_f64 = 0;
     fuse_packed_body<32, true>(P, c0, c1, none, nq, max_out, out_ids, out_vals, out_mask, out_count, pre, blockIdx.x * 2);
   }
+}
+
+struct LongBmArgs {
+  const long long* term_ptr;
+  const int* post_doc;
+  const double* post_w;
+  const double* idf;
+  long n_terms, n_docs;
+  const int* q_terms;
+  const long long* q_ptr;
+  int nq_all, q0;
+  int kb, cap, slab, use_select;
+  unsigned int region;
+  double* bm_scores;
+  long long* bm_ids;
+};
+
+template <int D128, int NVT>
+__global__ __launch_bounds__(128) void hybrid_long_select_fuse_kernel(
+    amdr_fuse_params_t P, const float* __restrict__ S, long ldS, long n, int nq, int kd, const float* __restrict__ X,
+    const float* __restrict__ Q, int d, const float* __restrict__ eps, float margin_scale, float* __restrict__ fin_scores,
+    long long* __restrict__ fin_ids, ChanIn c0, ChanIn c1, int max_out, long long* __restrict__ out_ids,
+    double* __restrict__ out_vals, int* __restrict__ out_mask, int* __restrict__ out_count,
+    unsigned int* __restrict__ fallbacks, LongBmArgs B) {
+  extern __shared__ __attribute__((aligned(16))) unsigned char smem[];
+  C32* buf = reinterpret_cast<C32*>(smem);
+  unsigned char* bm_smem = smem + 128 * sizeof(C32);
+  double* hand_s = reinterpret_cast<double*>(bm_smem + B.region);
+  long long* hand_i = reinterpret_cast<long long*>(hand_s + 2 * B.kb);
+  const int lane = threadIdx.x & 63, sl = lane & 31, half = lane >> 5;
+  const int wave = __builtin_amdgcn_readfirstlane((int)(threadIdx.x >> 6));
+  FusePre pre;
+  pre.have[0] = pre.have[1] = true;
+  pre.have[2] = false;
+  pre.id[0] = pre.id[1] = -1;
+  pre.s[0] = pre.s[1] = 0.0;
+  if (wave == 0) {
+    dense_hi_select_pair<D128>(S, ldS, n, nq, kd, X, Q, d, eps, margin_scale, fin_scores, fin_ids, fallbacks, buf, blockIdx.x, lane,
+                               pre.id[0], pre.s[0]);
+  } else {
+    for (int h = 0; h < 2; ++h) {
+      const int q = 2 * blockIdx.x + h;
+      if (q >= nq) break;
+      bm25_block_query<1, NVT>(B.term_ptr, B.post_doc, B.post_w, B.idf, B.n_terms, B.n_docs, B.q_terms, B.q_ptr, B.nq_all, B.kb,
+                               B.cap, B.slab, B.use_select, nullptr, nullptr, B.bm_scores, B.bm_ids, B.q0 + q, 0, lane, bm_smem,
+                               hand_s + h * B.kb, hand_i + h * B.kb);
+      wave_lds_fence();
+    }
+  }
+  __syncthreads();
+  if (wave != 0) return;
+  if (2 * blockIdx.x + half < nq && sl < B.kb) {
+    pre.id[1] = hand_i[half * B.kb + sl];
+    pre.s[1] = hand_s[half * B.kb + sl];
+  }
+  ChanIn none;
+  none.ids = nullptr;
+  none.scores = nullptr;
+  none.row2uid = nullptr;
+  none.k = 0;
+  none.is_f64 = 0;
+  fuse_packed_body<32, true>(P, c0, c1, none, nq, max_out, out_ids, out_vals, out_mask, out_count, pre, blockIdx.x * 2);
+}
+
+using HybridLongKernel = void (*)(amdr_fuse_params_t, const float*, long, long, int, int, const float*, const float*, int,
+                                  const float*, float, float*, long long*, ChanIn, ChanIn, int, long long*, double*, int*, int*,
+                                  unsigned int*, LongBmArgs);
+struct HybridLongEntry {
+  int d128, nvt;
+  HybridLongKernel fn;
+};
+#define AMDR_HL_ROW(D)                                                                                    \
+  {D, 4, hybrid_long_select_fuse_kernel<D, 4>}, {D, 8, hybrid_long_select_fuse_kernel<D, 8>},             \
+      {D, 10, hybrid_long_select_fuse_kernel<D, 10>}, {D, 16, hybrid_long_select_fuse_kernel<D, 16>}
+static const HybridLongEntry kHybridLongTable[] = {AMDR_HL_ROW(1), AMDR_HL_ROW(2), AMDR_HL_ROW(3), AMDR_HL_ROW(4),
+                                                   AMDR_HL_ROW(5), AMDR_HL_ROW(6), AMDR_HL_ROW(7), AMDR_HL_ROW(8)};
+#undef AMDR_HL_ROW
+static int hybrid_long_bucket(int nvt) { return nvt <= 4 ? 4 : nvt <= 8 ? 8 : nvt <= 10 ? 10 : nvt <= 16 ? 16 : 0; }
+static HybridLongKernel hybrid_long_find(int d, int nvt) {
+  for (const HybridLongEntry& e : kHybridLongTable)
+    if (d == 128 * e.d128 && hybrid_long_bucket(nvt) == e.nvt) return e.fn;
+  return nullptr;
+}
+bool hybrid_long_kernel_exists(int d, const Bm25Raw& br) {
+  return br.nslabs == 1 && br.argmax && hybrid_long_find(d, br.nvt) != nullptr;
 }
 
 struct SmallArgs {
@@ -786,7 +885,7 @@
   if (role == 0) {
     if (wave != 0) return;
     bm25_block_query<1, NVT>(A.term_ptr, A.post_doc, A.post_w, A.idf, A.n_terms, A.n_docs, A.q_terms, A.q_ptr, nq, A.kb,
-                             A.cap, A.slab, A.use_select, nullptr, nullptr, A.bm_scores, A.bm_ids, q, 0, smem);
+                             A.cap, A.slab, A.use_select, nullptr, nullptr, A.bm_scores, A.bm_ids, q, 0, lane, smem);
   } else {
     const long r0 = (long)(role - 1) * A.rows_per_block;
     long r1 = r0 + A.rows_per_block;
@@ -1026,6 +1125,43 @@
     }
 #undef AMDR_HSF_PLAIN
   }
+  AMDR_HIP(hipGetLastError());
+  return AMDR_OK;
+}
+
+int hybrid_long_select_launch(const FuseTail& t, const LongBmJob& j, int q0, const float* S, long ldS, long n, int m, int kd,
+                              const float* X, const float* Q, int d, const float* eps, float* fin_scores, int64_t* fin_ids,
+                              unsigned int* fallbacks, hipStream_t st) {
+  const char* ms = getenv("AMDR_DENSE_SMALL_HI_MARGIN");
+  const float margin_scale = ms ? (float)atof(ms) : 1.f;
+  const HybridLongKernel fn = hybrid_long_find(d, j.br.nvt);
+  if (!fn || j.br.nslabs != 1 || !j.br.argmax) return fail(AMDR_EINVAL, "hybrid_long: no kernel for d=%d, %d scores per lane", d, j.br.nvt);
+  LongBmArgs B;
+  B.term_ptr = j.br.term_ptr;
+  B.post_doc = j.br.post_doc;
+  B.post_w = j.br.post_w;
+  B.idf = j.br.idf;
+  B.n_terms = j.br.n_terms;
+  B.n_docs = j.br.n_docs;
+  B.q_terms = j.q_terms;
+  B.q_ptr = j.q_ptr;
+  B.nq_all = j.nq_all;
+  B.q0 = q0;
+  B.kb = t.kb;
+  B.cap = j.br.cap;
+  B.slab = j.br.slab;
+  B.use_select = j.br.select_on ? 1 : 0;
+  B.region = (unsigned int)((j.br.lds + 15) / 16 * 16);
+  B.bm_scores = j.bm_scores;
+  B.bm_ids = (long long*)j.bm_ids;
+  const int mo = kd + t.kb;
+  ChanIn c0{nullptr, nullptr, (const long long*)t.dense_row2uid, kd, 0};
+  ChanIn c1{nullptr, nullptr, (const long long*)t.bm25_row2uid, t.kb, 1};
+  const size_t lds = 128 * sizeof(C32) + B.region + (size_t)2 * t.kb * 16;
+  hipLaunchKernelGGL(fn, dim3((m + 1) / 2), dim3(128), lds, st, *t.p, S, ldS, n, m, kd, X, Q, d, eps, margin_scale, fin_scores,
+                     (long long*)fin_ids, c0, c1, mo, (long long*)(t.out_ids + (size_t)q0 * mo),
+                     t.out_vals + (size_t)q0 * mo * AMDR_FUSE_NVALS, t.out_mask + (size_t)q0 * mo, t.out_count + q0, fallbacks,
+                     B);
   AMDR_HIP(hipGetLastError());
   return AMDR_OK;
 }
diff --git a/legal-rag_amd/csrc/hybrid_long.hpp b/legal-rag_amd/csrc/hybrid_long.hpp
--- /dev/null
+++ b/legal-rag_amd/csrc/hybrid_long.hpp
@@ -0,0 +1,20 @@
+#pragma once
+#include "common.hpp"
+
+namespace amdr {
+
+struct LongBmJob {
+  Bm25Raw br;
+  const int* q_terms;
+  const long long* q_ptr;
+  int nq_all;
+  double* bm_scores;
+  int64_t* bm_ids;
+};
+bool hybrid_long_kernel_exists(int d, const Bm25Raw& br);
+int hybrid_long_select_launch(const FuseTail& t, const LongBmJob& job, int q0, const float* S, long ldS, long n, int m, int kd,
+                              const float* X, const float* Q, int d, const float* eps, float* fin_scores, int64_t* fin_ids,
+                              unsigned int* fallbacks, hipStream_t st);
+int bm25_device_of(const amdr_bm25_t* h);
+
+}
diff --git a/legal-rag_amd/retrieval/engine.py b/legal-rag_amd/retrieval/engine.py
--- a/legal-rag_amd/retrieval/engine.py
+++ b/legal-rag_amd/retrieval/engine.py
@@ -289,6 +289,31 @@
         res.bm25_scores, res.bm25_ids = bs, bi
         return res
 
+    def _hybrid_long(self, params: _native.FuseParams, q_emb: torch.Tensor, q_terms: torch.Tensor, q_ptr: torch.Tensor,
+                     k: int) -> Optional[BatchResult]:
+        nq = int(q_emb.shape[0])
+        assert q_emb.is_cuda and q_emb.dtype == torch.float32 and q_emb.is_contiguous()
+        assert q_terms.dtype == torch.int32 and q_ptr.dtype == torch.int64 and q_terms.is_cuda and q_ptr.is_cuda
+        assert q_ptr.shape[0] - 1 == nq
+        ds = self._buf("ds", (nq, k), torch.float32)
+        di = self._buf("di", (nq, k), torch.int64)
+        bs = self._buf("bs", (nq, k), torch.float64)
+        bi = self._buf("bi", (nq, k), torch.int64)
+        pk, ids, vals, mask, count = self._fused_outputs(nq, 2 * k)
+        m0, m1 = self.maps[0], self.maps[1]
+        args = _native.HybridLongArgs(
+            Q_dev=q_emb.data_ptr(), q_terms_dev=q_terms.data_ptr(), q_ptr_dev=q_ptr.data_ptr(), nq=nq, kd=k, kb=k,
+            dense_row2uid=m0.data_ptr() if m0 is not None else 0, bm25_row2uid=m1.data_ptr() if m1 is not None else 0,
+            dense_scores_dev=ds.data_ptr(), dense_ids_dev=di.data_ptr(), bm25_scores_dev=bs.data_ptr(),
+            bm25_ids_dev=bi.data_ptr(), out_ids=ids.data_ptr(), out_vals=vals.data_ptr(), out_mask=mask.data_ptr(),
+            out_count=count.data_ptr())
+        if not _native.hybrid_long_device(self.dense, self.bm25, params, args, _stream()):
+            return None
+        res = BatchResult(ids=ids, vals=vals, mask=mask, count=count, packed=pk)
+        res.dense_scores, res.dense_ids = ds, di
+        res.bm25_scores, res.bm25_ids = bs, bi
+        return res
+
     def rerank_blend(self, res: BatchResult, ce_raw: torch.Tensor, beta: float) -> BatchResult:
         nq, mo = res.ids.shape
         assert ce_raw.is_cuda and ce_raw.dtype == torch.float64 and ce_raw.is_contiguous() and ce_raw.shape[0] == nq
@@ -316,6 +341,10 @@
             nq = int(q_emb.shape[0])
             if nq <= 4 and 2 * k <= 32:
                 return self._hybrid_small(params, q_emb, q_terms, q_ptr, k)
+            if nq > 4:
+                res = self._hybrid_long(params, q_emb, q_terms, q_ptr, k)
+                if res is not None:
+                    return res
             b = self.bm25_topk(q_terms, q_ptr, k)
             d, res = self.dense_topk_fuse(params, q_emb, k, b)
             res.dense_scores, res.dense_ids = d
```
